# NVlabs/latentfusion

Hardware: AMD Instinct MI355X
Metric: pose-optim iters/sec (reconstruct+render+backward), 16 views, 128^3 voxels (higher is better)
Workload: dtype f32

## Files before the change

### include/lf_hip.h

```cpp
#ifndef LF_HIP_H
#define LF_HIP_H

#include <stddef.h>
#include <stdint.h>

#ifdef __cplusplus
extern "C" {
#endif

#define LF_ABI_VERSION 1

#define LF_EINVAL   (-1)
#define LF_EALIGN   (-2)
#define LF_ENOSPC   (-3)

#define LF_EPI_LRELU     1u
#define LF_EPI_PIXELNORM 2u
#define LF_EPI_ADD       4u
#define LF_EPI_DOT       8u

#define LF_MAP_O2C 0
#define LF_MAP_C2O 1
#define LF_MAP_COEFS 20

int lf_abi_version(void);

int lf_device_name(char* buf, int buflen);

int lf_resample3d_fwd(const float* vol, int vol_n, const float* coef, int kind,
                      float* out, int N, int D, int H, int W, int C, void* stream);

size_t lf_resample3d_bwd_coef_scratch_bytes(int N, int D, int H, int W);
int lf_resample3d_bwd_coef(const float* gout, const float* vol, int vol_n, const float* coef,
                           float* gcoef, void* scratch, size_t scratch_bytes,
                           int N, int D, int H, int W, int C, void* stream);
size_t lf_resample3d_bwd_coef_part_scratch_bytes(int N, int part_n, int D, int H, int W);
int lf_resample3d_bwd_coef_part(const float* gout, const float* vol, int vol_n, const float* coef,
                                float* gcoef, void* scratch, size_t scratch_bytes,
                                int N, int D, int H, int W, int C, int part_n, void* stream);

int lf_resample3d_fwd_indexed(const float* vol, int vol_n, const int32_t* vol_idx, const float* coef, int kind,
                              float* out, int N, int D, int H, int W, int C, void* stream);
size_t lf_resample3d_bwd_coef_indexed_scratch_bytes(int N, int part_n, int D, int H, int W);
int lf_resample3d_bwd_coef_indexed(const float* gout, const float* vol, int vol_n, const int32_t* vol_idx, const float* coef,
                                   float* gcoef, void* scratch, size_t scratch_bytes,
                                   int N, int D, int H, int W, int C, int part_n, void* stream);


size_t lf_resample3d_bwd_vol_det_scratch_bytes(int vol_n, int D, int H, int W, int C);
int lf_resample3d_bwd_vol_det(const float* gout, const float* coef, int kind, float* gvol, int vol_n, void* scratch,
                              size_t scratch_bytes, int N, int D, int H, int W, int C, void* stream);

int lf_conv3x3_cout_padded(int Cout);
int lf_conv1x1_cout_padded(int Cout);

int lf_conv3x3_fwd(const float* x, const float* wpack, const float* bias, float* y, float* norm_out,
                   int dims, int N, int D, int H, int W, int Cin, int Cout,
                   float he, unsigned flags, float slope, float eps, void* stream);

int lf_conv1x1_fwd(const float* x, const float* wpack, const float* bias, float* y, float* norm_out,
                   int N, int P, int Cin, int ksl, long x_batch_stride, long x_slice_stride,
                   int Cout, long y_batch_stride, int y_row_stride, int y_slice_channels,
                   long y_slice_stride,
                   float he, unsigned flags, float slope, float eps, void* stream);
int lf_conv1x1_fwd_scaled(const float* x, const float* xscale, const float* wpack, const float* bias, float* y, float* norm_out,
                          int N, int P, int Cin, int ksl, long x_batch_stride, long x_slice_stride,
                          int Cout, long y_batch_stride, int y_row_stride, int y_slice_channels,
                          long y_slice_stride,
                          float he, unsigned flags, float slope, float eps, void* stream);

int lf_conv3x3_bwd_data(const float* gy, const float* wpack_t, float* gx, int dims, int N, int D, int H, int W,
                        int Cin, int Cout, float he, const float* prev_y, const float* prev_norm,
                        unsigned prev_flags, float slope, void* stream);
int lf_conv1x1_bwd_data(const float* gy, const float* wpack_t, float* gx, int N, int P, int Cin, int Cout,
                        long y_batch_stride, int y_row_stride, int y_slice_channels, long y_slice_stride,
                        float he, const float* prev_y, const float* prev_norm, unsigned prev_flags,
                        float slope, float* amax_out, void* stream);

#define LF_AMAX_FLOATS 2048
size_t lf_conv3d_c16_split_wpack_halfs(void);
void lf_conv3d_c16_split_pairs(int* taps28);
int lf_conv3d_c16_split(const float* x, const void* wsplit, const float* bias, float* y, float* norm_out,
                        int N, int D, int H, int W, float he, unsigned flags, float slope, float eps,
                        const float* prev_y, const float* prev_norm, unsigned prev_flags,
                        const float* amax_in, float* amax_out, void* stream);

size_t lf_conv3d_c16_wino_upack_floats(void);
int lf_conv3d_c16_wino(const float* x, const float* upack, const float* bias, float* y, float* norm_out,
                       int N, int D, int H, int W, float he, unsigned flags, float slope, float eps,
                       const float* prev_y, const float* prev_norm, unsigned prev_flags,
                       float* amax_out, void* stream);

size_t lf_conv3d_c16_wino_proj_pack_floats(int D);
int lf_conv3d_c16_wino_projfwd(const float* x, const float* upack, const float* bias, float* y, float* norm_out,
                               int N, int D, int H, int W, float he, unsigned flags, float slope, float eps,
                               const float* proj_wA, const float* proj_bias, float* zp, float* pnorm,
                               float proj_he, unsigned proj_flags, void* stream);

int lf_round_bf16(const float* x, float* y, long n, void* stream);
size_t lf_conv3d_c16_ring_bf16_wpack_elems(void);
int lf_conv3d_c16_ring_bf16(const float* x, const void* wpack, const float* bias, float* y, float* norm_out,
                            int N, int D, int H, int W, float he, unsigned flags, float slope, float eps,
                            const float* addend, int round_out, void* stream);
#define LF_IO_IN_BF16 1
#define LF_IO_OUT_BF16 2
#define LF_IO_ADDEND_BF16 4
int lf_conv3d_c16_ring_bf16_io(const void* x, const void* wpack, const float* bias, void* y, float* norm_out,
                               int N, int D, int H, int W, float he, unsigned flags, float slope, float eps,
                               const void* addend, int round_out, int io, void* stream);

#define LF_RING_ADD_BF16 1u
#define LF_RING_OUT_BF16 2u
#define LF_RING_ROUND 4u
#define LF_RING_EX_NONE 0
#define LF_RING_EX_RH 1
#define LF_RING_EX_BLEND 2
#define LF_RING_EX_ABWD 3
#define LF_RING_EX_BLOCK 4
#define LF_RING_EX_PREV 5
int lf_conv3d_c16_ring_multi(const void* x, int x_bf16, const void* wpack, int ngroups,
                             void* y0, const void* add0, unsigned flags0, void* y1, const void* add1, unsigned flags1,
                             int extra, const void* e0, const void* e1, void* o2,
                             int N, int D, int H, int W, float he, int addend_per_sample, void* stream);
int lf_conv3d_c16_ring_blend(const void* rh, const void* wpack, void* cand, const void* addend, const float* h, const void* upre,
                             float* h_new, void* h_new_bf16, int N, int D, int H, int W, float he, void* stream);

long lf_wino3d_tiles(int N, int D, int H, int W);
int lf_wino3d_input_transform(const float* x, float* V, int N, int D, int H, int W, int C, void* stream);

#define LF_OUT_DEPTH_INNER 0x100u
int lf_wino_fused_cout_padded(int Cout);
size_t lf_wino_fused_scratch_bytes(int dims, int N, int D, int H, int W, int Cout);
int lf_wino_fused_gemm(const float* V, const float* U2, const float* bias, float* y, void* scratch, size_t scratch_bytes,
                       int dims, int N, int D, int H, int W, int Cin, int Cout, float he, unsigned flags, float slope,
                       void* stream);

size_t lf_wino_fused_scratch_bytes_part(int dims, int N, int D, int H, int W, int Cout, int part_n);
int lf_wino_fused_gemm_part(const float* V, const float* U2, const float* bias, float* y, void* scratch, size_t scratch_bytes,
                            int dims, int N, int D, int H, int W, int Cin, int Cout, float he, unsigned flags, float slope,
                            int part_n, void* stream);

int lf_rows_gemm_cout_padded(int Cout);
int lf_rows_gemm_epi(const float* x, const float* wpack, const float* bias, float* y, float* norm_out,
                     long M, int K, int Cout, float he, unsigned flags, float slope, float eps, void* stream);

int lf_wino_f16x3_cin_padded(int Cin);
int lf_wino3d_input_transform_f16x3(const float* x, const float* amax_in, void* V, int N, int D, int H, int W, int C, void* stream);
size_t lf_wino_fused_f16x3_scratch_bytes(int N, int D, int H, int W, int Cout);
int lf_wino_fused_f16x3_gemm(const void* V, const void* U2, int eU, const float* amax_in, const float* bias, float* y,
                             float* amax_out, void* scratch, size_t scratch_bytes, int N, int D, int H, int W, int Cin, int Cout,
                             float he, unsigned flags, float slope, void* stream);

long lf_wino2d_tiles(int N, int H, int W);
int lf_wino2d_input_transform(const float* x, float* V, int N, int H, int W, int C, void* stream);

int lf_wino2d_input_transform_f16x3(const float* x, void* V, int* eV, int N, int H, int W, int C, void* stream);
size_t lf_wino_fused2d_f16x3_scratch_bytes(int N, int H, int W, int Cout);
int lf_wino_fused2d_f16x3_gemm(const void* V, const int* eV, const void* U2, int eU, const float* bias, float* y, void* scratch,
                               size_t scratch_bytes, int N, int H, int W, int Cin, int Cout, float he, unsigned flags, float slope,
                               void* stream);

int lf_gru_stage_a(const float* upre, const float* rpre, int pre_stride, const float* h, float* u, float* rec,
                   long nvox, int Ch, int rec_stride, int rec_off, void* stream);
int lf_gru_stage_b(const float* h, const float* u, const float* cand, float* h_out, float* rec, long nvox, int Ch,
                   int rec_stride, int rec_off, void* stream);
int lf_gru_stage_b_bwd(const float* g, const float* h, const float* u, const float* cand, float* gh, float* gu, float* gc,
                       long n, void* stream);
int lf_gru_stage_a_bwd(const float* gu, const float* grh, const float* u, const float* rpre, const float* h, float* gupre,
                       float* grpre, float* gh, long n, void* stream);
int lf_gru_train_stage_a(const void* rpre, const float* h, void* rh, long n, int bf16, void* stream);
int lf_gru_train_stage_b(const float* h, const void* upre, const void* cand, float* h_out, long n, int bf16, void* stream);
int lf_gru_train_stage_b_bwd(const float* g, const float* h, const void* upre, const void* cand, float* gh1, void* gupre,
                             void* gc, float* acc_u, float* acc_o, long n, int bf16, void* stream);
int lf_gru_train_stage_a_bwd(const void* grh, const void* rpre, const float* h, const float* gh1, void* grpre, float* gh12,
                             float* acc_r, long n, int bf16, void* stream);
int lf_sum_views_bf16(const void* src, float* dst, long n, int views, int accumulate, void* stream);

int lf_resample3d_fwd_io(const void* vol, int vol_n, const float* coef, int kind, void* out, int N, int D, int H, int W,
                         int io, void* stream);
size_t lf_resample3d_bwd_vol_det_io_scratch_bytes(int vol_n, int N, int D, int H, int W);
int lf_resample3d_bwd_vol_det_io(const void* gout, const float* coef, int kind, void* gvol, int vol_n, void* scratch,
                                 size_t scratch_bytes, int N, int D, int H, int W, int io, void* stream);

int lf_occ_input_fwd(const float* z, const float* w, const float* b, float* ta, float* t16, int N, int D, long P, float slope,
                     void* stream);
int lf_occ_input_bwd(const float* gta, const float* ta, const float* gp16, const float* w, const float* g_zs, const float* wocc,
                     float* gz, long rows, float slope, const float* prev_y, const float* prev_norm, unsigned prev_flags,
                     void* stream);
int lf_occ_input_bwd_proj(const float* gta, const float* gp16, const float* w, const float* gp2d, const float* wpack_t, float he_p,
                          const float* wocc, float* gz, int N, int D, long P, float slope,
                          const float* prev_y, const float* prev_norm, unsigned prev_flags, void* stream);
int lf_occ_weight_grad(const float* z, const float* gp2d, const float* wpack_t, float he_p, float* gw, int N, int D, long P, void* stream);
int lf_occ_weight_grad_softmax_bwd(const float* z, const float* gp2d, const float* wpack_t, float he_p, const float* weights,
                                   float* glogits, int N, int D, long P, void* stream);
int lf_occ_head_bwd(const float* gl, const float* w16, float he, const float* y, const float* norm, unsigned flags, float slope,
                    float* g, long rows, void* stream);
int lf_occ_conv17_fwd(const float* t16, const float* w27, float* pre, int N, int D, int H, int W, void* stream);
int lf_occ_conv17_bwd(const float* g, const float* t16, const float* w27, float* gp16, int N, int D, int H, int W, float slope,
                      void* stream);
int lf_column_reduce_sum_fwd(const float* x, float* y, int N, int D, long P, int C, void* stream);
int lf_column_reduce_sum_bwd(const float* gy, float* gx, int N, int D, long P, int C, void* stream);
int lf_column_softmax_fwd(const float* logits, float* weights, float* zdepth, int N, int D, long P, void* stream);
int lf_column_softmax_head_fwd(const float* y, const float* w16, const float* bias, float he, float* weights, float* zdepth,
                               int N, int D, long P, void* stream);
int lf_column_softmax_bwd(const float* weights, const float* gweights, const float* gzdepth, float* glogits,
                          int N, int D, long P, void* stream);
int lf_column_scale_fwd(const float* z, const float* w, float* out, long rows, int C, void* stream);
int lf_column_scale_bwd(const float* gout, const float* z, const float* w, float* gz, float* gw, long rows, int C,
                        void* stream);

#define LF_FUSE_MEAN   0
#define LF_FUSE_MAX    1
#define LF_FUSE_ABSMAX 2
#define LF_FUSE_MEDIAN 3
int lf_fuse_views_fwd(const float* z, float* out, int* idx, int kind, int V, long n, long view_stride, void* stream);
int lf_fuse_views_bwd(const float* g, const int* idx, float* gz, int kind, int V, long n, long view_stride, void* stream);
int lf_fuse_blend_fwd(const float* z, const float* logits, float* weights, float* out, int V, long rows, int C,
                      long z_view_stride, long logit_view_stride, void* stream);
int lf_fuse_blend_bwd(const float* g, const float* z, const float* weights, float* gz, float* glogits, int V, long rows,
                      int C, long z_view_stride, long logit_view_stride, void* stream);

int lf_lstm_cell_fwd(const float* cc, const float* c_cur, float* h_next, float* c_next, long nvox, int Ch, void* stream);
int lf_lstm_cell_bwd(const float* cc, const float* c_cur, const float* gh, const float* gcn, float* gcc, float* gc,
                     long nvox, int Ch, void* stream);

int lf_grid_sample2d_fwd(const float* img, const float* grid, float* out, int N, int C, int H, int W, int Ho, int Wo,
                         int bilinear, int border, void* stream);
int lf_grid_sample2d_bwd(const float* img, const float* grid, const float* gout, float* gimg, float* ggrid,
                         int N, int C, int H, int W, int Ho, int Wo, int bilinear, int border, void* stream);

#define LF_IBR_PAIR_FLOATS 32
#define LF_IBR_PAIR_SPLIT 16
#define LF_IBR_VIEW_FLOATS 16
#define LF_IBR_VIEW_SPLIT 8
int lf_ibr_reproject_fwd(const float* image_in, const float* depth_in, const float* depth_out, const float* mask_out,
                         const float* pair_rec, const float* in_rec, const float* out_rec, float* image_re, float* depth_re,
                         int B, int Vo, int Vi, int C, int H, int W, long image_row_stride, long depth_row_stride, void* stream);
int lf_ibr_reproject_bwd(const float* image_in, const float* depth_in, const float* depth_out, const float* mask_out,
                         const float* pair_rec, const float* in_rec, const float* out_rec, const float* g_image_re,
                         const float* g_depth_re, float* g_image_in, float* g_depth_in, float* g_depth_out,
                         int B, int Vo, int Vi, int C, int H, int W, void* stream);

size_t lf_conv_bwd_weight_scratch_bytes(int dims, int N, int D, int H, int W, int Cin, int Cout);
int lf_conv_bwd_weight(const float* x, const float* gpre, float* gw, void* scratch, size_t scratch_bytes,
                       int dims, int N, int D, int H, int W, int Cin, int Cout, float scale, void* stream);
size_t lf_conv_bwd_weight_bf16_scratch_bytes(int dims, int N, int D, int H, int W, int Cin, int Cout);
int lf_conv_bwd_weight_bf16(const float* x, const float* gpre, float* gw, void* scratch, size_t scratch_bytes,
                            int dims, int N, int D, int H, int W, int Cin, int Cout, float scale, void* stream);
int lf_conv_bwd_weight_bf16_io(const void* x, const void* gpre, float* gw, void* scratch, size_t scratch_bytes,
                               int dims, int N, int D, int H, int W, int Cin, int Cout, float scale, int io, void* stream);
size_t lf_conv_bwd_weight_wide_scratch_bytes(int dims, int N, int D, int H, int W, int Cin, int Cout);
int lf_conv_bwd_weight_wide(const float* x, const float* gpre, float* gw, void* scratch, size_t scratch_bytes,
                            int dims, int N, int D, int H, int W, int Cin, int Cout, float scale, void* stream);

size_t lf_epilogue_bwd_c16_scratch_bytes(long rows);
int lf_epilogue_bwd_c16(const void* gy, const void* y, const float* norm, void* gp, float* gbias, void* scratch,
                        size_t scratch_bytes, long rows, unsigned flags, float slope, int io, void* stream);

int lf_lift16_fwd(const float* x, const void* wtab, const float* btab, void* vol, float* norm, long R, long P, int S,
                  float he, float slope, float eps, void* stream);
size_t lf_lift16_bwd_scratch_bytes(int S);
int lf_lift16_bwd(const void* gvol, const void* yvol, const float* norm, const float* x, const void* wtab_t, float* gx, float* gw,
                  float* gb, void* scratch, size_t scratch_bytes, long R, long P, int S, float he, float slope, int round_gx,
                  void* stream);

int lf_proj16_fwd(const void* vol, const void* wtab, const float* bias, float* y, float* norm, long R, long P, int S, float he,
                  float slope, float eps, void* stream);
size_t lf_proj16_bwd_scratch_bytes(int S);
int lf_proj16_bwd(const float* gp, const void* vol, const void* wtab_t, void* gxvol, float* gw, void* scratch, size_t scratch_bytes,
                  long R, long P, int S, float he, void* stream);

int lf_pw16_fwd(const void* x, int x_bf16, const void* w_bf16, const float* bias, float he, unsigned flags, float slope, void* y,
                long rows, void* stream);
size_t lf_pw16_bwd_scratch_bytes(long rows);
int lf_pw16_bwd(const void* gy_bf16, const void* wt_bf16, float he, void* gx, int gx_bf16, float* gbias, void* scratch,
                size_t scratch_bytes, long rows, void* stream);

int lf_pixelnorm_fwd(const float* x, float* y, float* norm_out, long rows, int C, float eps, void* stream);

int lf_epilogue_bwd(const float* gy, const float* y, const float* norm, float* gp,
                    long rows, int C, unsigned flags, float slope, void* stream);
int lf_epilogue_bwd_amax(const float* gy, const float* y, const float* norm, float* gp,
                         long rows, int C, unsigned flags, float slope, float* amax_out, void* stream);

size_t lf_latent_cosine_scratch_bytes(int N, long P, int C);
int lf_latent_cosine_fwd(const float* zp, const float* zt, int zt_n, long zt_sn, long zt_sp, long zt_sc, float* sums,
                         float* losses, float w_latent, void* scratch, size_t scratch_bytes, int N, long P, int C,
                         void* stream);
int lf_latent_cosine_bwd_epi(const float* g_in, const float* zp, const float* norm, const float* zt, int zt_n, long zt_sn,
                             long zt_sp, long zt_sc, const float* sums, float gscale, float* gp, int N, long P, int C,
                             unsigned flags, float slope, void* stream);

size_t lf_nn_dist_scratch_bytes(int B, int M, int Q);
int lf_nn_dist(const float* x1, long x1_sb, const float* T1, const float* x2, long x2_sb, const float* T2, float* dist, int* idx,
               float* mean, void* scratch, size_t scratch_bytes, int B, int M, int Q, void* stream);
size_t lf_points_pair_dist_scratch_bytes(int R, int P);
int lf_points_pair_dist(const float* pts, long pts_sr, const float* A, const float* Bm, int rows, float* mean, void* scratch,
                        size_t scratch_bytes, int R, int P, void* stream);

int lf_resize_fwd(const float* x, float* y, int dims, int N, int D, int H, int W, int C, int linear, int up,
                  void* stream);
int lf_resize_bwd(const float* gy, float* gx, int dims, int N, int D, int H, int W, int C, int linear, int up,
                  void* stream);

#define LF_CAM_PARAMS 10
#define LF_CAM_COEFS  24
int lf_camera_coefs(const float* params, const float* intrinsics, float cube_size, float z_span,
                    int crop_h, int crop_w, float* coefs, float* jac, int N, void* stream);
int lf_camera_coefs_bwd(const float* gcoefs, const float* jac, float* gparams, int N, void* stream);

size_t lf_pose_loss_scratch_bytes(int N, int h, int w, int H, int W);
int lf_pose_loss_fwd(const float* logits, const float* coefs, const float* target_depth,
                     const float* target_mask, const float* weights, float* sums, float* losses,
                     float* gsums, void* scratch, size_t scratch_bytes,
                     int N, int h, int w, int H, int W, void* stream);
int lf_pose_loss_bwd(const float* logits, const float* coefs, const float* target_depth,
                     const float* target_mask, const float* gsums, float* glogits, float* gcoefs,
                     void* scratch, size_t scratch_bytes, int N, int h, int w, int H, int W, void* stream);
int lf_pose_loss_fwd_masked(const float* logits, const float* coefs, const float* target_depth,
                            const float* target_mask, const float* weights, float* sums, float* losses,
                            void* scratch, size_t scratch_bytes, int N, int h, int w, int H, int W, void* stream);
int lf_pose_loss_fwd_depth(const float* depth_and_logits, const float* coefs, const float* target_depth,
                           const float* target_mask, const float* weights, float* sums, float* losses,
                           float* gsums, void* scratch, size_t scratch_bytes,
                           int N, int h, int w, int H, int W, void* stream);
int lf_pose_loss_bwd_depth(const float* depth_and_logits, const float* coefs, const float* target_depth,
                           const float* target_mask, const float* gsums, float* gcrop, float* gcoefs,
                           void* scratch, size_t scratch_bytes, int N, int h, int w, int H, int W, void* stream);
int lf_pose_loss_fwd_mt(const float* logits, const float* coefs, const float* target_depth,
                        const float* target_mask, const float* weights, float* sums, float* losses,
                        float* gsums, void* scratch, size_t scratch_bytes,
                        int N, int T, int n, int h, int w, int H, int W, void* stream);
int lf_pose_loss_fwd_masked_mt(const float* logits, const float* coefs, const float* target_depth,
                               const float* target_mask, const float* weights, float* sums, float* losses,
                               void* scratch, size_t scratch_bytes, int N, int T, int n, int h, int w, int H, int W,
                               void* stream);
int lf_pose_loss_bwd_mt(const float* logits, const float* coefs, const float* target_depth,
                        const float* target_mask, const float* gsums, float* glogits, float* gcoefs,
                        void* scratch, size_t scratch_bytes, int N, int T, int n, int h, int w, int H, int W,
                        void* stream);

int lf_adam_step(float* params, const float* grads, float* exp_avg, float* exp_avg_sq,
                 const float* step_size, const float* lr, float bias_correction2_sqrt,
                 float beta1, float beta2, float eps, float weight_decay, int N, int P, void* stream);

int lf_nchw_to_nhwc(const float* src, float* dst, int N, int C, long P, void* stream);
int lf_nhwc_to_nchw(const float* src, float* dst, int N, int C, long P, void* stream);
int lf_lift_unfold(const float* src, const float* norm_or_null, float* dst,
                   int N, long P, int C0, int S, void* stream);
int lf_lift_permute(const float* src, float* dst, int N, long P, int C0, int S, int fold, void* stream);
int lf_lift_norm_unfold(const float* src, void* dst, float* norm_out, int N, long P, int C0, int S, float eps, int out_bf16,
                        void* stream);
int lf_lift_bwd(const void* gvol, const void* yvol, const float* norm, float* gp, int N, long P, int C0, int S, float slope,
                int round_bf16, int io, void* stream);

#ifdef __cplusplus
}
#endif
#endif
```

### latentfusion_amd/_lib.py

```python
import ctypes
import os
from ctypes import c_char_p, c_float, c_int, c_long, c_size_t, c_uint, c_void_p

_HERE = os.path.dirname(os.path.abspath(__file__))
LIB_PATH = os.path.join(_HERE, 'csrc', 'liblf_hip.so')

LF_EPI_LRELU = 1
LF_EPI_PIXELNORM = 2
LF_EPI_ADD = 4
LF_EPI_DOT = 8
LF_RING_ADD_BF16, LF_RING_OUT_BF16, LF_RING_ROUND = 1, 2, 4
LF_RING_EX_NONE, LF_RING_EX_RH, LF_RING_EX_BLEND, LF_RING_EX_ABWD, LF_RING_EX_BLOCK, LF_RING_EX_PREV = 0, 1, 2, 3, 4, 5
LF_OUT_DEPTH_INNER = 0x100
LF_IO_IN_BF16, LF_IO_OUT_BF16, LF_IO_ADDEND_BF16 = 1, 2, 4
LF_MAP_O2C = 0
LF_MAP_C2O = 1
LF_MAP_COEFS = 20
LF_FUSE_MEAN, LF_FUSE_MAX, LF_FUSE_ABSMAX, LF_FUSE_MEDIAN = 0, 1, 2, 3
LF_IBR_PAIR_FLOATS, LF_IBR_PAIR_SPLIT, LF_IBR_VIEW_FLOATS, LF_IBR_VIEW_SPLIT = 32, 16, 16, 8
LF_AMAX_FLOATS = 2048

P = c_void_p
SIGNATURES = {
    'lf_abi_version': (c_int, []),
    'lf_device_name': (c_int, [c_char_p, c_int]),
    'lf_resample3d_fwd': (c_int, [P, c_int, P, c_int, P, c_int, c_int, c_int, c_int, c_int, P]),
    'lf_resample3d_bwd_coef_scratch_bytes': (c_size_t, [c_int, c_int, c_int, c_int]),
    'lf_resample3d_bwd_coef': (c_int, [P, P, c_int, P, P, P, c_size_t, c_int, c_int, c_int, c_int, c_int, P]),
    'lf_resample3d_bwd_coef_part_scratch_bytes': (c_size_t, [c_int, c_int, c_int, c_int, c_int]),
    'lf_resample3d_bwd_coef_part': (c_int, [P, P, c_int, P, P, P, c_size_t, c_int, c_int, c_int, c_int, c_int, c_int, P]),
    'lf_resample3d_fwd_indexed': (c_int, [P, c_int, P, P, c_int, P, c_int, c_int, c_int, c_int, c_int, P]),
    'lf_resample3d_bwd_coef_indexed_scratch_bytes': (c_size_t, [c_int, c_int, c_int, c_int, c_int]),
    'lf_resample3d_bwd_coef_indexed': (c_int, [P, P, c_int, P, P, P, P, c_size_t, c_int, c_int, c_int, c_int, c_int, c_int, P]),
    'lf_resample3d_bwd_vol_det_scratch_bytes': (c_size_t, [c_int, c_int, c_int, c_int, c_int]),
    'lf_resample3d_bwd_vol_det': (c_int, [P, P, c_int, P, c_int, P, c_size_t, c_int, c_int, c_int, c_int, c_int, P]),
    'lf_conv3x3_cout_padded': (c_int, [c_int]),
    'lf_conv1x1_cout_padded': (c_int, [c_int]),
    'lf_conv3x3_fwd': (c_int, [P, P, P, P, P, c_int, c_int, c_int, c_int, c_int, c_int, c_int,
                               c_float, c_uint, c_float, c_float, P]),
    'lf_conv1x1_fwd': (c_int, [P, P, P, P, P, c_int, c_int, c_int, c_int, c_long, c_long, c_int, c_long, c_int,
                               c_int, c_long, c_float, c_uint, c_float, c_float, P]),
    'lf_conv1x1_fwd_scaled': (c_int, [P, P, P, P, P, P, c_int, c_int, c_int, c_int, c_long, c_long, c_int, c_long, c_int,
                                      c_int, c_long, c_float, c_uint, c_float, c_float, P]),
    'lf_conv3x3_bwd_data': (c_int, [P, P, P, c_int, c_int, c_int, c_int, c_int, c_int, c_int, c_float, P, P, c_uint,
                                    c_float, P]),
    'lf_conv1x1_bwd_data': (c_int, [P, P, P, c_int, c_int, c_int, c_int, c_long, c_int, c_int, c_long, c_float, P, P,
                                    c_uint, c_float, P, P]),
    'lf_conv3d_c16_split_wpack_halfs': (c_size_t, []),
    'lf_conv3d_c16_split_pairs': (None, [P]),
    'lf_conv3d_c16_split': (c_int, [P, P, P, P, P, c_int, c_int, c_int, c_int, c_float, c_uint, c_float, c_float, P, P,
                                    c_uint, P, P, P]),
    'lf_conv3d_c16_wino_upack_floats': (c_size_t, []),
    'lf_conv3d_c16_wino': (c_int, [P, P, P, P, P, c_int, c_int, c_int, c_int, c_float, c_uint, c_float, c_float, P, P,
                                   c_uint, P, P]),
    'lf_conv3d_c16_wino_proj_pack_floats': (c_size_t, [c_int]),
    'lf_conv3d_c16_wino_projfwd': (c_int, [P, P, P, P, P, c_int, c_int, c_int, c_int, c_float, c_uint, c_float, c_float,
                                           P, P, P, P, c_float, c_uint, P]),
    'lf_round_bf16': (c_int, [P, P, c_long, P]),
    'lf_conv3d_c16_ring_bf16_wpack_elems': (c_size_t, []),
    'lf_conv3d_c16_ring_bf16': (c_int, [P, P, P, P, P, c_int, c_int, c_int, c_int, c_float, c_uint, c_float, c_float, P, c_int, P]),
    'lf_conv3d_c16_ring_bf16_io': (c_int, [P, P, P, P, P, c_int, c_int, c_int, c_int, c_float, c_uint, c_float, c_float, P, c_int, c_int, P]),
    'lf_conv3d_c16_ring_multi': (c_int, [P, c_int, P, c_int, P, P, c_uint, P, P, c_uint, c_int, P, P, P, c_int, c_int, c_int, c_int, c_float, c_int, P]),
    'lf_conv3d_c16_ring_blend': (c_int, [P, P, P, P, P, P, P, P, c_int, c_int, c_int, c_int, c_float, P]),
    'lf_wino3d_tiles': (c_long, [c_int, c_int, c_int, c_int]),
    'lf_wino3d_input_transform': (c_int, [P, P, c_int, c_int, c_int, c_int, c_int, P]),
    'lf_wino_fused_cout_padded': (c_int, [c_int]),
    'lf_wino_fused_scratch_bytes': (c_size_t, [c_int, c_int, c_int, c_int, c_int, c_int]),
    'lf_wino_fused_gemm': (c_int, [P, P, P, P, P, c_size_t, c_int, c_int, c_int, c_int, c_int, c_int, c_int, c_float, c_uint, c_float, P]),
    'lf_wino_fused_scratch_bytes_part': (c_size_t, [c_int, c_int, c_int, c_int, c_int, c_int, c_int]),
    'lf_wino_fused_gemm_part': (c_int, [P, P, P, P, P, c_size_t, c_int, c_int, c_int, c_int, c_int, c_int, c_int, c_float, c_uint, c_float, c_int, P]),
    'lf_rows_gemm_cout_padded': (c_int, [c_int]),
    'lf_rows_gemm_epi': (c_int, [P, P, P, P, P, c_long, c_int, c_int, c_float, c_uint, c_float, c_float, P]),
    'lf_wino_f16x3_cin_padded': (c_int, [c_int]),
    'lf_wino3d_input_transform_f16x3': (c_int, [P, P, P, c_int, c_int, c_int, c_int, c_int, P]),
    'lf_wino_fused_f16x3_scratch_bytes': (c_size_t, [c_int, c_int, c_int, c_int, c_int]),
    'lf_wino_fused_f16x3_gemm': (c_int, [P, P, c_int, P, P, P, P, P, c_size_t, c_int, c_int, c_int, c_int, c_int, c_int,
                                         c_float, c_uint, c_float, P]),
    'lf_wino2d_tiles': (c_long, [c_int, c_int, c_int]),
    'lf_wino2d_input_transform': (c_int, [P, P, c_int, c_int, c_int, c_int, P]),
    'lf_wino2d_input_transform_f16x3': (c_int, [P, P, P, c_int, c_int, c_int, c_int, P]),
    'lf_wino_fused2d_f16x3_scratch_bytes': (c_size_t, [c_int, c_int, c_int, c_int]),
    'lf_wino_fused2d_f16x3_gemm': (c_int, [P, P, P, c_int, P, P, P, c_size_t, c_int, c_int, c_int, c_int, c_int, c_float, c_uint,
                                           c_float, P]),
    'lf_gru_stage_a': (c_int, [P, P, c_int, P, P, P, c_long, c_int, c_int, c_int, P]),
    'lf_gru_stage_b': (c_int, [P, P, P, P, P, c_long, c_int, c_int, c_int, P]),
    'lf_lstm_cell_fwd': (c_int, [P, P, P, P, c_long, c_int, P]),
    'lf_lstm_cell_bwd': (c_int, [P, P, P, P, P, P, c_long, c_int, P]),
    'lf_gru_stage_b_bwd': (c_int, [P, P, P, P, P, P, P, c_long, P]),
    'lf_gru_stage_a_bwd': (c_int, [P, P, P, P, P, P, P, P, c_long, P]),
    'lf_gru_train_stage_a': (c_int, [P, P, P, c_long, c_int, P]),
    'lf_gru_train_stage_b': (c_int, [P, P, P, P, c_long, c_int, P]),
    'lf_gru_train_stage_b_bwd': (c_int, [P, P, P, P, P, P, P, P, P, c_long, c_int, P]),
    'lf_gru_train_stage_a_bwd': (c_int, [P, P, P, P, P, P, P, c_long, c_int, P]),
    'lf_lift16_fwd': (c_int, [P, P, P, P, P, c_long, c_long, c_int, c_float, c_float, c_float, P]),
    'lf_lift16_bwd_scratch_bytes': (c_size_t, [c_int]),
    'lf_lift16_bwd': (c_int, [P, P, P, P, P, P, P, P, P, c_size_t, c_long, c_long, c_int, c_float, c_float, c_int, P]),
    'lf_proj16_fwd': (c_int, [P, P, P, P, P, c_long, c_long, c_int, c_float, c_float, c_float, P]),
    'lf_proj16_bwd_scratch_bytes': (c_size_t, [c_int]),
    'lf_proj16_bwd': (c_int, [P, P, P, P, P, P, c_size_t, c_long, c_long, c_int, c_float, P]),
    'lf_sum_views_bf16': (c_int, [P, P, c_long, c_int, c_int, P]),
    'lf_occ_input_fwd': (c_int, [P, P, P, P, P, c_int, c_int, c_long, c_float, P]),
    'lf_occ_input_bwd': (c_int, [P, P, P, P, P, P, P, c_long, c_float, P, P, c_uint, P]),
    'lf_occ_conv17_fwd': (c_int, [P, P, P, c_int, c_int, c_int, c_int, P]),
    'lf_occ_conv17_bwd': (c_int, [P, P, P, P, c_int, c_int, c_int, c_int, c_float, P]),
    'lf_column_reduce_sum_fwd': (c_int, [P, P, c_int, c_int, c_long, c_int, P]),
    'lf_column_reduce_sum_bwd': (c_int, [P, P, c_int, c_int, c_long, c_int, P]),
    'lf_column_softmax_fwd': (c_int, [P, P, P, c_int, c_int, c_long, P]),
    'lf_occ_input_bwd_proj': (c_int, [P, P, P, P, P, c_float, P, P, c_int, c_int, c_long, c_float, P, P, c_uint, P]),
    'lf_occ_weight_grad': (c_int, [P, P, P, c_float, P, c_int, c_int, c_long, P]),
    'lf_pw16_fwd': (c_int, [P, c_int, P, P, c_float, c_uint, c_float, P, c_long, P]),
    'lf_pw16_bwd_scratch_bytes': (c_size_t, [c_long]),
    'lf_pw16_bwd': (c_int, [P, P, c_float, P, c_int, P, P, c_size_t, c_long, P]),
    'lf_occ_weight_grad_softmax_bwd': (c_int, [P, P, P, c_float, P, P, c_int, c_int, c_long, P]),
    'lf_occ_head_bwd': (c_int, [P, P, c_float, P, P, c_uint, c_float, P, c_long, P]),
    'lf_column_softmax_head_fwd': (c_int, [P, P, P, c_float, P, P, c_int, c_int, c_long, P]),
    'lf_column_softmax_bwd': (c_int, [P, P, P, P, c_int, c_int, c_long, P]),
    'lf_column_scale_fwd': (c_int, [P, P, P, c_long, c_int, P]),
    'lf_column_scale_bwd': (c_int, [P, P, P, P, P, c_long, c_int, P]),
    'lf_fuse_views_fwd': (c_int, [P, P, P, c_int, c_int, c_long, c_long, P]),
    'lf_fuse_views_bwd': (c_int, [P, P, P, c_int, c_int, c_long, c_long, P]),
    'lf_fuse_blend_fwd': (c_int, [P, P, P, P, c_int, c_long, c_int, c_long, c_long, P]),
    'lf_fuse_blend_bwd': (c_int, [P, P, P, P, P, c_int, c_long, c_int, c_long, c_long, P]),
    'lf_grid_sample2d_fwd': (c_int, [P, P, P, c_int, c_int, c_int, c_int, c_int, c_int, c_int, c_int, P]),
    'lf_grid_sample2d_bwd': (c_int, [P, P, P, P, P, c_int, c_int, c_int, c_int, c_int, c_int, c_int, c_int, P]),
    'lf_ibr_reproject_fwd': (c_int, [P, P, P, P, P, P, P, P, P, c_int, c_int, c_int, c_int, c_int, c_int, c_long, c_long, P]),
    'lf_ibr_reproject_bwd': (c_int, [P, P, P, P, P, P, P, P, P, P, P, P, c_int, c_int, c_int, c_int, c_int, c_int, P]),
    'lf_conv_bwd_weight_scratch_bytes': (c_size_t, [c_int, c_int, c_int, c_int, c_int, c_int, c_int]),
    'lf_conv_bwd_weight': (c_int, [P, P, P, P, c_size_t, c_int, c_int, c_int, c_int, c_int, c_int, c_int, c_float, P]),
    'lf_conv_bwd_weight_bf16_scratch_bytes': (c_size_t, [c_int, c_int, c_int, c_int, c_int, c_int, c_int]),
    'lf_conv_bwd_weight_bf16': (c_int, [P, P, P, P, c_size_t, c_int, c_int, c_int, c_int, c_int, c_int, c_int, c_float, P]),
    'lf_conv_bwd_weight_bf16_io': (c_int, [P, P, P, P, c_size_t, c_int, c_int, c_int, c_int, c_int, c_int, c_int, c_float, c_int, P]),
    'lf_conv_bwd_weight_wide_scratch_bytes': (c_size_t, [c_int, c_int, c_int, c_int, c_int, c_int, c_int]),
    'lf_conv_bwd_weight_wide': (c_int, [P, P, P, P, c_size_t, c_int, c_int, c_int, c_int, c_int, c_int, c_int, c_float, P]),
    'lf_pixelnorm_fwd': (c_int, [P, P, P, c_long, c_int, c_float, P]),
    'lf_epilogue_bwd': (c_int, [P, P, P, P, c_long, c_int, c_uint, c_float, P]),
    'lf_epilogue_bwd_amax': (c_int, [P, P, P, P, c_long, c_int, c_uint, c_float, P, P]),
    'lf_latent_cosine_scratch_bytes': (c_size_t, [c_int, c_long, c_int]),
    'lf_latent_cosine_fwd': (c_int, [P, P, c_int, c_long, c_long, c_long, P, P, c_float, P, c_size_t, c_int, c_long, c_int, P]),
    'lf_latent_cosine_bwd_epi': (c_int, [P, P, P, P, c_int, c_long, c_long, c_long, P, c_float, P, c_int, c_long, c_int, c_uint,
                                         c_float, P]),
    'lf_nn_dist_scratch_bytes': (c_size_t, [c_int, c_int, c_int]),
    'lf_nn_dist': (c_int, [P, c_long, P, P, c_long, P, P, P, P, P, c_size_t, c_int, c_int, c_int, P]),
    'lf_points_pair_dist_scratch_bytes': (c_size_t, [c_int, c_int]),
    'lf_points_pair_dist': (c_int, [P, c_long, P, P, c_int, P, P, c_size_t, c_int, c_int, P]),
    'lf_epilogue_bwd_c16_scratch_bytes': (c_size_t, [c_long]),
    'lf_epilogue_bwd_c16': (c_int, [P, P, P, P, P, P, c_size_t, c_long, c_uint, c_float, c_int, P]),
    'lf_resample3d_fwd_io': (c_int, [P, c_int, P, c_int, P, c_int, c_int, c_int, c_int, c_int, P]),
    'lf_resample3d_bwd_vol_det_io_scratch_bytes': (c_size_t, [c_int, c_int, c_int, c_int, c_int]),
    'lf_resample3d_bwd_vol_det_io': (c_int, [P, P, c_int, P, c_int, P, c_size_t, c_int, c_int, c_int, c_int, c_int, P]),
    'lf_resize_fwd': (c_int, [P, P, c_int, c_int, c_int, c_int, c_int, c_int, c_int, c_int, P]),
    'lf_resize_bwd': (c_int, [P, P, c_int, c_int, c_int, c_int, c_int, c_int, c_int, c_int, P]),
    'lf_camera_coefs': (c_int, [P, P, c_float, c_float, c_int, c_int, P, P, c_int, P]),
    'lf_camera_coefs_bwd': (c_int, [P, P, P, c_int, P]),
    'lf_pose_loss_scratch_bytes': (c_size_t, [c_int, c_int, c_int, c_int, c_int]),
    'lf_pose_loss_fwd': (c_int, [P, P, P, P, P, P, P, P, P, c_size_t, c_int, c_int, c_int, c_int, c_int, P]),
    'lf_pose_loss_bwd': (c_int, [P, P, P, P, P, P, P, P, c_size_t, c_int, c_int, c_int, c_int, c_int, P]),
    'lf_pose_loss_fwd_depth': (c_int, [P, P, P, P, P, P, P, P, P, c_size_t, c_int, c_int, c_int, c_int, c_int, P]),
    'lf_pose_loss_bwd_depth': (c_int, [P, P, P, P, P, P, P, P, c_size_t, c_int, c_int, c_int, c_int, c_int, P]),
    'lf_pose_loss_fwd_masked': (c_int, [P, P, P, P, P, P, P, P, c_size_t, c_int, c_int, c_int, c_int, c_int, P]),
    'lf_pose_loss_fwd_mt': (c_int, [P, P, P, P, P, P, P, P, P, c_size_t, c_int, c_int, c_int, c_int, c_int, c_int, c_int, P]),
    'lf_pose_loss_fwd_masked_mt': (c_int, [P, P, P, P, P, P, P, P, c_size_t, c_int, c_int, c_int, c_int, c_int, c_int, c_int,
                                           P]),
    'lf_pose_loss_bwd_mt': (c_int, [P, P, P, P, P, P, P, P, c_size_t, c_int, c_int, c_int, c_int, c_int, c_int, c_int, P]),
    'lf_adam_step': (c_int, [P, P, P, P, P, P, c_float, c_float, c_float, c_float, c_float, c_int, c_int, P]),
    'lf_nchw_to_nhwc': (c_int, [P, P, c_int, c_int, c_long, P]),
    'lf_nhwc_to_nchw': (c_int, [P, P, c_int, c_int, c_long, P]),
    'lf_lift_unfold': (c_int, [P, P, P, c_int, c_long, c_int, c_int, P]),
    'lf_lift_permute': (c_int, [P, P, c_int, c_long, c_int, c_int, c_int, P]),
    'lf_lift_norm_unfold': (c_int, [P, P, P, c_int, c_long, c_int, c_int, c_float, c_int, P]),
    'lf_lift_bwd': (c_int, [P, P, P, P, c_int, c_long, c_int, c_int, c_float, c_int, c_int, P]),
}

EXPERIMENTAL_SIGNATURES = {
    'lf_set_tuning': (c_int, [c_int, c_int]),
    'lf_resample3d_bwd_vol': (c_int, [P, P, c_int, P, c_int, c_int, c_int, c_int, c_int, c_int, P]),
    'lf_conv3d_c16_wino_projbwd': (c_int, [P, P, c_float, P, P, c_uint, P, P, c_int, c_int, c_int, c_int, c_float, c_float,
                                           P, P, c_uint, P]),
    'lf_conv3d_c16_wino_split_upack_halfs': (c_size_t, []),
    'lf_conv3d_c16_wino_split': (c_int, [P, P, P, P, P, c_int, c_int, c_int, c_int, c_float, c_uint, c_float, c_float, P, P,
                                         c_uint, P, P, P]),
    'lf_conv3d_c16_bf16_wpack_elems': (c_size_t, []),
    'lf_conv3d_c16_bf16': (c_int, [P, P, P, P, P, c_int, c_int, c_int, c_int, c_float, c_uint, c_float, c_float, c_int, P]),
    'lf_wino3d_output_transform': (c_int, [P, P, P, P, c_int, c_int, c_int, c_int, c_int, c_float, c_uint, c_float, c_float, P]),
    'lf_wino2d_output_transform': (c_int, [P, P, P, P, c_int, c_int, c_int, c_int, c_float, c_uint, c_float, c_float, P]),
}

_lib = None


class LFHipError(RuntimeError):
    pass


def lib():
    global _lib
    if _lib is not None:
        return _lib
    if not os.path.exists(LIB_PATH):
        try:
            from .csrc import build as _build
            _build.build(verbose=False)
        except Exception as e:
            raise LFHipError(f'liblf_hip.so is missing at {LIB_PATH} and could not be built: {e}') from e
    import torch
    try:
        handle = ctypes.CDLL(LIB_PATH)
    except OSError as e:
        raise LFHipError(f'cannot load {LIB_PATH}: {e}') from e
    for name, (res, args) in list(SIGNATURES.items()) + list(EXPERIMENTAL_SIGNATURES.items()):
        try:
            fn = getattr(handle, name)
        except AttributeError as e:
            raise LFHipError(f'{LIB_PATH} does not export {name}') from e
        fn.restype = res
        fn.argtypes = args
    if handle.lf_abi_version() != 1:
        raise LFHipError('liblf_hip.so ABI version mismatch')
    _lib = handle
    return _lib


_ERR = {-1: 'LF_EINVAL (bad size/flag combination)', -2: 'LF_EALIGN (alignment / channel count)',
        -3: 'LF_ENOSPC (scratch too small)'}


BYTE_LOG = None
_PENDING = [0]


def note_bytes(t, scratch=False):
    if BYTE_LOG is not None and not scratch:
        n = t.numel() * t.element_size()
        try:
            n = min(n, t.untyped_storage().nbytes() - t.storage_offset() * t.element_size())
        except Exception:
            pass
        _PENDING[0] += n


def check(rc, what):
    if BYTE_LOG is not None:
        e = BYTE_LOG.setdefault(what, [0, 0])
        e[0] += 1
        e[1] += _PENDING[0]
        _PENDING[0] = 0
    if rc != 0:
        raise LFHipError(f'{what} failed: {_ERR.get(rc, "hipError " + str(rc))}')
```

### latentfusion_amd/csrc/image.hip

```cpp
#include "lf_common.h"

namespace {

constexpr int NP = 10;
template <int ND>
struct DualT {
  double v;
  double d[ND];
};
template <int ND> __device__ inline DualT<ND> dconst_(double c) { DualT<ND> r; r.v = c; for (int i = 0; i < ND; ++i) r.d[i] = 0.0; return r; }
template <int ND> __device__ inline DualT<ND> dvar_(double c, int idx, int mine) {
  DualT<ND> r = dconst_<ND>(c);
  if (ND == 1) r.d[0] = (idx == mine) ? 1.0 : 0.0; else r.d[idx % ND] = 1.0;
  return r;
}
template <int ND> __device__ inline DualT<ND> operator+(const DualT<ND>& a, const DualT<ND>& b) { DualT<ND> r; r.v = a.v + b.v; for (int i = 0; i < ND; ++i) r.d[i] = a.d[i] + b.d[i]; return r; }
template <int ND> __device__ inline DualT<ND> operator-(const DualT<ND>& a, const DualT<ND>& b) { DualT<ND> r; r.v = a.v - b.v; for (int i = 0; i < ND; ++i) r.d[i] = a.d[i] - b.d[i]; return r; }
template <int ND> __device__ inline DualT<ND> operator-(const DualT<ND>& a) { DualT<ND> r; r.v = -a.v; for (int i = 0; i < ND; ++i) r.d[i] = -a.d[i]; return r; }
template <int ND> __device__ inline DualT<ND> operator*(const DualT<ND>& a, const DualT<ND>& b) { DualT<ND> r; r.v = a.v * b.v; for (int i = 0; i < ND; ++i) r.d[i] = a.d[i] * b.v + a.v * b.d[i]; return r; }
template <int ND> __device__ inline DualT<ND> operator*(const DualT<ND>& a, double s) { DualT<ND> r; r.v = a.v * s; for (int i = 0; i < ND; ++i) r.d[i] = a.d[i] * s; return r; }
template <int ND> __device__ inline DualT<ND> operator+(const DualT<ND>& a, double s) { DualT<ND> r = a; r.v += s; return r; }
template <int ND> __device__ inline DualT<ND> operator-(const DualT<ND>& a, double s) { DualT<ND> r = a; r.v -= s; return r; }
template <int ND> __device__ inline DualT<ND> operator/(const DualT<ND>& a, const DualT<ND>& b) {
  DualT<ND> r; const double inv = 1.0 / b.v; r.v = a.v * inv;
  for (int i = 0; i < ND; ++i) r.d[i] = (a.d[i] - r.v * b.d[i]) * inv;
  return r;
}
template <int ND> __device__ inline DualT<ND> dsqrt(const DualT<ND>& a) {
  DualT<ND> r; r.v = sqrt(a.v); const double k = r.v > 0.0 ? 0.5 / r.v : 0.0;
  for (int i = 0; i < ND; ++i) r.d[i] = a.d[i] * k;
  return r;
}
template <int ND> __device__ inline DualT<ND> dsin(const DualT<ND>& a) { DualT<ND> r; r.v = sin(a.v); const double c = cos(a.v); for (int i = 0; i < ND; ++i) r.d[i] = a.d[i] * c; return r; }
template <int ND> __device__ inline DualT<ND> dcos(const DualT<ND>& a) { DualT<ND> r; r.v = cos(a.v); const double s = -sin(a.v); for (int i = 0; i < ND; ++i) r.d[i] = a.d[i] * s; return r; }
template <int ND> __device__ inline DualT<ND> dclamp_min(const DualT<ND>& a, double lo) { return a.v >= lo ? a : dconst_<ND>(lo); }

constexpr int NOUT = 24;

template <int ND>
__global__ void camera_coefs_kernel(const float* __restrict__ params, const float* __restrict__ intr,
                                    float cube, float z_span, int crop_h, int crop_w,
                                    float* __restrict__ out, float* __restrict__ jac, int N) {
  typedef DualT<ND> Dual;
  const int tid = blockIdx.x * blockDim.x + threadIdx.x;
  const int n = ND == 1 ? tid / NP : tid, mine = ND == 1 ? tid % NP : 0;
  if (n >= N) return;
  auto dconst = [](double c) { return dconst_<ND>(c); };
  auto dvar = [&](double c, int idx) { return dvar_<ND>(c, idx, mine); };
  const float* p = params + n * NP;
  Dual w[3], t[3], vp[4];
  for (int i = 0; i < 3; ++i) w[i] = dvar((double)p[i], i);
  for (int i = 0; i < 3; ++i) t[i] = dvar((double)p[3 + i], 3 + i);
  for (int i = 0; i < 4; ++i) vp[i] = dvar((double)p[6 + i], 6 + i);
  const double fu = intr[n * 4 + 0], fv = intr[n * 4 + 1], u0 = intr[n * 4 + 2], v0 = intr[n * 4 + 3];

  const Dual theta = dsqrt(w[0] * w[0] + w[1] * w[1] + w[2] * w[2]);
  const Dual sc = dsin(theta) / dclamp_min(theta, 1e-8);
  Dual q[4] = {dcos(theta), sc * w[0], sc * w[1], sc * w[2]};
  for (int rep = 0; rep < 2; ++rep) {
    const Dual nrm = dclamp_min(dsqrt(q[0] * q[0] + q[1] * q[1] + q[2] * q[2] + q[3] * q[3]), 1e-12);
    for (int i = 0; i < 4; ++i) q[i] = q[i] / nrm;
  }
  const Dual qw = q[0], qx = q[1], qy = q[2], qz = q[3];
  const Dual tx = qx * 2.0, ty = qy * 2.0, tz = qz * 2.0;
  Dual R[3][3];
  R[0][0] = dconst(1.0) - (ty * qy + tz * qz); R[0][1] = ty * qx - tz * qw;               R[0][2] = tz * qx + ty * qw;
  R[1][0] = ty * qx + tz * qw;               R[1][1] = dconst(1.0) - (tx * qx + tz * qz); R[1][2] = tz * qy - tx * qw;
  R[2][0] = tz * qx - ty * qw;               R[2][1] = tz * qy + tx * qw;               R[2][2] = dconst(1.0) - (tx * qx + ty * qy);

  const Dual vw = vp[2] - vp[0], vh = vp[3] - vp[1];
  const Dual al0 = (vp[0] - u0) * (1.0 / fu), al1 = vw * (1.0 / fu);
  const Dual be0 = (vp[1] - v0) * (1.0 / fv), be1 = vh * (1.0 / fv);
  const Dual g0 = t[2] - (double)z_span;
  const double g1 = z_span, s = 2.0 / cube;
  Dual c[6][3];
  for (int r = 0; r < 3; ++r) {
    const Dual m0 = R[0][r], m1 = R[1][r], m2 = R[2][r];
    const Dual rt = m0 * t[0] + m1 * t[1] + m2 * t[2];
    c[0][r] = (al0 * g0 * m0 + be0 * g0 * m1 + g0 * m2 - rt) * s;
    c[1][r] = (al1 * g0 * m0) * s;
    c[2][r] = (be1 * g0 * m1) * s;
    c[3][r] = (al0 * m0 + be0 * m1 + m2) * (g1 * s);
    c[4][r] = (al1 * m0) * (g1 * s);
    c[5][r] = (be1 * m1) * (g1 * s);
  }
  Dual o[NOUT];
  for (int j = 0; j < 6; ++j) for (int r = 0; r < 3; ++r) o[j * 3 + r] = c[j][r];
  o[18] = dconst((double)crop_w) / vw;
  o[19] = -(vp[0] * o[18]) - 0.5;
  o[20] = dconst((double)crop_h) / vh;
  o[21] = -(vp[1] * o[20]) - 0.5;
  o[22] = dconst((double)z_span + 0.01);
  o[23] = t[2];
  for (int j = 0; j < NOUT; ++j) {
    if (ND != 1 || mine == 0) out[n * NOUT + j] = (float)o[j].v;
    if (ND == 1) jac[(n * NOUT + j) * NP + mine] = (float)o[j].d[0];
    else for (int i = 0; i < ND; ++i) jac[(n * NOUT + j) * NP + i] = (float)o[j].d[i];
  }
}

__global__ void camera_coefs_bwd_kernel(const float* __restrict__ gout, const float* __restrict__ jac,
                                        float* __restrict__ gparams, int N) {
  const int idx = blockIdx.x * blockDim.x + threadIdx.x;
  if (idx >= N * NP) return;
  const int n = idx / NP, i = idx % NP;
  double s = 0.0;
  for (int j = 0; j < NOUT; ++j) s += (double)gout[n * NOUT + j] * (double)jac[(n * NOUT + j) * NP + i];
  gparams[idx] = (float)s;
}

constexpr int NSUM = 8;
constexpr int LOSS_BLOCK = 256;

struct PixelFwd {
  float sig, dhat, pd, td, mt, valid, l1, logit;
  float wx0, wx1, wy0, wy1, mx, my;
  int x0, x1, y0, y1, xn, yn;
  float dn;
  bool mask_on;
};

__device__ __forceinline__ float sigmoidf_(float v) { return 1.f / (1.f + expf(-v)); }

__device__ __forceinline__ void clip_pos(float p, int size, float& pos, float& mult) {
  const float hi = (float)(size - 1);
  mult = (p > 0.f && p < hi) ? 1.f : 0.f;
  pos = fminf(fmaxf(p, 0.f), hi);
}

template <int MODE = 0>
__device__ __forceinline__ PixelFwd pixel_forward(const float* __restrict__ lg, const float* __restrict__ cf,
                                                  int h, int w, int x, int y, float td_raw, float mt) {
  PixelFwd r;
  float px, py;
  clip_pos(cf[0] * (float)x + cf[1], w, px, r.mx);
  clip_pos(cf[2] * (float)y + cf[3], h, py, r.my);
  const float fx = floorf(px), fy = floorf(py);
  r.wx1 = px - fx; r.wx0 = 1.f - r.wx1; r.wy1 = py - fy; r.wy0 = 1.f - r.wy1;
  r.x0 = (int)fx; r.y0 = (int)fy; r.x1 = min(r.x0 + 1, w - 1); r.y1 = min(r.y0 + 1, h - 1);
  r.xn = (int)nearbyintf(px); r.yn = (int)nearbyintf(py);
  const float m00 = lg[(r.y0 * w + r.x0) * 2 + 1], m01 = lg[(r.y0 * w + r.x1) * 2 + 1];
  const float m10 = lg[(r.y1 * w + r.x0) * 2 + 1], m11 = lg[(r.y1 * w + r.x1) * 2 + 1];
  r.logit = m00 * (r.wx0 * r.wy0) + m01 * (r.wx1 * r.wy0) + m10 * (r.wx0 * r.wy1) + m11 * (r.wx1 * r.wy1);
  r.sig = sigmoidf_(r.logit);
  const float dl = lg[(r.yn * w + r.xn) * 2 + 0], ml = lg[(r.yn * w + r.xn) * 2 + 1];
  if constexpr (MODE == 2) {
    r.mask_on = true;
    r.dn = dl;
    r.dhat = dl;
  } else {
    r.mask_on = sigmoidf_(ml) > 0.5f;
    r.dn = r.mask_on ? tanhf(dl) : (dl != dl ? dl : -1.f);
    r.dhat = r.dn * cf[4] + cf[5];
    if constexpr (MODE == 1) r.dhat *= sigmoidf_(ml);
  }
  r.pd = r.dhat * r.sig;
  r.mt = mt;
  r.valid = (td_raw == 0.f && mt > 0.1f) ? 0.f : 1.f;
  r.td = td_raw * mt;
  r.l1 = fabsf(r.pd - r.td) * r.valid;
  return r;
}

__device__ __forceinline__ void block_reduce_store(float (&acc)[NSUM], float* __restrict__ dst) {
  __shared__ float red[LOSS_BLOCK / 64][NSUM];
  const int lane = threadIdx.x & 63, wave = threadIdx.x >> 6;
#pragma unroll
  for (int i = 0; i < NSUM; ++i) {
    const float s = lf_wave_sum(acc[i]);
    if (lane == 0) red[wave][i] = s;
  }
  __syncthreads();
  if (threadIdx.x < NSUM) {
    float s = 0.f;
    for (int wv = 0; wv < LOSS_BLOCK / 64; ++wv) s += red[wv][threadIdx.x];
    dst[threadIdx.x] = s;
  }
}

template <int MODE>
__global__ void __launch_bounds__(LOSS_BLOCK) pose_loss_fwd_kernel(
    const float* __restrict__ logits, const float* __restrict__ coef, const float* __restrict__ tdepth,
    const float* __restrict__ tmask, float* __restrict__ partial, int nblk, int h, int w, int H, int W) {
  const int n = blockIdx.y;
  const float* lg = logits + (long)n * h * w * 2;
  const float* cf = coef + n * NOUT + 18;
  float acc[NSUM];
#pragma unroll
  for (int i = 0; i < NSUM; ++i) acc[i] = 0.f;
  for (int p = blockIdx.x * LOSS_BLOCK + threadIdx.x; p < H * W; p += nblk * LOSS_BLOCK) {
    const int y = p / W, x = p - y * W;
    const PixelFwd f = pixel_forward<MODE>(lg, cf, h, w, x, y, tdepth[p], tmask[p]);
    acc[0] += f.l1;
    acc[1] += f.l1 * (f.sig * f.mt);
    acc[2] += f.sig * f.mt;
    acc[3] += f.sig;
    acc[4] += f.sig * (f.mt * f.valid);
    acc[5] += f.mt * f.valid;
    acc[6] += (1.f - f.mt) * f.logit + (log1pf(expf(-fabsf(f.logit))) + fmaxf(-f.logit, 0.f));
  }
  block_reduce_store(acc, partial + ((long)n * nblk + blockIdx.x) * NSUM);
}

__global__ void pose_loss_finish_kernel(const float* __restrict__ partial, int nblk, const float* __restrict__ weights,
                                        int N, int HW, float* __restrict__ sums, float* __restrict__ losses,
                                        float* __restrict__ gsums) {
  const int n = blockIdx.x;
  __shared__ double S[NSUM];
#pragma unroll
  for (int c = 0; c < NSUM; ++c) {
    double s = 0.0;
    for (int b = threadIdx.x; b < nblk; b += 64) s += (double)partial[((long)n * nblk + b) * NSUM + c];
#pragma unroll
    for (int o = 32; o > 0; o >>= 1) s += __shfl_xor(s, o, 64);
    if (threadIdx.x == 0) {
      S[c] = s;
      sums[n * NSUM + c] = (float)s;
    }
  }
  __syncthreads();
  if (threadIdx.x == 0) {
    const float S0 = (float)S[0], S1 = (float)S[1], S2 = (float)S[2], S3 = (float)S[3], S4 = (float)S[4],
                S5 = (float)S[5], S6 = (float)S[6];
    const float w_depth = weights[0], w_ov = weights[1], w_iou = weights[2], w_mask = weights[3];
    const float inv_hw = 1.f / (float)HW;
    const float depth = S0 * inv_hw;
    auto clamp_min = [](float v, float lo) { return v < lo ? lo : v; };
    const float num = clamp_min(S1, 1e-5f), den = clamp_min(S2, 1e-4f);
    const float ov = num / den;
    const float uni = S3 + S5 - S4;
    const float iou = logf(clamp_min(uni, 1e-4f)) - logf(clamp_min(S4, 1e-4f));
    const float mask = S6 * inv_hw;
    losses[n * 8 + 0] = depth; losses[n * 8 + 1] = ov; losses[n * 8 + 2] = iou; losses[n * 8 + 3] = mask;
    losses[n * 8 + 4] = w_depth * depth + w_ov * ov + w_iou * iou + w_mask * mask;
    losses[n * 8 + 5] = 0.f; losses[n * 8 + 6] = 0.f; losses[n * 8 + 7] = 0.f;
    const float k = 1.f / (float)N;
    float* g = gsums + n * NSUM;
    const float d_uni = uni > 1e-4f ? 1.f / uni : 0.f;
    g[0] = k * w_depth * inv_hw;
    g[1] = k * w_ov * (S1 > 1e-5f ? 1.f / den : 0.f);
    g[2] = k * w_ov * (S2 > 1e-4f ? -num / (den * den) : 0.f);
    g[3] = k * w_iou * d_uni;
    g[4] = k * w_iou * (-d_uni - (S4 > 1e-4f ? 1.f / S4 : 0.f));
    g[5] = 0.f;
    g[6] = k * w_mask * inv_hw;
    g[7] = 0.f;
  }
}

template <int MODE>
__global__ void __launch_bounds__(LOSS_BLOCK) pose_loss_bwd_pixels_kernel(
    const float* __restrict__ logits, const float* __restrict__ coef, const float* __restrict__ tdepth,
    const float* __restrict__ tmask, const float* __restrict__ gsums, float* __restrict__ gd_frame,
    float* __restrict__ gm_frame, float* __restrict__ partial, int nblk, int h, int w, int H, int W) {
  const int n = blockIdx.y;
  const float* lg = logits + (long)n * h * w * 2;
  const float* cf = coef + n * NOUT + 18;
  const float* g = gsums + n * NSUM;
  const float g0 = g[0], g1 = g[1], g2 = g[2], g3 = g[3], g4 = g[4], g6 = g[6];
  float acc[NSUM];
#pragma unroll
  for (int i = 0; i < NSUM; ++i) acc[i] = 0.f;
  for (int p = blockIdx.x * LOSS_BLOCK + threadIdx.x; p < H * W; p += nblk * LOSS_BLOCK) {
    const int y = p / W, x = p - y * W;
    const PixelFwd f = pixel_forward<MODE>(lg, cf, h, w, x, y, tdepth[p], tmask[p]);
    const float dl1 = g0 + g1 * (f.sig * f.mt);
    const float diff = f.pd - f.td;
    const float dpd = dl1 * f.valid * (diff > 0.f ? 1.f : (diff < 0.f ? -1.f : 0.f));
    const float ddhat = dpd * f.sig;
    const float dsig = dpd * f.dhat + g1 * f.l1 * f.mt + g2 * f.mt + g3 + g4 * (f.mt * f.valid);
    const float dlogit = dsig * f.sig * (1.f - f.sig) + g6 * (f.sig - f.mt);
    gd_frame[(long)n * H * W + p] = ddhat;
    gm_frame[(long)n * H * W + p] = dlogit;
    const float m00 = lg[(f.y0 * w + f.x0) * 2 + 1], m01 = lg[(f.y0 * w + f.x1) * 2 + 1];
    const float m10 = lg[(f.y1 * w + f.x0) * 2 + 1], m11 = lg[(f.y1 * w + f.x1) * 2 + 1];
    const float dix = ((m01 - m00) * f.wy0 + (m11 - m10) * f.wy1) * f.mx * dlogit;
    const float diy = ((m10 - m00) * f.wx0 + (m11 - m01) * f.wx1) * f.my * dlogit;
    acc[0] += dix * (float)x; acc[1] += dix;
    acc[2] += diy * (float)y; acc[3] += diy;
    if constexpr (MODE != 2) { acc[4] += ddhat * f.dn;   acc[5] += ddhat; }
  }
  block_reduce_store(acc, partial + ((long)n * nblk + blockIdx.x) * NSUM);
}

__global__ void __launch_bounds__(256) pose_loss_bwd_rows_kernel(
    const float* __restrict__ coef, const float* __restrict__ gd_frame, const float* __restrict__ gm_frame,
    float* __restrict__ Td, float* __restrict__ Tm, int w, int H, int W) {
  const int n = blockIdx.z;
  const int y = blockIdx.y;
  const int cx = blockIdx.x * blockDim.x + threadIdx.x;
  if (cx >= w) return;
  const float ax = coef[n * NOUT + 18], bx = coef[n * NOUT + 19];
  int xlo = (int)floorf(((float)cx - 1.f - bx) / ax) - 1, xhi = (int)ceilf(((float)cx + 1.f - bx) / ax) + 1;
  if (cx == 0) xlo = 0;
  if (cx == w - 1) xhi = W - 1;
  xlo = max(xlo, 0); xhi = min(xhi, W - 1);
  const float* gd = gd_frame + ((long)n * H + y) * W;
  const float* gm = gm_frame + ((long)n * H + y) * W;
  float sd = 0.f, sm = 0.f;
  for (int x = xlo; x <= xhi; ++x) {
    float px, mult;
    clip_pos(ax * (float)x + bx, w, px, mult);
    const float fx = floorf(px);
    const int x0 = (int)fx, x1 = min(x0 + 1, w - 1);
    const float wx1 = px - fx, wx0 = 1.f - wx1;
    float wgt = 0.f;
    if (x0 == cx) wgt += wx0;
    if (x1 == cx) wgt += wx1;
    sm += wgt * gm[x];
    if ((int)nearbyintf(px) == cx) sd += gd[x];
  }
  Td[((long)n * H + y) * w + cx] = sd;
  Tm[((long)n * H + y) * w + cx] = sm;
}

template <int MODE>
__global__ void __launch_bounds__(256) pose_loss_bwd_cols_kernel(
    const float* __restrict__ logits, const float* __restrict__ coef, const float* __restrict__ Td,
    const float* __restrict__ Tm, float* __restrict__ glogits, int h, int w, int H) {
  const int n = blockIdx.z;
  const int cy = blockIdx.y;
  const int cx = blockIdx.x * blockDim.x + threadIdx.x;
  if (cx >= w) return;
  const float ay = coef[n * NOUT + 20], by = coef[n * NOUT + 21], a_depth = coef[n * NOUT + 22];
  int ylo = (int)floorf(((float)cy - 1.f - by) / ay) - 1, yhi = (int)ceilf(((float)cy + 1.f - by) / ay) + 1;
  if (cy == 0) ylo = 0;
  if (cy == h - 1) yhi = H - 1;
  ylo = max(ylo, 0); yhi = min(yhi, H - 1);
  float sd = 0.f, sm = 0.f;
  for (int y = ylo; y <= yhi; ++y) {
    float py, mult;
    clip_pos(ay * (float)y + by, h, py, mult);
    const float fy = floorf(py);
    const int y0 = (int)fy, y1 = min(y0 + 1, h - 1);
    const float wy1 = py - fy, wy0 = 1.f - wy1;
    float wgt = 0.f;
    if (y0 == cy) wgt += wy0;
    if (y1 == cy) wgt += wy1;
    sm += wgt * Tm[((long)n * H + y) * w + cx];
    if ((int)nearbyintf(py) == cy) sd += Td[((long)n * H + y) * w + cx];
  }
  const long o = ((long)n * h * w + (long)cy * w + cx) * 2;
  if constexpr (MODE == 2) {
    glogits[o] = sd;
  } else {
    const float dl = logits[o], ml = logits[o + 1];
    const float th = tanhf(dl);
    const bool on = sigmoidf_(ml) > 0.5f;
    const float g = on ? sd * a_depth * (1.f - th * th) : 0.f;
    glogits[o] = (!on && dl != dl) ? dl : g;
  }
  glogits[o + 1] = sm;
}

__global__ void reduce_partials_kernel(const float* __restrict__ partial, int nblk, float* __restrict__ out, int ncomp,
                                       int out_stride, int out_offset) {
  const int n = blockIdx.x;
  for (int c = 0; c < ncomp; ++c) {
    double s = 0.0;
    for (int b = threadIdx.x; b < nblk; b += 64) s += (double)partial[((long)n * nblk + b) * NSUM + c];
#pragma unroll
    for (int o = 32; o > 0; o >>= 1) s += __shfl_xor(s, o, 64);
    if (threadIdx.x == 0) out[n * out_stride + out_offset + c] = (float)s;
  }
}

constexpr int LOSS_NBLK = 240;

}

extern "C" int lf_camera_coefs(const float* params, const float* intrinsics, float cube_size, float z_span,
                               int crop_h, int crop_w, float* coefs, float* jac, int N, void* stream) {
  lf_clear_error();
  if (N <= 0 || crop_h <= 0 || crop_w <= 0 || cube_size <= 0.f) return LF_EINVAL;
  hipLaunchKernelGGL((camera_coefs_kernel<1>), dim3((N * NP + 63) / 64), dim3(64), 0, (hipStream_t)stream, params, intrinsics,
                     cube_size, z_span, crop_h, crop_w, coefs, jac, N);
  return lf_launch_status();
}

extern "C" int lf_camera_coefs_bwd(const float* gcoefs, const float* jac, float* gparams, int N, void* stream) {
  lf_clear_error();
  if (N <= 0) return LF_EINVAL;
  hipLaunchKernelGGL(camera_coefs_bwd_kernel, dim3((N * NP + 63) / 64), dim3(64), 0, (hipStream_t)stream, gcoefs, jac,
                     gparams, N);
  return lf_launch_status();
}

extern "C" size_t lf_pose_loss_scratch_bytes(int N, int h, int w, int H, int W) {
  return ((size_t)N * LOSS_NBLK * NSUM + 2 * (size_t)N * H * W + 2 * (size_t)N * H * w) * sizeof(float);
}

static int pose_loss_fwd_launch(int mode, const float* logits, const float* coefs, const float* target_depth,
                                const float* target_mask, const float* weights, float* sums, float* losses,
                                float* gsums, void* scratch, size_t scratch_bytes,
                                int N, int h, int w, int H, int W, void* stream) {
  lf_clear_error();
  if (N <= 0 || h <= 1 || w <= 1 || H <= 0 || W <= 0) return LF_EINVAL;
  if (scratch_bytes < lf_pose_loss_scratch_bytes(N, h, w, H, W)) return LF_ENOSPC;
  hipStream_t s = (hipStream_t)stream;
  float* partial = (float*)scratch;
  if (mode == 1)
    hipLaunchKernelGGL(pose_loss_fwd_kernel<1>, dim3(LOSS_NBLK, N), dim3(LOSS_BLOCK), 0, s, logits, coefs, target_depth,
                       target_mask, partial, LOSS_NBLK, h, w, H, W);
  else if (mode == 2)
    hipLaunchKernelGGL(pose_loss_fwd_kernel<2>, dim3(LOSS_NBLK, N), dim3(LOSS_BLOCK), 0, s, logits, coefs, target_depth,
                       target_mask, partial, LOSS_NBLK, h, w, H, W);
  else
    hipLaunchKernelGGL(pose_loss_fwd_kernel<0>, dim3(LOSS_NBLK, N), dim3(LOSS_BLOCK), 0, s, logits, coefs, target_depth,
                       target_mask, partial, LOSS_NBLK, h, w, H, W);
  int st = lf_launch_status();
  if (st) return st;
  hipLaunchKernelGGL(pose_loss_finish_kernel, dim3(N), dim3(64), 0, s, partial, LOSS_NBLK, weights, N, H * W, sums, losses,
                     gsums);
  return lf_launch_status();
}

extern "C" int lf_pose_loss_fwd(const float* logits, const float* coefs, const float* target_depth,
                                const float* target_mask, const float* weights, float* sums, float* losses,
                                float* gsums, void* scratch, size_t scratch_bytes,
                                int N, int h, int w, int H, int W, void* stream) {
  return pose_loss_fwd_launch(0, logits, coefs, target_depth, target_mask, weights, sums, losses, gsums, scratch,
                              scratch_bytes, N, h, w, H, W, stream);
}

extern "C" int lf_pose_loss_fwd_depth(const float* depth_and_logits, const float* coefs, const float* target_depth,
                                      const float* target_mask, const float* weights, float* sums, float* losses,
                                      float* gsums, void* scratch, size_t scratch_bytes,
                                      int N, int h, int w, int H, int W, void* stream) {
  return pose_loss_fwd_launch(2, depth_and_logits, coefs, target_depth, target_mask, weights, sums, losses, gsums, scratch,
                              scratch_bytes, N, h, w, H, W, stream);
}

extern "C" int lf_pose_loss_fwd_masked(const float* logits, const float* coefs, const float* target_depth,
                                       const float* target_mask, const float* weights, float* sums, float* losses,
                                       void* scratch, size_t scratch_bytes,
                                       int N, int h, int w, int H, int W, void* stream) {
  float* gs = (float*)scratch + (size_t)N * LOSS_NBLK * NSUM;
  return pose_loss_fwd_launch(1, logits, coefs, target_depth, target_mask, weights, sums, losses, gs, scratch,
                              scratch_bytes, N, h, w, H, W, stream);
}

static int pose_loss_bwd_launch(int mode, const float* logits, const float* coefs, const float* target_depth,
                                const float* target_mask, const float* gsums, float* glogits, float* gcoefs,
                                void* scratch, size_t scratch_bytes, int N, int h, int w, int H, int W, void* stream);

extern "C" int lf_pose_loss_bwd(const float* logits, const float* coefs, const float* target_depth,
                                const float* target_mask, const float* gsums, float* glogits, float* gcoefs,
                                void* scratch, size_t scratch_bytes, int N, int h, int w, int H, int W, void* stream) {
  return pose_loss_bwd_launch(0, logits, coefs, target_depth, target_mask, gsums, glogits, gcoefs, scratch, scratch_bytes, N, h, w, H, W,
                              stream);
}

extern "C" int lf_pose_loss_bwd_depth(const float* depth_and_logits, const float* coefs, const float* target_depth,
                                      const float* target_mask, const float* gsums, float* gcrop, float* gcoefs,
                                      void* scratch, size_t scratch_bytes, int N, int h, int w, int H, int W, void* stream) {
  return pose_loss_bwd_launch(2, depth_and_logits, coefs, target_depth, target_mask, gsums, gcrop, gcoefs, scratch, scratch_bytes, N, h, w,
                              H, W, stream);
}

static int pose_loss_bwd_launch(int mode, const float* logits, const float* coefs, const float* target_depth,
                                const float* target_mask, const float* gsums, float* glogits, float* gcoefs,
                                void* scratch, size_t scratch_bytes, int N, int h, int w, int H, int W, void* stream) {
  lf_clear_error();
  if (N <= 0 || h <= 1 || w <= 1 || H <= 0 || W <= 0) return LF_EINVAL;
  if (scratch_bytes < lf_pose_loss_scratch_bytes(N, h, w, H, W)) return LF_ENOSPC;
  hipStream_t s = (hipStream_t)stream;
  float* partial = (float*)scratch;
  float* gd = partial + (size_t)N * LOSS_NBLK * NSUM;
  float* gm = gd + (size_t)N * H * W;
  float* Td = gm + (size_t)N * H * W;
  float* Tm = Td + (size_t)N * H * w;
  if (mode == 2)
    hipLaunchKernelGGL(pose_loss_bwd_pixels_kernel<2>, dim3(LOSS_NBLK, N), dim3(LOSS_BLOCK), 0, s, logits, coefs, target_depth,
                       target_mask, gsums, gd, gm, partial, LOSS_NBLK, h, w, H, W);
  else
    hipLaunchKernelGGL(pose_loss_bwd_pixels_kernel<0>, dim3(LOSS_NBLK, N), dim3(LOSS_BLOCK), 0, s, logits, coefs, target_depth,
                       target_mask, gsums, gd, gm, partial, LOSS_NBLK, h, w, H, W);
  int st = lf_launch_status();
  if (st) return st;
  hipLaunchKernelGGL(reduce_partials_kernel, dim3(N), dim3(64), 0, s, partial, LOSS_NBLK, gcoefs, 6, NOUT, 18);
  hipLaunchKernelGGL(pose_loss_bwd_rows_kernel, dim3((w + 255) / 256, H, N), dim3(256), 0, s, coefs, gd, gm, Td, Tm, w, H, W);
  if (mode == 2)
    hipLaunchKernelGGL(pose_loss_bwd_cols_kernel<2>, dim3((w + 255) / 256, h, N), dim3(256), 0, s, logits, coefs, Td, Tm, glogits,
                       h, w, H);
  else
    hipLaunchKernelGGL(pose_loss_bwd_cols_kernel<0>, dim3((w + 255) / 256, h, N), dim3(256), 0, s, logits, coefs, Td, Tm, glogits,
                       h, w, H);
  return lf_launch_status();
}

static bool pose_loss_mt_args_ok(int N, int T, int n) {
  return T >= 1 && n >= 1 && (long)T * n == (long)N;
}

static int pose_loss_fwd_mt_launch(int mode, const float* logits, const float* coefs, const float* target_depth,
                                   const float* target_mask, const float* weights, float* sums, float* losses,
                                   float* gsums, void* scratch, size_t scratch_bytes,
                                   int N, int T, int n, int h, int w, int H, int W, void* stream) {
  if (N <= 0 || h <= 1 || w <= 1 || H <= 0 || W <= 0) return LF_EINVAL;
  if (scratch_bytes < lf_pose_loss_scratch_bytes(N, h, w, H, W)) return LF_ENOSPC;
  hipStream_t s = (hipStream_t)stream;
  float* partial = (float*)scratch;
  for (int t = 0; t < T; ++t) {
    const long r0 = (long)t * n;
    const float* lg = logits + r0 * h * w * 2;
    const float* cf = coefs + r0 * NOUT;
    const float* td = target_depth + (long)t * H * W;
    const float* tm = target_mask + (long)t * H * W;
    float* pt = partial + r0 * LOSS_NBLK * NSUM;
    if (mode == 1)
      hipLaunchKernelGGL(pose_loss_fwd_kernel<1>, dim3(LOSS_NBLK, n), dim3(LOSS_BLOCK), 0, s, lg, cf, td, tm, pt, LOSS_NBLK, h, w, H, W);
    else
      hipLaunchKernelGGL(pose_loss_fwd_kernel<0>, dim3(LOSS_NBLK, n), dim3(LOSS_BLOCK), 0, s, lg, cf, td, tm, pt, LOSS_NBLK, h, w, H, W);
    int st = lf_launch_status();
    if (st) return st;
  }
  hipLaunchKernelGGL(pose_loss_finish_kernel, dim3(N), dim3(64), 0, s, partial, LOSS_NBLK, weights, n, H * W, sums, losses, gsums);
  return lf_launch_status();
}

extern "C" int lf_pose_loss_fwd_mt(const float* logits, const float* coefs, const float* target_depth,
                                   const float* target_mask, const float* weights, float* sums, float* losses,
                                   float* gsums, void* scratch, size_t scratch_bytes,
                                   int N, int T, int n, int h, int w, int H, int W, void* stream) {
  lf_clear_error();
  if (!logits || !coefs || !target_depth || !target_mask || !weights || !sums || !losses || !gsums || !scratch)
    return LF_EINVAL;
  if (!pose_loss_mt_args_ok(N, T, n)) return LF_EINVAL;
  return pose_loss_fwd_mt_launch(0, logits, coefs, target_depth, target_mask, weights, sums, losses, gsums, scratch,
                                 scratch_bytes, N, T, n, h, w, H, W, stream);
// ... 44 lines not shown
```

### latentfusion_amd/csrc/lf_common.h

```cpp
#pragma once
#include <hip/hip_runtime.h>
#include <stdint.h>
#include "../../include/lf_hip.h"
#include "../../include/lf_hip_experimental.h"

#define LF_WAVE 64

typedef float f32x4 __attribute__((ext_vector_type(4)));

static inline void lf_clear_error() { (void)hipGetLastError(); }

static inline int lf_launch_status() {
  hipError_t e = hipGetLastError();
  return (int)e;
}

static inline bool lf_aligned16(const void* p) { return (((uintptr_t)p) & 15u) == 0; }

#include <atomic>
typedef std::atomic<unsigned long long> lf_devmask_t;
static inline hipError_t lf_ensure_dyn_lds(lf_devmask_t& done, const void* fn, int bytes) {
  int dev = 0;
  if (hipGetDevice(&dev) != hipSuccess) dev = 0;
  const unsigned long long bit = 1ull << (dev & 63);
  if (done.load(std::memory_order_acquire) & bit) return hipSuccess;
  const hipError_t e = hipFuncSetAttribute(fn, hipFuncAttributeMaxDynamicSharedMemorySize, bytes);
  if (e == hipSuccess) done.fetch_or(bit, std::memory_order_release);
  return e;
}

static inline int lf_cu_count() {
  static std::atomic<int> cus[64];
  int dev = 0, v = 0;
  const bool known = hipGetDevice(&dev) == hipSuccess;
  std::atomic<int>& slot = cus[dev & 63];
  const int c = slot.load(std::memory_order_relaxed);
  if (c != 0) return c;
  const int n = (known && hipDeviceGetAttribute(&v, hipDeviceAttributeMultiprocessorCount, dev) == hipSuccess && v > 0) ? v : 256;
  slot.store(n, std::memory_order_relaxed);
  return n;
}

__device__ __forceinline__ float lf_wave_sum(float v) {
#pragma unroll
  for (int o = 32; o > 0; o >>= 1) v += __shfl_xor(v, o, 64);
  return v;
}

#define LF_AMAX_SLOTS 64
#define LF_AMAX_STRIDE 32
static_assert(LF_AMAX_FLOATS == LF_AMAX_SLOTS * LF_AMAX_STRIDE, "lf_hip.h: LF_AMAX_FLOATS");

__device__ __forceinline__ void lf_amax_publish(float* base, float wave_max, int lane) {
  if (lane == 0 && wave_max > 0.f)
    atomicMax((unsigned int*)(base + (blockIdx.x % LF_AMAX_SLOTS) * LF_AMAX_STRIDE), __float_as_uint(wave_max));
}

__device__ __forceinline__ float lf_amax_read(const float* base, int lane) {
  float m = base[(lane % LF_AMAX_SLOTS) * LF_AMAX_STRIDE];
#pragma unroll
  for (int o = 32; o > 0; o >>= 1) m = fmaxf(m, __shfl_xor(m, o, 64));
  return m;
}

__device__ __forceinline__ float lf_lrelu(float v, float slope) { return v > 0.f ? v : v * slope; }

int lf_internal_ring_bf16_set_wgs(int v);
int lf_internal_wino_set_pack(int v);
int lf_internal_wino_set_forms(int v);
int lf_internal_fused_set_cfg(int v);
int lf_internal_splat_set_variant(int v);
int lf_internal_splat_set_chunk_cap(int v);
```

### latentfusion_amd/csrc/resample.hip

```cpp
#include "resample_map.h"

namespace {

typedef unsigned u32x4_t __attribute__((ext_vector_type(4)));

struct Tap {
  int x0, y0, z0, x1, y1, z1;
  float tx, ty, tz;
  float mx, my, mz;
};

__device__ __forceinline__ float lattice01(int i, int size, float step) {
  return (i < size / 2) ? step * (float)i : 1.f - step * (float)(size - 1 - i);
}


template <int KIND>
__device__ __forceinline__ void eval_grid(const float* __restrict__ cf, int x, int y, int z,
                                          int W, int H, int D, Steps st, float& gx, float& gy, float& gz,
                                          float& a, float& b, float& k) {
  a = lattice01(x, W, st.w);
  b = lattice01(y, H, st.h);
  k = lattice01(z, D, st.d);
  if (KIND == LF_MAP_O2C) {
    const float ak = a * k, bk = b * k;
    gx = cf[0] + cf[3] * a + cf[6] * b + cf[9] * k + cf[12] * ak + cf[15] * bk;
    gy = cf[1] + cf[4] * a + cf[7] * b + cf[10] * k + cf[13] * ak + cf[16] * bk;
    gz = cf[2] + cf[5] * a + cf[8] * b + cf[11] * k + cf[14] * ak + cf[17] * bk;
  } else {
    const float lx = 2.f * a - 1.f, ly = 2.f * b - 1.f, lz = 2.f * k - 1.f;
    const float n0 = cf[0] * lx + cf[1] * ly + cf[2] * lz + cf[3];
    const float n1 = cf[4] * lx + cf[5] * ly + cf[6] * lz + cf[7];
    const float n2 = cf[8] * lx + cf[9] * ly + cf[10] * lz + cf[11];
    const float dn = cf[12] * lx + cf[13] * ly + cf[14] * lz + cf[15];
    gx = n0 / dn;
    gy = n1 / dn;
    gz = n2;
  }
}

__device__ __forceinline__ void unnormalize_clip(float g, int size, float& pos, float& mult) {
  float p = ((g + 1.f) * (float)size - 1.f) * 0.5f;
  const float hi = (float)(size - 1);
  mult = (p > 0.f && p < hi) ? 0.5f * (float)size : 0.f;
  p = fminf(fmaxf(p, 0.f), hi);
  pos = p;
}

__device__ __forceinline__ Tap make_tap(float gx, float gy, float gz, int W, int H, int D) {
  Tap t;
  float px, py, pz;
  unnormalize_clip(gx, W, px, t.mx);
  unnormalize_clip(gy, H, py, t.my);
  unnormalize_clip(gz, D, pz, t.mz);
  if (!(px == px)) px = 0.f;
  if (!(py == py)) py = 0.f;
  if (!(pz == pz)) pz = 0.f;
  const float fx = floorf(px), fy = floorf(py), fz = floorf(pz);
  t.tx = px - fx; t.ty = py - fy; t.tz = pz - fz;
  t.x0 = (int)fx; t.y0 = (int)fy; t.z0 = (int)fz;
  t.x1 = min(t.x0 + 1, W - 1); t.y1 = min(t.y0 + 1, H - 1); t.z1 = min(t.z0 + 1, D - 1);
  return t;
}

__device__ __forceinline__ unsigned xcd_contiguous(unsigned b, unsigned nb) {
  return (nb % 8 == 0) ? (b % 8) * (nb / 8) + b / 8 : b;
}

static int bwd_vox_per_block(long nvox, int N) {
  long v = nvox * N / 2048;
  int p = 64;
  while (p < 4096 && p * 2 <= v) p <<= 1;
  return p;
}
struct BwdTile { int lx, ly, lz, ntx, nty, ntz; };
static BwdTile bwd_tile(int vpb, int D, int H, int W) {
  int lg = 0;
  while ((1 << lg) < vpb) ++lg;
  BwdTile t;
  t.lx = (lg + 2) / 3; t.ly = (lg + 1) / 3; t.lz = lg / 3;
  t.ntx = (W + (1 << t.lx) - 1) >> t.lx; t.nty = (H + (1 << t.ly) - 1) >> t.ly; t.ntz = (D + (1 << t.lz) - 1) >> t.lz;
  return t;
}

__global__ void __launch_bounds__(256) resample_bwd_coef_reduce(const float* __restrict__ partial,
                                                                int nblk, float* __restrict__ gcoef) {
  const int n = blockIdx.x;
  __shared__ double red[256];
  const int comp = threadIdx.x % 18;
  const int grp = threadIdx.x / 18;
  double s = 0.0;
  if (grp < 14)
    for (int b = grp; b < nblk; b += 14) s += (double)partial[((long)n * nblk + b) * 18 + comp];
  red[threadIdx.x] = (grp < 14) ? s : 0.0;
  __syncthreads();
  if (threadIdx.x < 18) {
    double tot = 0.0;
    for (int g = 0; g < 14; ++g) tot += red[g * 18 + threadIdx.x];
    gcoef[(long)n * 18 + threadIdx.x] = (float)tot;
  }
}

template <int KIND>
__global__ void __launch_bounds__(256) resample_bwd_vol_kernel(
    const float* __restrict__ gout, const float* __restrict__ coef, float* __restrict__ gvol,
    long gvol_bstride, int N, int D, int H, int W, int C, Steps st) {
  const long per_sample = (long)D * H * W * C;
  const int n = blockIdx.y;
  const float* cf = coef + (long)n * LF_MAP_COEFS;
  for (long idx = (long)blockIdx.x * blockDim.x + threadIdx.x; idx < per_sample;
       idx += (long)gridDim.x * blockDim.x) {
    const int c = (int)(idx % C);
    long v = idx / C;
    const int x = (int)(v % W); v /= W;
    const int y = (int)(v % H);
    const int z = (int)(v / H);
    float gx, gy, gz, a, b, k;
    eval_grid<KIND>(cf, x, y, z, W, H, D, st, gx, gy, gz, a, b, k);
    const Tap t = make_tap(gx, gy, gz, W, H, D);
    const float go = gout[(long)n * per_sample + idx];
    float* base = gvol + (long)n * gvol_bstride + c;
    const long sW = C, sH = (long)W * C, sD = (long)H * W * C;
    const float wx1 = t.tx, wx0 = 1.f - t.tx, wy1 = t.ty, wy0 = 1.f - t.ty, wz1 = t.tz, wz0 = 1.f - t.tz;
    atomicAdd(base + t.z0 * sD + t.y0 * sH + t.x0 * sW, go * (wx0 * wy0 * wz0));
    atomicAdd(base + t.z0 * sD + t.y0 * sH + t.x1 * sW, go * (wx1 * wy0 * wz0));
    atomicAdd(base + t.z0 * sD + t.y1 * sH + t.x0 * sW, go * (wx0 * wy1 * wz0));
    atomicAdd(base + t.z0 * sD + t.y1 * sH + t.x1 * sW, go * (wx1 * wy1 * wz0));
    atomicAdd(base + t.z1 * sD + t.y0 * sH + t.x0 * sW, go * (wx0 * wy0 * wz1));
    atomicAdd(base + t.z1 * sD + t.y0 * sH + t.x1 * sW, go * (wx1 * wy0 * wz1));
    atomicAdd(base + t.z1 * sD + t.y1 * sH + t.x0 * sW, go * (wx0 * wy1 * wz1));
    atomicAdd(base + t.z1 * sD + t.y1 * sH + t.x1 * sW, go * (wx1 * wy1 * wz1));
  }
}

typedef unsigned u32;

struct Tap32 {
  u32 o000, o001, o010, o011, o100, o101, o110, o111;
  float tx, ty, tz, mx, my, mz;
};

__device__ __forceinline__ void axis_tap(float g, int size, u32 stride, u32& o0, u32& d1, float& t, float& m) {
  float p;
  unnormalize_clip(g, size, p, m);
  if (!(p == p)) p = 0.f;
  const float f = floorf(p);
  t = p - f;
  const int i0 = (int)f;
  o0 = (u32)i0 * stride;
  d1 = (i0 + 1 <= size - 1) ? stride : 0u;
}

__device__ __forceinline__ Tap32 make_tap32(float gx, float gy, float gz, int W, int H, int D, u32 rec_bytes) {
  Tap32 t;
  u32 x0, dx, y0, dy, z0, dz;
  axis_tap(gx, W, rec_bytes, x0, dx, t.tx, t.mx);
  axis_tap(gy, H, rec_bytes * (u32)W, y0, dy, t.ty, t.my);
  axis_tap(gz, D, rec_bytes * (u32)W * (u32)H, z0, dz, t.tz, t.mz);
  const u32 b00 = z0 + y0, b01 = b00 + dy, b10 = b00 + dz, b11 = b01 + dz;
  t.o000 = b00 + x0; t.o001 = t.o000 + dx;
  t.o010 = b01 + x0; t.o011 = t.o010 + dx;
  t.o100 = b10 + x0; t.o101 = t.o100 + dx;
  t.o110 = b11 + x0; t.o111 = t.o110 + dx;
  return t;
}

__device__ __forceinline__ f32x4 ldrec(__amdgpu_buffer_rsrc_t rs, u32 off) {
  return __builtin_bit_cast(f32x4, __builtin_amdgcn_raw_buffer_load_b128(rs, (int)off, 0, 0));
}

typedef unsigned u32x2_t __attribute__((ext_vector_type(2)));
template <bool B16>
__device__ __forceinline__ f32x4 ldrec_t(__amdgpu_buffer_rsrc_t rs, u32 off) {
  if constexpr (B16)
    return __builtin_convertvector(__builtin_bit_cast(bf16x4r, __builtin_amdgcn_raw_buffer_load_b64(rs, (int)off, 0, 0)), f32x4);
  else
    return __builtin_bit_cast(f32x4, __builtin_amdgcn_raw_buffer_load_b128(rs, (int)off, 0, 0));
}

__device__ __forceinline__ float quad_sum4(float v) {
  const float a = v + __int_as_float(__builtin_amdgcn_update_dpp(0, __float_as_int(v), 0xB1, 0xF, 0xF, true));
  return a + __int_as_float(__builtin_amdgcn_update_dpp(0, __float_as_int(a), 0x4E, 0xF, 0xF, true));
}

__device__ __forceinline__ long vol_offset(int n, long vol_bstride, const int* __restrict__ vol_idx, int vol_n) {
  const int v = vol_idx[n];
  return (long)(v < 0 ? 0 : (v >= vol_n ? vol_n - 1 : v)) * vol_bstride;
}

#define GATHER_KERNEL(stem) stem##_kernel
#define GATHER_TABLE_PARAMS
#define GATHER_VOL_OFFSET ((long)n * vol_bstride)
#include "resample_gather.inc"
#undef GATHER_KERNEL
#undef GATHER_TABLE_PARAMS
#undef GATHER_VOL_OFFSET
#define GATHER_KERNEL(stem) stem##_indexed_kernel
#define GATHER_TABLE_PARAMS const int* __restrict__ vol_idx, int vol_n,
#define GATHER_VOL_OFFSET vol_offset(n, vol_bstride, vol_idx, vol_n)
#include "resample_gather.inc"
#undef GATHER_KERNEL
#undef GATHER_TABLE_PARAMS
#undef GATHER_VOL_OFFSET

template <int KIND>
__global__ void __launch_bounds__(256) resample_fwd_c16_dedup_kernel(
    const float* __restrict__ vol, long vol_bstride, const float* __restrict__ coef,
    float* __restrict__ out, int D, int H, int W, int nbx, int nby, int nbz, Steps st) {
  __shared__ u32x4_t tapo[4][64];
  __shared__ f32x4 tapf[4][64];
  const int lane = threadIdx.x & 63, wave = threadIdx.x >> 6;
  const int n = blockIdx.z / nbz, bz = blockIdx.z - n * nbz;
  const int x0 = ((blockIdx.x << 2) + wave) << 2, y0 = blockIdx.y << 2, z0 = bz << 2;
  const u32 sample_bytes = (u32)D * (u32)H * (u32)W * 64u;
  const __amdgpu_buffer_rsrc_t rs = __builtin_amdgcn_make_buffer_rsrc((void*)(vol + (long)n * vol_bstride), 0, sample_bytes, 0x00020000);
  const __amdgpu_buffer_rsrc_t ro = __builtin_amdgcn_make_buffer_rsrc((void*)(out + (long)n * D * H * W * 16), 0, sample_bytes, 0x00020000);
  const float* cf = coef + n * LF_MAP_COEFS;
  {
    const int x = x0 + (lane & 3), y = y0 + ((lane >> 2) & 3), z = z0 + (lane >> 4);
    const bool live = x < W && y < H && z < D;
    float gx, gy, gz, a, b, k;
    eval_grid<KIND>(cf, live ? x : 0, live ? y : 0, live ? z : 0, W, H, D, st, gx, gy, gz, a, b, k);
    const Tap32 t = make_tap32(gx, gy, gz, W, H, D, 64u);
    u32x4_t o;
    o[0] = live ? t.o000 : 0xffffffffu;
    o[1] = t.o001 - t.o000; o[2] = t.o010 - t.o000; o[3] = t.o100 - t.o000;
    tapo[wave][lane] = o;
    tapf[wave][lane] = (f32x4){t.tx, t.ty, t.tz, 0.f};
  }
  asm volatile("s_waitcnt lgkmcnt(0)" ::: "memory");
  const int q = lane & 3, vq = lane >> 2;
  const u32 co = (u32)q * 16u;
#pragma unroll
  for (int i = 0; i < 4; ++i) {
    const int vi = 16 * i + vq;
    const u32x4_t o = tapo[wave][vi];
    const f32x4 f = tapf[wave][vi];
    if (o[0] == 0xffffffffu) continue;
    const u32 b00 = o[0] + co, b01 = b00 + o[2], b10 = b00 + o[3], b11 = b01 + o[3];
    const f32x4 v000 = ldrec(rs, b00), v001 = ldrec(rs, b00 + o[1]), v010 = ldrec(rs, b01), v011 = ldrec(rs, b01 + o[1]);
    const f32x4 v100 = ldrec(rs, b10), v101 = ldrec(rs, b10 + o[1]), v110 = ldrec(rs, b11), v111 = ldrec(rs, b11 + o[1]);
    const float wx1 = f[0], wx0 = 1.f - f[0], wy1 = f[1], wy0 = 1.f - f[1], wz1 = f[2], wz0 = 1.f - f[2];
    const float w000 = wx0 * wy0 * wz0, w001 = wx1 * wy0 * wz0, w010 = wx0 * wy1 * wz0, w011 = wx1 * wy1 * wz0;
    const float w100 = wx0 * wy0 * wz1, w101 = wx1 * wy0 * wz1, w110 = wx0 * wy1 * wz1, w111 = wx1 * wy1 * wz1;
    f32x4 r;
#pragma unroll
    for (int e = 0; e < 4; ++e) {
      float acc = v000[e] * w000;
      asm("v_fmac_f32 %0, %1, %2" : "+v"(acc) : "v"(v001[e]), "v"(w001));
      asm("v_fmac_f32 %0, %1, %2" : "+v"(acc) : "v"(v010[e]), "v"(w010));
      asm("v_fmac_f32 %0, %1, %2" : "+v"(acc) : "v"(v011[e]), "v"(w011));
      asm("v_fmac_f32 %0, %1, %2" : "+v"(acc) : "v"(v100[e]), "v"(w100));
      asm("v_fmac_f32 %0, %1, %2" : "+v"(acc) : "v"(v101[e]), "v"(w101));
      asm("v_fmac_f32 %0, %1, %2" : "+v"(acc) : "v"(v110[e]), "v"(w110));
      asm("v_fmac_f32 %0, %1, %2" : "+v"(acc) : "v"(v111[e]), "v"(w111));
      r[e] = acc;
    }
    const int x = x0 + (vi & 3), y = y0 + ((vi >> 2) & 3), z = z0 + (vi >> 4);
    __builtin_amdgcn_raw_buffer_store_b128(__builtin_bit_cast(u32x4_t, r), ro, (int)((u32)((z * H + y) * W + x) * 64u + co), 0, 2);
  }
}

#include "resample_staged.inc"

#ifdef STAGED_TPW_OVERRIDE
constexpr int STAGED_TPW = STAGED_TPW_OVERRIDE;
#else
constexpr int STAGED_TPW = 16;
#endif

int g_bwd_coef_variant = 10;
int g_resample_variant = 3;

}

struct FwdPlan {
  bool vec;
  int lpt, tlx, tly, tlz, nbz;
  dim3 grid;
  Steps st;
};
static int fwd_plan(const float* vol, const float* out, int N, int D, int H, int W, int C, FwdPlan& p) {
  if ((long)D * H * W >= 0x7fffffffL) return LF_EINVAL;
  p.vec = (C % 4 == 0) && lf_aligned16(vol) && lf_aligned16(out);
  const int lpv = p.vec ? C / 4 : C;
  p.lpt = lpv < 256 ? lpv : 256;
  int lg = 0;
  while ((2 << lg) * p.lpt <= 256) ++lg;
  if (lg >= 6) { p.tlx = (lg + 2) / 3; p.tly = (lg + 1) / 3; p.tlz = lg / 3; }
  else         { p.tlx = lg < 2 ? lg : 2; p.tly = lg - p.tlx < 2 ? lg - p.tlx : 2; p.tlz = lg - p.tlx - p.tly; }
  p.nbz = (D + (1 << p.tlz) - 1) >> p.tlz;
  const int nby = (H + (1 << p.tly) - 1) >> p.tly;
  if ((long)p.nbz * N > 65535 || nby > 65535) return LF_EINVAL;
  p.grid = dim3((unsigned)((W + (1 << p.tlx) - 1) >> p.tlx), (unsigned)nby, (unsigned)(p.nbz * N));
  p.st = make_steps(D, H, W);
  return 0;
}

extern "C" int lf_resample3d_fwd(const float* vol, int vol_n, const float* coef, int kind, float* out,
                                 int N, int D, int H, int W, int C, void* stream) {
  lf_clear_error();
  if (N <= 0 || D <= 0 || H <= 0 || W <= 0 || C <= 0) return LF_EINVAL;
  if (vol_n != 1 && vol_n != N) return LF_EINVAL;
  if (kind != LF_MAP_O2C && kind != LF_MAP_C2O) return LF_EINVAL;
  const long bstride = vol_n == 1 ? 0 : (long)D * H * W * C;
  FwdPlan p;
  if (int e = fwd_plan(vol, out, N, D, H, W, C, p)) return e;
  hipStream_t s = (hipStream_t)stream;
  if (g_resample_variant == 4 && p.vec && C == 16 && (long)D * H * W * 64 < 0xffffffffL && W <= 65535) {
    const int ntx = (W + LT_X - 1) / LT_X, nty = (H + LT_Y - 1) / LT_Y, ntz = (D + LT_Z - 1) / LT_Z;
    const long nwg = (long)ntx * nty * ntz * N;
    if (nwg > 0x7fffffffL) return LF_EINVAL;
    LAUNCH_BY_KIND(resample_fwd_staged_kernel, dim3((unsigned)nwg), vol, bstride, coef, out, D, H, W, ntx, nty, ntz, p.st);
    return lf_launch_status();
  }
  if (g_resample_variant == 5 && p.vec && C == 16 && (long)D * H * W * 64 < 0xffffffffL) {
    const int nbz4 = (D + 3) >> 2, nbx16 = (W + 15) >> 4, nby4 = (H + 3) >> 2;
    if ((long)nbz4 * N > 65535 || nby4 > 65535) return LF_EINVAL;
    dim3 g5((unsigned)nbx16, (unsigned)nby4, (unsigned)(nbz4 * N));
    LAUNCH_BY_KIND(resample_fwd_c16_dedup_kernel, g5, vol, bstride, coef, out, D, H, W, nbx16, nby4, nbz4, p.st);
    return lf_launch_status();
  }
  if (g_resample_variant >= 3 && p.vec && C == 16 && (long)D * H * W * 64 < 0xffffffffL) {
    LAUNCH_BY_KIND(resample_fwd_c16_kernel, p.grid, vol, bstride, coef, out, D, H, W, p.nbz, p.st);
  } else if (g_resample_variant >= 2 && p.vec && (long)D * H * W * C * 4 < 0xffffffffL) {
    LAUNCH_BY_KIND(resample_fwd_lean_kernel, p.grid, vol, bstride, coef, out, D, H, W, C, p.lpt, p.tlx, p.tly, p.tlz, p.nbz, p.st);
  } else {
#define LAUNCH(K, V) hipLaunchKernelGGL((resample_fwd_kernel<K, V>), p.grid, dim3(256), 0, s, vol, bstride, coef, out, N, D, H, W, C, p.lpt, p.tlx, p.tly, p.tlz, p.nbz, p.st)
    if (kind == LF_MAP_O2C) { if (p.vec) LAUNCH(LF_MAP_O2C, 4); else LAUNCH(LF_MAP_O2C, 1); }
    else                    { if (p.vec) LAUNCH(LF_MAP_C2O, 4); else LAUNCH(LF_MAP_C2O, 1); }
#undef LAUNCH
  }
  return lf_launch_status();
}

static long staged_bwd_blocks(int D, int H, int W) {
  const long nt = (long)((W + LT_X - 1) / LT_X) * ((H + LT_Y - 1) / LT_Y) * ((D + LT_Z - 1) / LT_Z);
  return (nt + STAGED_TPW - 1) / STAGED_TPW;
}

static size_t bwd_coef_scratch_bytes(int N, int part_n, int D, int H, int W) {
  const long nvox = (long)D * H * W;
  const int vpb = bwd_vox_per_block(nvox, part_n);
  const BwdTile bt = bwd_tile(vpb, D, H, W);
  const long nblk = (long)bt.ntx * bt.nty * bt.ntz;
  const long nblk_staged = staged_bwd_blocks(D, H, W);
  return (size_t)N * (nblk > nblk_staged ? nblk : nblk_staged) * 18 * sizeof(float);
}

extern "C" size_t lf_resample3d_bwd_coef_scratch_bytes(int N, int D, int H, int W) {
  return bwd_coef_scratch_bytes(N, N, D, H, W);
}

extern "C" size_t lf_resample3d_bwd_coef_part_scratch_bytes(int N, int part_n, int D, int H, int W) {
  if (N <= 0 || part_n <= 0) return 0;
  return bwd_coef_scratch_bytes(N, part_n, D, H, W);
}

struct BwdCoefPlan {
  long nvox;
  int vpb, nblk, lpv;
  BwdTile bt;
  bool vec;
  dim3 grid;
  Steps st;
};
static int bwd_coef_plan(const float* gout, const float* vol, size_t scratch_bytes, int N, int part_n, int D, int H, int W, int C,
                         BwdCoefPlan& p) {
  if (scratch_bytes < bwd_coef_scratch_bytes(N, part_n, D, H, W)) return LF_ENOSPC;
  if ((long)D * H * W >= 0x7fffffffL) return LF_EINVAL;
  p.nvox = (long)D * H * W;
  p.vpb = bwd_vox_per_block(p.nvox, part_n);
  p.bt = bwd_tile(p.vpb, D, H, W);
  const long nblk_l = (long)p.bt.ntx * p.bt.nty * p.bt.ntz;
  if (nblk_l * N > 0x7fffffffL) return LF_EINVAL;
  p.nblk = (int)nblk_l;
  p.grid = dim3((unsigned)(nblk_l * N));
  p.vec = (C % 4 == 0) && lf_aligned16(gout) && lf_aligned16(vol);
  const int groups = p.vec ? C / 4 : C;
  p.lpv = 1;
  while (p.lpv < groups) p.lpv <<= 1;
  if (p.lpv > 64) return LF_EINVAL;
  p.st = make_steps(D, H, W);
  return 0;
}

static int bwd_coef_finish(const float* partial, int nblk, float* gcoef, int N, hipStream_t s) {
  if (int e = lf_launch_status()) return e;
  hipLaunchKernelGGL(resample_bwd_coef_reduce, dim3(N), dim3(256), 0, s, partial, nblk, gcoef);
  return lf_launch_status();
}

static int bwd_coef_launch(const float* gout, const float* vol, int vol_n, const float* coef,
                           float* gcoef, void* scratch, size_t scratch_bytes,
                           int N, int part_n, int D, int H, int W, int C, void* stream) {
  if (N <= 0 || D <= 0 || H <= 0 || W <= 0 || C <= 0) return LF_EINVAL;
  if (vol_n != 1 && vol_n != N) return LF_EINVAL;
  BwdCoefPlan p;
  if (int e = bwd_coef_plan(gout, vol, scratch_bytes, N, part_n, D, H, W, C, p)) return e;
  const long bstride = vol_n == 1 ? 0 : p.nvox * C;
  hipStream_t s = (hipStream_t)stream;
  float* partial = (float*)scratch;
  if (g_resample_variant == 4 && p.vec && C == 16 && p.nvox * 64 < 0xffffffffL && W <= 65535) {
    const int ntx = (W + LT_X - 1) / LT_X, nty = (H + LT_Y - 1) / LT_Y, ntz = (D + LT_Z - 1) / LT_Z;
    const long nb = staged_bwd_blocks(D, H, W);
    if (nb * N > 0x7fffffffL) return LF_EINVAL;
    hipLaunchKernelGGL((resample_bwd_coef_staged_kernel<STAGED_TPW>), dim3((unsigned)(nb * N)), dim3(256), 0, s, gout, vol, bstride, coef,
                       partial, (int)nb, D, H, W, ntx, nty, ntz, p.st);
    return bwd_coef_finish(partial, (int)nb, gcoef, N, s);
  }
  if (g_resample_variant >= 2 && p.vec && C == 16 && p.vpb >= 64 && p.nvox * 64 < 0xffffffffL) {
    const int v = g_bwd_coef_variant;
    const bool big = p.vpb >= 256;
#define LAUNCH(...) hipLaunchKernelGGL((__VA_ARGS__), p.grid, dim3(256), 0, s, gout, vol, bstride, coef, partial, p.nblk, p.vpb, p.bt, D, H, W, p.st)
    if (v == 1)              LAUNCH(resample_bwd_coef_c16_kernel<1, 1>);
    else if (v == 2)         LAUNCH(resample_bwd_coef_c16_kernel<1, 2>);
    else if (v == 3)         LAUNCH(resample_bwd_coef_c16_kernel<4, 2>);
    else if (v == 6 && big)  LAUNCH(resample_bwd_coef_c16_dedup_kernel<2, 1>);
    else if (v == 7 && big)  LAUNCH(resample_bwd_coef_c16_dedup_kernel<1, 1>);
    else if (v == 8 && big)  LAUNCH(resample_bwd_coef_c16_dedup_kernel<2, 4>);
    else if (v == 9 && big)  LAUNCH(resample_bwd_coef_c16_dedup_kernel<1, 5>);
    else if (v == 10 && big) LAUNCH(resample_bwd_coef_c16_dedup_kernel<2, 1, true>);
    else if (v == 11 && big) LAUNCH(resample_bwd_coef_c16_dedup_kernel<1, 1, true>);
    else if (v == 4)         LAUNCH(resample_bwd_coef_c16_kernel<6, 1>);
    else                     LAUNCH(resample_bwd_coef_c16_kernel<8, 1>);
#undef LAUNCH
  } else if (p.vec) {
    hipLaunchKernelGGL((resample_bwd_coef_kernel<4>), p.grid, dim3(256), 0, s, gout, vol, bstride, coef, partial, p.nblk, p.vpb, p.bt, N, D, H, W, C, p.lpv, p.st);
  } else {
    hipLaunchKernelGGL((resample_bwd_coef_kernel<1>), p.grid, dim3(256), 0, s, gout, vol, bstride, coef, partial, p.nblk, p.vpb, p.bt, N, D, H, W, C, p.lpv, p.st);
  }
  return bwd_coef_finish(partial, p.nblk, gcoef, N, s);
}

extern "C" int lf_resample3d_bwd_coef(const float* gout, const float* vol, int vol_n, const float* coef,
                                      float* gcoef, void* scratch, size_t scratch_bytes,
                                      int N, int D, int H, int W, int C, void* stream) {
  lf_clear_error();
  return bwd_coef_launch(gout, vol, vol_n, coef, gcoef, scratch, scratch_bytes, N, N, D, H, W, C, stream);
}

extern "C" int lf_resample3d_bwd_coef_part(const float* gout, const float* vol, int vol_n, const float* coef,
                                           float* gcoef, void* scratch, size_t scratch_bytes,
                                           int N, int D, int H, int W, int C, int part_n, void* stream) {
  lf_clear_error();
  if (!gout || !vol || !coef || !gcoef || !scratch) return LF_EINVAL;
  if (part_n <= 0 || N <= 0) return LF_EINVAL;
  return bwd_coef_launch(gout, vol, vol_n, coef, gcoef, scratch, scratch_bytes, N, part_n, D, H, W, C, stream);
}

extern "C" int lf_resample3d_fwd_indexed(const float* vol, int vol_n, const int* vol_idx, const float* coef, int kind, float* out,
                                         int N, int D, int H, int W, int C, void* stream) {
  lf_clear_error();
  if (!vol || !vol_idx || !coef || !out) return LF_EINVAL;
  if (N <= 0 || D <= 0 || H <= 0 || W <= 0 || C <= 0 || vol_n < 1) return LF_EINVAL;
  if (kind != LF_MAP_O2C && kind != LF_MAP_C2O) return LF_EINVAL;
  if (((uintptr_t)vol_idx & 3) != 0) return LF_EALIGN;
  const long bstride = (long)D * H * W * C;
  FwdPlan p;
  if (int e = fwd_plan(vol, out, N, D, H, W, C, p)) return e;
  hipStream_t s = (hipStream_t)stream;
  if (g_resample_variant >= 3 && p.vec && C == 16 && (long)D * H * W * 64 < 0xffffffffL) {
    LAUNCH_BY_KIND(resample_fwd_c16_indexed_kernel, p.grid, vol, bstride, vol_idx, vol_n, coef, out, D, H, W, p.nbz, p.st);
  } else if (g_resample_variant >= 2 && p.vec && (long)D * H * W * C * 4 < 0xffffffffL) {
    LAUNCH_BY_KIND(resample_fwd_lean_indexed_kernel, p.grid, vol, bstride, vol_idx, vol_n, coef, out, D, H, W, C, p.lpt, p.tlx, p.tly, p.tlz, p.nbz, p.st);
  } else {
#define LAUNCH(K, V) hipLaunchKernelGGL((resample_fwd_indexed_kernel<K, V>), p.grid, dim3(256), 0, s, vol, bstride, vol_idx, vol_n, coef, out, N, D, H, W, C, p.lpt, p.tlx, p.tly, p.tlz, p.nbz, p.st)
    if (kind == LF_MAP_O2C) { if (p.vec) LAUNCH(LF_MAP_O2C, 4); else LAUNCH(LF_MAP_O2C, 1); }
    else                    { if (p.vec) LAUNCH(LF_MAP_C2O, 4); else LAUNCH(LF_MAP_C2O, 1); }
#undef LAUNCH
  }
  return lf_launch_status();
}

extern "C" size_t lf_resample3d_bwd_coef_indexed_scratch_bytes(int N, int part_n, int D, int H, int W) {
  if (N <= 0 || part_n <= 0) return 0;
  return bwd_coef_scratch_bytes(N, part_n, D, H, W);
}

extern "C" int lf_resample3d_bwd_coef_indexed(const float* gout, const float* vol, int vol_n, const int* vol_idx, const float* coef,
                                              float* gcoef, void* scratch, size_t scratch_bytes,
                                              int N, int D, int H, int W, int C, int part_n, void* stream) {
  lf_clear_error();
  if (!gout || !vol || !vol_idx || !coef || !gcoef || !scratch) return LF_EINVAL;
  if (part_n <= 0 || N <= 0 || vol_n < 1) return LF_EINVAL;
  if (D <= 0 || H <= 0 || W <= 0 || C <= 0) return LF_EINVAL;
  if (((uintptr_t)vol_idx & 3) != 0) return LF_EALIGN;
  BwdCoefPlan p;
  if (int e = bwd_coef_plan(gout, vol, scratch_bytes, N, part_n, D, H, W, C, p)) return e;
  const long bstride = p.nvox * C;
  hipStream_t s = (hipStream_t)stream;
  float* partial = (float*)scratch;
  if (g_resample_variant >= 2 && p.vec && C == 16 && p.vpb >= 64 && p.nvox * 64 < 0xffffffffL) {
    if (p.vpb >= 256)
      hipLaunchKernelGGL((resample_bwd_coef_c16_dedup_indexed_kernel<2, 1, true>), p.grid, dim3(256), 0, s, gout, vol, bstride, vol_idx, vol_n, coef, partial, p.nblk, p.vpb, p.bt, D, H, W, p.st);
    else
      hipLaunchKernelGGL((resample_bwd_coef_c16_indexed_kernel<8, 1>), p.grid, dim3(256), 0, s, gout, vol, bstride, vol_idx, vol_n, coef, partial, p.nblk, p.vpb, p.bt, D, H, W, p.st);
  } else if (p.vec) {
    hipLaunchKernelGGL((resample_bwd_coef_indexed_kernel<4>), p.grid, dim3(256), 0, s, gout, vol, bstride, vol_idx, vol_n, coef, partial, p.nblk, p.vpb, p.bt, N, D, H, W, C, p.lpv, p.st);
  } else {
    hipLaunchKernelGGL((resample_bwd_coef_indexed_kernel<1>), p.grid, dim3(256), 0, s, gout, vol, bstride, vol_idx, vol_n, coef, partial, p.nblk, p.vpb, p.bt, N, D, H, W, C, p.lpv, p.st);
  }
  return bwd_coef_finish(partial, p.nblk, gcoef, N, s);
}

extern "C" int lf_resample3d_bwd_vol(const float* gout, const float* coef, int kind, float* gvol, int vol_n,
                                     int N, int D, int H, int W, int C, void* stream) {
  lf_clear_error();
  if (N <= 0 || D <= 0 || H <= 0 || W <= 0 || C <= 0) return LF_EINVAL;
  if (vol_n != 1 && vol_n != N) return LF_EINVAL;
  const long bstride = vol_n == 1 ? 0 : (long)D * H * W * C;
  const long items = (long)D * H * W * C;
  dim3 grid((unsigned)min((items + 255) / 256, (long)65535 * 16), N), block(256);
  hipStream_t s = (hipStream_t)stream;
  if (kind == LF_MAP_O2C)
    hipLaunchKernelGGL((resample_bwd_vol_kernel<LF_MAP_O2C>), grid, block, 0, s, gout, coef, gvol, bstride, N, D, H, W, C, make_steps(D, H, W));
  else if (kind == LF_MAP_C2O)
    hipLaunchKernelGGL((resample_bwd_vol_kernel<LF_MAP_C2O>), grid, block, 0, s, gout, coef, gvol, bstride, N, D, H, W, C, make_steps(D, H, W));
  else
    return LF_EINVAL;
  return lf_launch_status();
}

#ifdef STAGE_TS
extern "C" int lf_debug_stage_ts(void* dst) {
  return (int)hipMemcpyFromSymbol(dst, HIP_SYMBOL(g_stage_ts), sizeof(unsigned long long) * 256 * 16, 0, hipMemcpyDeviceToHost);
}
#endif

extern "C" int lf_set_tuning(int key, int value) {
  if (key == 1) {
    const int prev = g_resample_variant;
    if (value >= 1 && value <= 5) g_resample_variant = value;
    return prev;
  }
  if (key == 4) return lf_internal_splat_set_variant(value);
  if (key == 6) return lf_internal_splat_set_chunk_cap(value);
  if (key == 3) return lf_internal_fused_set_cfg(value);
  if (key == 7) return lf_internal_wino_set_pack(value);
  if (key == 8) return lf_internal_wino_set_forms(value);
  if (key == 5) return lf_internal_ring_bf16_set_wgs(value);
  if (key == 2) {
    const int prev = g_bwd_coef_variant;
    if (value >= 1 && value <= 11) g_bwd_coef_variant = value;
    return prev;
  }
  return LF_EINVAL;
}

extern "C" int lf_resample3d_fwd_io(const void* vol, int vol_n, const float* coef, int kind, void* out,
                                    int N, int D, int H, int W, int io, void* stream) {
  lf_clear_error();
  if (N <= 0 || D <= 0 || H <= 0 || W <= 0 || io < 0 || io > 3) return LF_EINVAL;
  if ((vol_n != 1 && vol_n != N) || (kind != LF_MAP_O2C && kind != LF_MAP_C2O)) return LF_EINVAL;
  if (!lf_aligned16(vol) || !lf_aligned16(out)) return LF_EALIGN;
  if ((long)D * H * W * 64 >= 0xffffffffL) return LF_EINVAL;
  const long bstride = vol_n == 1 ? 0 : (long)D * H * W * 16;
  const int nbz4 = (D + 3) >> 2;
  if ((long)nbz4 * N > 65535 || ((H + 3) >> 2) > 65535) return LF_EINVAL;
  dim3 g4((unsigned)((W + 3) >> 2), (unsigned)((H + 3) >> 2), (unsigned)(nbz4 * N)), block(256);
  const Steps st = make_steps(D, H, W);
  typedef void (*kern_t)(const float*, long, const float*, float*, int, int, int, int, Steps);
  static const kern_t kerns[2][4] = {
      {resample_fwd_c16_kernel<LF_MAP_O2C, 0>, resample_fwd_c16_kernel<LF_MAP_O2C, 1>, resample_fwd_c16_kernel<LF_MAP_O2C, 2>, resample_fwd_c16_kernel<LF_MAP_O2C, 3>},
      {resample_fwd_c16_kernel<LF_MAP_C2O, 0>, resample_fwd_c16_kernel<LF_MAP_C2O, 1>, resample_fwd_c16_kernel<LF_MAP_C2O, 2>, resample_fwd_c16_kernel<LF_MAP_C2O, 3>}};
  hipLaunchKernelGGL(kerns[kind == LF_MAP_O2C ? 0 : 1][io], g4, block, 0, (hipStream_t)stream, (const float*)vol, bstride, coef, (float*)out, D, H, W, nbz4, st);
  return lf_launch_status();
}
```

### latentfusion_amd/csrc/resample_gather.inc

```

template <int KIND, int VEC>
__global__ void __launch_bounds__(256) GATHER_KERNEL(resample_fwd)(
    const float* __restrict__ vol, long vol_bstride, GATHER_TABLE_PARAMS const float* __restrict__ coef,
    float* __restrict__ out, int N, int D, int H, int W, int C, int lpt, int lx, int ly, int lz, int nbz, Steps st) {
  const int lpv = C / VEC;
  const int n = blockIdx.z / nbz, bz = blockIdx.z - n * nbz;
  const int slot = threadIdx.x / lpt, q0 = threadIdx.x - slot * lpt;
  if (slot >= (1 << (lx + ly + lz))) return;
  const int x = (blockIdx.x << lx) + (slot & ((1 << lx) - 1));
  const int y = (blockIdx.y << ly) + ((slot >> lx) & ((1 << ly) - 1));
  const int z = (bz << lz) + (slot >> (lx + ly));
  if (x >= W || y >= H || z >= D) return;
  const float* cf = coef + (long)n * LF_MAP_COEFS;
  float gx, gy, gz, a, b, k;
  eval_grid<KIND>(cf, x, y, z, W, H, D, st, gx, gy, gz, a, b, k);
  const Tap t = make_tap(gx, gy, gz, W, H, D);
  const float wx1 = t.tx, wx0 = 1.f - t.tx, wy1 = t.ty, wy0 = 1.f - t.ty, wz1 = t.tz, wz0 = 1.f - t.tz;
  const float w000 = wx0 * wy0 * wz0, w001 = wx1 * wy0 * wz0, w010 = wx0 * wy1 * wz0, w011 = wx1 * wy1 * wz0;
  const float w100 = wx0 * wy0 * wz1, w101 = wx1 * wy0 * wz1, w110 = wx0 * wy1 * wz1, w111 = wx1 * wy1 * wz1;
  const int r00 = (t.z0 * H + t.y0) * W, r01 = (t.z0 * H + t.y1) * W;
  const int r10 = (t.z1 * H + t.y0) * W, r11 = (t.z1 * H + t.y1) * W;
  const float* base = vol + GATHER_VOL_OFFSET;
  float* orow = out + ((long)n * D * H * W + ((long)z * H + y) * W + x) * C;
  for (int q = q0; q < lpv; q += lpt) {
    const int co = q * VEC;
    if (VEC == 4) {
      const f32x4 v000 = *(const f32x4*)(base + (long)(r00 + t.x0) * C + co), v001 = *(const f32x4*)(base + (long)(r00 + t.x1) * C + co);
      const f32x4 v010 = *(const f32x4*)(base + (long)(r01 + t.x0) * C + co), v011 = *(const f32x4*)(base + (long)(r01 + t.x1) * C + co);
      const f32x4 v100 = *(const f32x4*)(base + (long)(r10 + t.x0) * C + co), v101 = *(const f32x4*)(base + (long)(r10 + t.x1) * C + co);
      const f32x4 v110 = *(const f32x4*)(base + (long)(r11 + t.x0) * C + co), v111 = *(const f32x4*)(base + (long)(r11 + t.x1) * C + co);
      const f32x4 r = v000 * w000 + v001 * w001 + v010 * w010 + v011 * w011 + v100 * w100 + v101 * w101 + v110 * w110 +
                      v111 * w111;
      __builtin_nontemporal_store(r, (f32x4*)(orow + co));
    } else {
      const float r = base[(long)(r00 + t.x0) * C + co] * w000 + base[(long)(r00 + t.x1) * C + co] * w001 +
                      base[(long)(r01 + t.x0) * C + co] * w010 + base[(long)(r01 + t.x1) * C + co] * w011 +
                      base[(long)(r10 + t.x0) * C + co] * w100 + base[(long)(r10 + t.x1) * C + co] * w101 +
                      base[(long)(r11 + t.x0) * C + co] * w110 + base[(long)(r11 + t.x1) * C + co] * w111;
      orow[co] = r;
    }
  }
}

template <int VEC>
__global__ void __launch_bounds__(256) GATHER_KERNEL(resample_bwd_coef)(
    const float* __restrict__ gout, const float* __restrict__ vol, long vol_bstride, GATHER_TABLE_PARAMS
    const float* __restrict__ coef, float* __restrict__ partial, int nblk, int vpb, BwdTile bt,
    int N, int D, int H, int W, int C, int lpv, Steps st) {
  const unsigned fb = xcd_contiguous(blockIdx.x, gridDim.x);
  const int n = fb / nblk, blk = fb - n * nblk;
  const float* cf = coef + (long)n * LF_MAP_COEFS;
  const int nvox = D * H * W;
  const int tx = blk % bt.ntx, ty = (blk / bt.ntx) % bt.nty, tz = blk / (bt.ntx * bt.nty);
  const int q = threadIdx.x % lpv;
  const int vslot = threadIdx.x / lpv;
  const int vstep = blockDim.x / lpv;
  float acc[18];
#pragma unroll
  for (int i = 0; i < 18; ++i) acc[i] = 0.f;
  const int iters = (vpb + vstep - 1) / vstep;
  for (int it = 0; it < iters; ++it) {
    const int i = it * vstep + vslot;
    const int sub = i >> 6;
    const int sbx = bt.lx - 2, sby = bt.ly - 2;
    const int x = (tx << bt.lx) + ((sub & ((1 << sbx) - 1)) << 2) + (i & 3);
    const int y = (ty << bt.ly) + (((sub >> sbx) & ((1 << sby) - 1)) << 2) + ((i >> 2) & 3);
    const int z = (tz << bt.lz) + ((sub >> (sbx + sby)) << 2) + ((i >> 4) & 3);
    const bool live = i < vpb && x < W && y < H && z < D;
    const int v = (z * H + y) * W + x;
    float hx = 0.f, hy = 0.f, hz = 0.f, a = 0.f, b = 0.f, k = 0.f;
    if (live && q * VEC < C) {
      float gx, gy, gz;
      eval_grid<LF_MAP_O2C>(cf, x, y, z, W, H, D, st, gx, gy, gz, a, b, k);
      const Tap t = make_tap(gx, gy, gz, W, H, D);
      const float* base = vol + GATHER_VOL_OFFSET + (long)q * VEC;
      const float* g = gout + (((long)n * nvox + v) * C) + (long)q * VEC;
      const long o00 = (long)((t.z0 * H + t.y0) * W) * C, o01 = (long)((t.z0 * H + t.y1) * W) * C;
      const long o10 = (long)((t.z1 * H + t.y0) * W) * C, o11 = (long)((t.z1 * H + t.y1) * W) * C;
      const long x0 = (long)t.x0 * C, x1 = (long)t.x1 * C;
      const float wx1 = t.tx, wx0 = 1.f - t.tx, wy1 = t.ty, wy0 = 1.f - t.ty, wz1 = t.tz, wz0 = 1.f - t.tz;
      float dx = 0.f, dy = 0.f, dz = 0.f;
#pragma unroll
      for (int e = 0; e < VEC; ++e) {
        const float go = __builtin_nontemporal_load(g + e);
        const float v000 = base[o00 + x0 + e], v001 = base[o00 + x1 + e];
        const float v010 = base[o01 + x0 + e], v011 = base[o01 + x1 + e];
        const float v100 = base[o10 + x0 + e], v101 = base[o10 + x1 + e];
        const float v110 = base[o11 + x0 + e], v111 = base[o11 + x1 + e];
        dx += go * ((v001 - v000) * (wy0 * wz0) + (v011 - v010) * (wy1 * wz0) +
                    (v101 - v100) * (wy0 * wz1) + (v111 - v110) * (wy1 * wz1));
        dy += go * ((v010 - v000) * (wx0 * wz0) + (v011 - v001) * (wx1 * wz0) +
                    (v110 - v100) * (wx0 * wz1) + (v111 - v101) * (wx1 * wz1));
        dz += go * ((v100 - v000) * (wx0 * wy0) + (v101 - v001) * (wx1 * wy0) +
                    (v110 - v010) * (wx0 * wy1) + (v111 - v011) * (wx1 * wy1));
      }
      hx = dx * t.mx; hy = dy * t.my; hz = dz * t.mz;
    }
    for (int o = lpv >> 1; o > 0; o >>= 1) {
      hx += __shfl_xor(hx, o, 64);
      hy += __shfl_xor(hy, o, 64);
      hz += __shfl_xor(hz, o, 64);
    }
    if (q == 0 && live) {
      const float ak = a * k, bk = b * k;
      acc[0] += hx;       acc[1] += hy;       acc[2] += hz;
      acc[3] += hx * a;   acc[4] += hy * a;   acc[5] += hz * a;
      acc[6] += hx * b;   acc[7] += hy * b;   acc[8] += hz * b;
      acc[9] += hx * k;   acc[10] += hy * k;  acc[11] += hz * k;
      acc[12] += hx * ak; acc[13] += hy * ak; acc[14] += hz * ak;
      acc[15] += hx * bk; acc[16] += hy * bk; acc[17] += hz * bk;
    }
  }
  __shared__ float red[4][18];
  const int wave = threadIdx.x >> 6, lane = threadIdx.x & 63;
#pragma unroll
  for (int i = 0; i < 18; ++i) {
    const float s = lf_wave_sum(acc[i]);
    if (lane == 0) red[wave][i] = s;
  }
  __syncthreads();
  if (threadIdx.x < 18) {
    const float s = (red[0][threadIdx.x] + red[1][threadIdx.x]) + (red[2][threadIdx.x] + red[3][threadIdx.x]);
    partial[((long)n * nblk + blk) * 18 + threadIdx.x] = s;
  }
}

template <int KIND>
__global__ void __launch_bounds__(256) GATHER_KERNEL(resample_fwd_lean)(
    const float* __restrict__ vol, long vol_bstride, GATHER_TABLE_PARAMS const float* __restrict__ coef,
    float* __restrict__ out, int D, int H, int W, int C, int lpt, int lx, int ly, int lz, int nbz, Steps st) {
  const int lpv = C >> 2;
  const int n = blockIdx.z / nbz, bz = blockIdx.z - n * nbz;
  const int slot = threadIdx.x / lpt, q0 = threadIdx.x - slot * lpt;
  if (slot >= (1 << (lx + ly + lz))) return;
  const int x = (blockIdx.x << lx) + (slot & ((1 << lx) - 1));
  const int y = (blockIdx.y << ly) + ((slot >> lx) & ((1 << ly) - 1));
  const int z = (bz << lz) + (slot >> (lx + ly));
  if (x >= W || y >= H || z >= D) return;
  const u32 rec = (u32)C * 4u;
  const u32 sample_bytes = (u32)D * (u32)H * (u32)W * rec;
  const __amdgpu_buffer_rsrc_t rs = __builtin_amdgcn_make_buffer_rsrc((void*)(vol + GATHER_VOL_OFFSET), 0, sample_bytes, 0x00020000);
  const __amdgpu_buffer_rsrc_t ro = __builtin_amdgcn_make_buffer_rsrc((void*)(out + (long)n * D * H * W * C), 0, sample_bytes, 0x00020000);
  const float* cf = coef + n * LF_MAP_COEFS;
  float gx, gy, gz, a, b, k;
  eval_grid<KIND>(cf, x, y, z, W, H, D, st, gx, gy, gz, a, b, k);
  const Tap32 t = make_tap32(gx, gy, gz, W, H, D, rec);
  const float wx1 = t.tx, wx0 = 1.f - t.tx, wy1 = t.ty, wy0 = 1.f - t.ty, wz1 = t.tz, wz0 = 1.f - t.tz;
  const float w000 = wx0 * wy0 * wz0, w001 = wx1 * wy0 * wz0, w010 = wx0 * wy1 * wz0, w011 = wx1 * wy1 * wz0;
  const float w100 = wx0 * wy0 * wz1, w101 = wx1 * wy0 * wz1, w110 = wx0 * wy1 * wz1, w111 = wx1 * wy1 * wz1;
  const u32 orow = (u32)((z * H + y) * W + x) * rec;
  for (int q = q0; q < lpv; q += lpt) {
    const u32 co = (u32)q * 16u;
    const f32x4 v000 = ldrec(rs, t.o000 + co), v001 = ldrec(rs, t.o001 + co), v010 = ldrec(rs, t.o010 + co), v011 = ldrec(rs, t.o011 + co);
    const f32x4 v100 = ldrec(rs, t.o100 + co), v101 = ldrec(rs, t.o101 + co), v110 = ldrec(rs, t.o110 + co), v111 = ldrec(rs, t.o111 + co);
    const f32x4 r = v000 * w000 + v001 * w001 + v010 * w010 + v011 * w011 + v100 * w100 + v101 * w101 + v110 * w110 + v111 * w111;
    __builtin_amdgcn_raw_buffer_store_b128(__builtin_bit_cast(u32x4_t, r), ro, (int)(orow + co), 0, 2);
  }
}

template <int KIND, int IO = 0>
__global__ void __launch_bounds__(256) GATHER_KERNEL(resample_fwd_c16)(
    const float* __restrict__ vol, long vol_bstride, GATHER_TABLE_PARAMS const float* __restrict__ coef,
    float* __restrict__ out, int D, int H, int W, int nbz, Steps st) {
  constexpr bool IN16 = (IO & 1) != 0, OUT16 = (IO & 2) != 0;
  constexpr u32 IREC = IN16 ? 32u : 64u, OREC = OUT16 ? 32u : 64u;
  const int n = blockIdx.z / nbz, bz = blockIdx.z - n * nbz;
  const int q = threadIdx.x & 3, vs = threadIdx.x >> 2;
  const int x = (blockIdx.x << 2) + (vs & 3), y = (blockIdx.y << 2) + ((vs >> 2) & 3), z = (bz << 2) + (vs >> 4);
  if (x >= W || y >= H || z >= D) return;
  const u32 nvox = (u32)D * (u32)H * (u32)W;
  const __amdgpu_buffer_rsrc_t rs = __builtin_amdgcn_make_buffer_rsrc((void*)((const char*)vol + GATHER_VOL_OFFSET * (IN16 ? 2 : 4)), 0, nvox * IREC, 0x00020000);
  const __amdgpu_buffer_rsrc_t ro = __builtin_amdgcn_make_buffer_rsrc((void*)((char*)out + (long)n * nvox * OREC), 0, nvox * OREC, 0x00020000);
  const float* cf = coef + n * LF_MAP_COEFS;
  float gx, gy, gz, a, b, k;
  eval_grid<KIND>(cf, x, y, z, W, H, D, st, gx, gy, gz, a, b, k);
  const Tap32 t = make_tap32(gx, gy, gz, W, H, D, IREC);
  const u32 co = (u32)q * (IREC / 4u);
  const f32x4 v000 = ldrec_t<IN16>(rs, t.o000 + co), v001 = ldrec_t<IN16>(rs, t.o001 + co), v010 = ldrec_t<IN16>(rs, t.o010 + co), v011 = ldrec_t<IN16>(rs, t.o011 + co);
  const f32x4 v100 = ldrec_t<IN16>(rs, t.o100 + co), v101 = ldrec_t<IN16>(rs, t.o101 + co), v110 = ldrec_t<IN16>(rs, t.o110 + co), v111 = ldrec_t<IN16>(rs, t.o111 + co);
  const float wx1 = t.tx, wx0 = 1.f - t.tx, wy1 = t.ty, wy0 = 1.f - t.ty, wz1 = t.tz, wz0 = 1.f - t.tz;
  const float w000 = wx0 * wy0 * wz0, w001 = wx1 * wy0 * wz0, w010 = wx0 * wy1 * wz0, w011 = wx1 * wy1 * wz0;
  const float w100 = wx0 * wy0 * wz1, w101 = wx1 * wy0 * wz1, w110 = wx0 * wy1 * wz1, w111 = wx1 * wy1 * wz1;
  f32x4 r;
#pragma unroll
  for (int e = 0; e < 4; ++e) {
    float acc = v000[e] * w000;
    asm("v_fmac_f32 %0, %1, %2" : "+v"(acc) : "v"(v001[e]), "v"(w001));
    asm("v_fmac_f32 %0, %1, %2" : "+v"(acc) : "v"(v010[e]), "v"(w010));
    asm("v_fmac_f32 %0, %1, %2" : "+v"(acc) : "v"(v011[e]), "v"(w011));
    asm("v_fmac_f32 %0, %1, %2" : "+v"(acc) : "v"(v100[e]), "v"(w100));
    asm("v_fmac_f32 %0, %1, %2" : "+v"(acc) : "v"(v101[e]), "v"(w101));
    asm("v_fmac_f32 %0, %1, %2" : "+v"(acc) : "v"(v110[e]), "v"(w110));
    asm("v_fmac_f32 %0, %1, %2" : "+v"(acc) : "v"(v111[e]), "v"(w111));
    r[e] = acc;
  }
  if constexpr (OUT16)
    __builtin_amdgcn_raw_buffer_store_b64(__builtin_bit_cast(u32x2_t, __builtin_convertvector(r, bf16x4r)), ro,
                                          (int)((u32)((z * H + y) * W + x) * 32u + (u32)q * 8u), 0, 2);
  else
    __builtin_amdgcn_raw_buffer_store_b128(__builtin_bit_cast(u32x4_t, r), ro, (int)((u32)((z * H + y) * W + x) * 64u + (u32)q * 16u), 0, 2);
}

template <int MINW, int UNR>
__global__ void __launch_bounds__(256, MINW) GATHER_KERNEL(resample_bwd_coef_c16)(
    const float* __restrict__ gout, const float* __restrict__ vol, long vol_bstride, GATHER_TABLE_PARAMS
    const float* __restrict__ coef, float* __restrict__ partial, int nblk, int vpb, BwdTile bt,
    int D, int H, int W, Steps st) {
  const unsigned fb = xcd_contiguous(blockIdx.x, gridDim.x);
  const int n = fb / nblk, blk = fb - n * nblk;
  const float* cf = coef + n * LF_MAP_COEFS;
  const u32 rec = 64u;
  const u32 sample_bytes = (u32)D * (u32)H * (u32)W * rec;
  const __amdgpu_buffer_rsrc_t rs = __builtin_amdgcn_make_buffer_rsrc((void*)(vol + GATHER_VOL_OFFSET), 0, sample_bytes, 0x00020000);
  const __amdgpu_buffer_rsrc_t rg = __builtin_amdgcn_make_buffer_rsrc((void*)(gout + (long)n * D * H * W * 16), 0, sample_bytes, 0x00020000);
  const int tx = blk % bt.ntx, ty = (blk / bt.ntx) % bt.nty, tz = blk / (bt.ntx * bt.nty);
  const int q = threadIdx.x & 3, vs = threadIdx.x >> 2;
  const int px = vs & 3, py = (vs >> 2) & 3, pz = vs >> 4;
  const int sbx = bt.lx - 2, sby = bt.ly - 2;
  float acc[6];
#pragma unroll
  for (int i = 0; i < 6; ++i) acc[i] = 0.f;
  const int nsub = vpb >> 6;
  const u32 co = (u32)q * 16u;
  for (int sub0 = 0; sub0 < nsub; sub0 += UNR) {
    Tap32 t[UNR];
    float a[UNR], b[UNR], k[UNR];
    f32x4 go[UNR], v[UNR][8];
#pragma unroll
    for (int u = 0; u < UNR; ++u) {
      const int sub = sub0 + u;
      const int x = (tx << bt.lx) + ((sub & ((1 << sbx) - 1)) << 2) + px;
      const int y = (ty << bt.ly) + (((sub >> sbx) & ((1 << sby) - 1)) << 2) + py;
      const int z = (tz << bt.lz) + ((sub >> (sbx + sby)) << 2) + pz;
      const bool live = sub < nsub && x < W && y < H && z < D;
      float gx, gy, gz;
      eval_grid<LF_MAP_O2C>(cf, live ? x : 0, live ? y : 0, live ? z : 0, W, H, D, st, gx, gy, gz, a[u], b[u], k[u]);
      t[u] = make_tap32(gx, gy, gz, W, H, D, rec);
      const u32 dead = live ? 0u : 0xffffffffu;
      go[u] = __builtin_bit_cast(f32x4, __builtin_amdgcn_raw_buffer_load_b128(
          rg, (int)(((u32)((z * H + y) * W + x) * rec + co) | dead), 0, 2));
      v[u][0] = ldrec(rs, (t[u].o000 + co) | dead); v[u][1] = ldrec(rs, (t[u].o001 + co) | dead);
      v[u][2] = ldrec(rs, (t[u].o010 + co) | dead); v[u][3] = ldrec(rs, (t[u].o011 + co) | dead);
      v[u][4] = ldrec(rs, (t[u].o100 + co) | dead); v[u][5] = ldrec(rs, (t[u].o101 + co) | dead);
      v[u][6] = ldrec(rs, (t[u].o110 + co) | dead); v[u][7] = ldrec(rs, (t[u].o111 + co) | dead);
    }
#pragma unroll
    for (int u = 0; u < UNR; ++u) {
      float p[8];
#pragma unroll
      for (int c8 = 0; c8 < 8; ++c8)
        p[c8] = quad_sum4((go[u][0] * v[u][c8][0] + go[u][1] * v[u][c8][1]) + (go[u][2] * v[u][c8][2] + go[u][3] * v[u][c8][3]));
      const float wx1 = t[u].tx, wx0 = 1.f - wx1, wy1 = t[u].ty, wy0 = 1.f - wy1, wz1 = t[u].tz, wz0 = 1.f - wz1;
      const float dxv = (p[1] - p[0]) * (wy0 * wz0) + (p[3] - p[2]) * (wy1 * wz0) + (p[5] - p[4]) * (wy0 * wz1) + (p[7] - p[6]) * (wy1 * wz1);
      const float dyv = (p[2] - p[0]) * (wx0 * wz0) + (p[3] - p[1]) * (wx1 * wz0) + (p[6] - p[4]) * (wx0 * wz1) + (p[7] - p[5]) * (wx1 * wz1);
      const float dzv = (p[4] - p[0]) * (wx0 * wy0) + (p[5] - p[1]) * (wx1 * wy0) + (p[6] - p[2]) * (wx0 * wy1) + (p[7] - p[3]) * (wx1 * wy1);
      const float hx = dxv * t[u].mx, hy = dyv * t[u].my, hz = dzv * t[u].mz;
      const float B0 = q == 0 ? 1.f : (q == 1 ? b[u] : (q == 2 ? a[u] * k[u] : 0.f));
      const float B1 = q == 0 ? a[u] : (q == 1 ? k[u] : (q == 2 ? b[u] * k[u] : 0.f));
      acc[0] += hx * B0; acc[1] += hy * B0; acc[2] += hz * B0;
      acc[3] += hx * B1; acc[4] += hy * B1; acc[5] += hz * B1;
    }
  }
  __shared__ double red[4][18];
  const int wave = threadIdx.x >> 6, lane = threadIdx.x & 63;
#pragma unroll
  for (int i = 0; i < 6; ++i) {
    double s = (double)acc[i];
#pragma unroll
    for (int o = 32; o >= 4; o >>= 1) s += __shfl_xor(s, o, 64);
    if (lane < 3) red[wave][(2 * lane + i / 3) * 3 + (i % 3)] = s;
  }
  __syncthreads();
  if (threadIdx.x < 18) {
    const double s = (red[0][threadIdx.x] + red[1][threadIdx.x]) + (red[2][threadIdx.x] + red[3][threadIdx.x]);
    partial[((long)n * nblk + blk) * 18 + threadIdx.x] = (float)s;
  }
}

template <int PIF, int MINW, bool GOPF = false>
__global__ void __launch_bounds__(256, MINW) GATHER_KERNEL(resample_bwd_coef_c16_dedup)(
    const float* __restrict__ gout, const float* __restrict__ vol, long vol_bstride, GATHER_TABLE_PARAMS
    const float* __restrict__ coef, float* __restrict__ partial, int nblk, int vpb, BwdTile bt,
    int D, int H, int W, Steps st) {
  __shared__ u32x4_t tapbuf[4][64];
  __shared__ float pbuf[4][64 * 8];
  __shared__ double red[4][18];
  const unsigned fb = xcd_contiguous(blockIdx.x, gridDim.x);
  const int n = fb / nblk, blk = fb - n * nblk;
  const float* cf = coef + n * LF_MAP_COEFS;
  const u32 rec = 64u;
  const u32 sample_bytes = (u32)D * (u32)H * (u32)W * rec;
  const __amdgpu_buffer_rsrc_t rs = __builtin_amdgcn_make_buffer_rsrc((void*)(vol + GATHER_VOL_OFFSET), 0, sample_bytes, 0x00020000);
  const __amdgpu_buffer_rsrc_t rg = __builtin_amdgcn_make_buffer_rsrc((void*)(gout + (long)n * D * H * W * 16), 0, sample_bytes, 0x00020000);
  const int tx = blk % bt.ntx, ty = (blk / bt.ntx) % bt.nty, tz = blk / (bt.ntx * bt.nty);
  const int lane = threadIdx.x & 63, wave = threadIdx.x >> 6;
  const int px = lane & 3, py = (lane >> 2) & 3, pz = lane >> 4;
  const int q = lane & 3, vq = lane >> 2;
  const int sbx = bt.lx - 2, sby = bt.ly - 2;
  const int nsub = vpb >> 6;
  const u32 co = (u32)q * 16u;
  float acc[18];
#pragma unroll
  for (int i = 0; i < 18; ++i) acc[i] = 0.f;
  u32x4_t* tb = tapbuf[wave];
  float* pb = pbuf[wave];
  f32x4 gnext[4];
  auto load_go = [&](int sub_, f32x4 (&dst)[4]) {
    const int bx0 = (tx << bt.lx) + ((sub_ & ((1 << sbx) - 1)) << 2);
    const int by0 = (ty << bt.ly) + (((sub_ >> sbx) & ((1 << sby) - 1)) << 2);
    const int bz0 = (tz << bt.lz) + ((sub_ >> (sbx + sby)) << 2);
#pragma unroll
    for (int i = 0; i < 4; ++i) {
      const int vi = 16 * i + vq;
      const int vx = bx0 + (vi & 3), vy = by0 + ((vi >> 2) & 3), vz = bz0 + (vi >> 4);
      const u32 dead = (sub_ < nsub && vx < W && vy < H && vz < D) ? 0u : 0xffffffffu;
      dst[i] = __builtin_bit_cast(f32x4, __builtin_amdgcn_raw_buffer_load_b128(
          rg, (int)(((u32)((vz * H + vy) * W + vx) * rec + co) | dead), 0, 2));
    }
  };
  if (GOPF) load_go(wave, gnext);
  for (int sub = wave; sub < nsub; sub += 4) {
    const int x0 = (tx << bt.lx) + ((sub & ((1 << sbx) - 1)) << 2);
    const int y0 = (ty << bt.ly) + (((sub >> sbx) & ((1 << sby) - 1)) << 2);
    const int z0 = (tz << bt.lz) + ((sub >> (sbx + sby)) << 2);
    f32x4 gcur[4];
    if (GOPF) {
#pragma unroll
      for (int i = 0; i < 4; ++i) gcur[i] = gnext[i];
      load_go(sub + 4, gnext);
    }
    const int x = x0 + px, y = y0 + py, z = z0 + pz;
    const bool live = x < W && y < H && z < D;
    float gx, gy, gz, a, b, k;
    eval_grid<LF_MAP_O2C>(cf, live ? x : 0, live ? y : 0, live ? z : 0, W, H, D, st, gx, gy, gz, a, b, k);
    u32 ox, dx, oy, dy, oz, dz;
    float tx_, ty_, tz_, mx, my, mz;
    axis_tap(gx, W, rec, ox, dx, tx_, mx);
    axis_tap(gy, H, rec * (u32)W, oy, dy, ty_, my);
    axis_tap(gz, D, rec * (u32)W * (u32)H, oz, dz, tz_, mz);
    u32x4_t tr;
    tr[0] = live ? (oz + oy + ox) : 0xffffffffu;
    tr[1] = live ? dx : 0u; tr[2] = live ? dy : 0u; tr[3] = live ? dz : 0u;
    tb[lane] = tr;
    asm volatile("s_waitcnt lgkmcnt(0)" ::: "memory");
#pragma unroll 1
    for (int i0 = 0; i0 < 4; i0 += (GOPF ? 4 : PIF)) {
      if (GOPF) {
#pragma unroll
        for (int j0 = 0; j0 < 4; j0 += PIF) {
          f32x4 v[PIF][8];
#pragma unroll
          for (int u = 0; u < PIF; ++u) {
            const u32x4_t t = tb[16 * (j0 + u) + vq];
            const u32 dead = t[0] == 0xffffffffu ? 0xffffffffu : 0u;
            const u32 b00 = (t[0] + co) | dead, b01 = b00 + t[2], b10 = b00 + t[3], b11 = b01 + t[3];
            v[u][0] = ldrec(rs, b00); v[u][1] = ldrec(rs, b00 + t[1]);
            v[u][2] = ldrec(rs, b01); v[u][3] = ldrec(rs, b01 + t[1]);
            v[u][4] = ldrec(rs, b10); v[u][5] = ldrec(rs, b10 + t[1]);
            v[u][6] = ldrec(rs, b11); v[u][7] = ldrec(rs, b11 + t[1]);
          }
#pragma unroll
          for (int u = 0; u < PIF; ++u) {
            const f32x4 go = gcur[j0 + u];
            float p[8];
#pragma unroll
            for (int c8 = 0; c8 < 8; ++c8)
              p[c8] = quad_sum4((go[0] * v[u][c8][0] + go[1] * v[u][c8][1]) + (go[2] * v[u][c8][2] + go[3] * v[u][c8][3]));
            const float e0 = q == 0 ? p[0] : (q == 1 ? p[2] : (q == 2 ? p[4] : p[6]));
            const float e1 = q == 0 ? p[1] : (q == 1 ? p[3] : (q == 2 ? p[5] : p[7]));
            *(float2*)(pb + (16 * (j0 + u) + vq) * 8 + 2 * q) = make_float2(e0, e1);
          }
          __builtin_amdgcn_sched_barrier(0);
        }
        continue;
      }
      f32x4 go[PIF], v[PIF][8];
#pragma unroll
      for (int u = 0; u < PIF; ++u) {
        const int vi = 16 * (i0 + u) + vq;
        const u32x4_t t = tb[vi];
        const int vx = x0 + (vi & 3), vy = y0 + ((vi >> 2) & 3), vz = z0 + (vi >> 4);
        const u32 dead = t[0] == 0xffffffffu ? 0xffffffffu : 0u;
        go[u] = __builtin_bit_cast(f32x4, __builtin_amdgcn_raw_buffer_load_b128(
            rg, (int)(((u32)((vz * H + vy) * W + vx) * rec + co) | dead), 0, 2));
        const u32 b00 = (t[0] + co) | dead, b01 = b00 + t[2], b10 = b00 + t[3], b11 = b01 + t[3];
        v[u][0] = ldrec(rs, b00); v[u][1] = ldrec(rs, b00 + t[1]);
        v[u][2] = ldrec(rs, b01); v[u][3] = ldrec(rs, b01 + t[1]);
        v[u][4] = ldrec(rs, b10); v[u][5] = ldrec(rs, b10 + t[1]);
        v[u][6] = ldrec(rs, b11); v[u][7] = ldrec(rs, b11 + t[1]);
      }
#pragma unroll
      for (int u = 0; u < PIF; ++u) {
        float p[8];
#pragma unroll
        for (int c8 = 0; c8 < 8; ++c8)
          p[c8] = quad_sum4((go[u][0] * v[u][c8][0] + go[u][1] * v[u][c8][1]) + (go[u][2] * v[u][c8][2] + go[u][3] * v[u][c8][3]));
        const float e0 = q == 0 ? p[0] : (q == 1 ? p[2] : (q == 2 ? p[4] : p[6]));
        const float e1 = q == 0 ? p[1] : (q == 1 ? p[3] : (q == 2 ? p[5] : p[7]));
        *(float2*)(pb + (16 * (i0 + u) + vq) * 8 + 2 * q) = make_float2(e0, e1);
      }
    }
    asm volatile("s_waitcnt lgkmcnt(0)" ::: "memory");
    {
      const f32x4 pa = *(const f32x4*)(pb + lane * 8), pc = *(const f32x4*)(pb + lane * 8 + 4);
      const float wx1 = tx_, wx0 = 1.f - wx1, wy1 = ty_, wy0 = 1.f - wy1, wz1 = tz_, wz0 = 1.f - wz1;
      const float dxv = (pa[1] - pa[0]) * (wy0 * wz0) + (pa[3] - pa[2]) * (wy1 * wz0) + (pc[1] - pc[0]) * (wy0 * wz1) + (pc[3] - pc[2]) * (wy1 * wz1);
      const float dyv = (pa[2] - pa[0]) * (wx0 * wz0) + (pa[3] - pa[1]) * (wx1 * wz0) + (pc[2] - pc[0]) * (wx0 * wz1) + (pc[3] - pc[1]) * (wx1 * wz1);
      const float dzv = (pc[0] - pa[0]) * (wx0 * wy0) + (pc[1] - pa[1]) * (wx1 * wy0) + (pc[2] - pa[2]) * (wx0 * wy1) + (pc[3] - pa[3]) * (wx1 * wy1);
      const float hx = live ? dxv * mx : 0.f, hy = live ? dyv * my : 0.f, hz = live ? dzv * mz : 0.f;
      const float ak = a * k, bk = b * k;
      acc[0] += hx;       acc[1] += hy;       acc[2] += hz;
      acc[3] += hx * a;   acc[4] += hy * a;   acc[5] += hz * a;
      acc[6] += hx * b;   acc[7] += hy * b;   acc[8] += hz * b;
      acc[9] += hx * k;   acc[10] += hy * k;  acc[11] += hz * k;
      acc[12] += hx * ak; acc[13] += hy * ak; acc[14] += hz * ak;
      acc[15] += hx * bk; acc[16] += hy * bk; acc[17] += hz * bk;
    }
    asm volatile("" ::: "memory");
  }
#pragma unroll
  for (int i = 0; i < 18; ++i) {
    double s = (double)acc[i];
#pragma unroll
    for (int o = 32; o > 0; o >>= 1) s += __shfl_xor(s, o, 64);
    if (lane == 0) red[wave][i] = s;
  }
  __syncthreads();
  if (threadIdx.x < 18) {
    const double s = (red[0][threadIdx.x] + red[1][threadIdx.x]) + (red[2][threadIdx.x] + red[3][threadIdx.x]);
    partial[((long)n * nblk + blk) * 18 + threadIdx.x] = (float)s;
  }
}
```

### latentfusion_amd/engine.py

```python
import collections
import contextlib
import math

import torch

from . import _lib, ops
from ._lib import LF_EPI_LRELU, LF_EPI_PIXELNORM, LF_MAP_O2C, check

NCOEF = 24
NPAR = 10


def _s():
    return torch.cuda.current_stream().cuda_stream


class _CameraCoefs(torch.autograd.Function):

    @staticmethod
    def forward(ctx, params, intr, cube, z_span, h, w):
        L = _lib.lib()
        n = params.shape[0]
        coefs = torch.empty(n, NCOEF, device=params.device, dtype=torch.float32)
        jac = torch.empty(n, NCOEF, NPAR, device=params.device, dtype=torch.float32)
# ... 119 lines not shown
    def __init__(self, convs, z):
        super().__init__(convs, z)
        self.packs = [(ops.pack_conv3x3(w), ops.pack_conv3x3(w, transpose=True)) for w in self.w]
        self.folds_prev = _block_kinds([tuple(w.shape[:2]) for w in self.w], z.shape[1])[0]

    def forward(self, li, x, flags, depth_inner=False):
        return ops._conv3x3_raw(x, self.packs[li][0], self.bias[li], self.w[li].shape[0], self.he[li], flags, True)

    def data_grad(self, i, g, acts, norms, flags, bounds):
        if self.folds_prev:
            return ops.conv3x3_bwd_data(g, self.packs[i][1], self.w[i].shape[1], self.he[i], _prev(i, acts, norms, flags))
        gpre = ops._epilogue_bwd(g, acts[i + 1], norms[i], flags)
        return ops._conv3x3_raw(gpre, self.packs[i][1], None, self.w[i].shape[1], self.he[i], 0, False)[0]


class _Winograd16(_CameraBlocks):
    folds_prev = wino16 = True

    def __init__(self, convs, z):
        super().__init__(convs, z)
        self.packs = [(ops.pack_conv3d_c16_wino(w), ops.pack_conv3d_c16_wino(w, transpose=True)) for w in self.w]
        self.rider = None

    def ride_projection(self, proj_pack, proj_bias, proj_he):
        self.rider = (proj_pack, proj_bias, proj_he)

    def forward(self, li, x, flags, depth_inner=False):
        if self.rider is not None and li == len(self.w) - 1:
            return ops.conv3d_c16_wino_projfwd(x, self.packs[li][0], self.bias[li], self.he[li], flags, *self.rider, flags)
        return ops.conv3d_c16_wino(x, self.packs[li][0], self.bias[li], self.he[li], flags)

    def data_grad(self, i, g, acts, norms, flags, bounds):
        return ops.conv3d_c16_wino(g, self.packs[i][1], None, self.he[i], 0, prev=_prev(i, acts, norms, flags))[0]


class _Direct16F16x3(_CameraBlocks):
    folds_prev = plain_factor_only = True
    _pack, _conv = staticmethod(ops.pack_conv3d_c16_split), staticmethod(ops.conv3d_c16_split)

    def __init__(self, convs, z):
        super().__init__(convs, z)
        self.packs = [(self._pack(w), self._pack(w, transpose=True)) for w in self.w]
        self.x0_bound = None

    def grad_bounds(self):
        return ops.amax_buffer(None, self.dev, rows=len(self.w) + 1)

    def forward(self, li, x, flags, depth_inner=False):
        return self._conv(x, self.packs[li][0], self.bias[li], self.he[li], flags, amax_in=self.x0_bound if li == 0 else None)

    def data_grad(self, i, g, acts, norms, flags, bounds):
        return self._conv(g, self.packs[i][1], None, self.he[i], 0, prev=_prev(i, acts, norms, flags), amax_in=bounds[i + 1],
                          amax_out=bounds[i])[0]


class _WideWinograd(_CameraBlocks):
    wide = True
    part_n = None

    def forward(self, li, x, flags, depth_inner=False):
        return ops.wide_conv(x, self.w[li], self.bias[li], self.he[li], flags, depth_inner=depth_inner, part_n=self.part_n)

    def data_grad(self, i, g, acts, norms, flags, bounds):
        gpre = ops._epilogue_bwd(g, acts[i + 1], norms[i], flags)
        return ops.wide_conv(gpre, self.w[i], None, self.he[i], 0, transpose=True, part_n=self.part_n)[0]


class _WideWinogradF16x3(_CameraBlocks):
    wide = plain_factor_only = True

    def __init__(self, convs, z):
        super().__init__(convs, z)
        self.x_bound = [ops.amax_buffer(z.abs().amax(), self.dev)] + [
            ops.amax_buffer(torch.tensor(math.sqrt(w.shape[1])), self.dev) for w in self.w[1:]]
        for w in self.w:
            ops._pk(w, 'wxf', lambda w_: ops.pack_conv_wino_fused_f16x3(w_))
            ops._pk(w, 'wxb', lambda w_: ops.pack_conv_wino_fused_f16x3(w_, transpose=True))

    def forward(self, li, x, flags, depth_inner=False):
        return ops.wide_conv_f16x3(x, self.w[li], self.bias[li], self.he[li], flags, depth_inner=depth_inner, amax_in=self.x_bound[li])

    def data_grad(self, i, g, acts, norms, flags, bounds):
        amax = ops.amax_buffer(None, self.dev)
        gpre = ops.epilogue_bwd_amax(g, acts[i + 1], norms[i], flags, amax)
        return ops.wide_conv_f16x3(gpre, self.w[i], None, self.he[i], 0, transpose=True, amax_in=amax)[0]


CONV_MODES = ('auto', 'fp32', 'winograd', 'f16x3')


def _block_kinds(shapes, C):
    c16 = C == 16 and len(shapes) > 0 and all(tuple(sh) == (16, 16) for sh in shapes)
    wide = len(shapes) > 0 and all(co >= 64 and ci >= 64 and co % 4 == 0 and ci % 4 == 0 for co, ci in shapes)
    return c16, wide


def select_camera_blocks(conv_mode, shapes, C):
    if conv_mode not in CONV_MODES:
        raise ValueError(conv_mode)
    c16, wide = _block_kinds(shapes, C)
    if conv_mode == 'auto':
        conv_mode = 'winograd' if (c16 or wide) else 'fp32'
    if conv_mode == 'f16x3' and not (c16 or wide):
        raise NotImplementedError('f16x3 mode is implemented for 16->16 and wide (>= 64 channel) camera blocks')
    if conv_mode == 'winograd' and not (c16 or wide):
        raise NotImplementedError('winograd mode needs 16->16 or wide (>= 64 channel) camera blocks')
    if conv_mode == 'fp32':
        return conv_mode, _Fp32Direct
    if conv_mode == 'winograd':
        return conv_mode, _Winograd16 if c16 else _WideWinograd
    return conv_mode, _Direct16F16x3 if c16 else _WideWinogradF16x3


PROJ_KERNELS = ('library', 'mfma')


def select_proj_kernel(proj_kernel, default, K, cout):
    if proj_kernel is None:
        proj_kernel = default
    if proj_kernel not in PROJ_KERNELS:
        raise ValueError(f'proj_kernel {proj_kernel!r}: one of {PROJ_KERNELS}')
    if proj_kernel == 'mfma':
        if K is None or cout is None:
            raise NotImplementedError("proj_kernel 'mfma' needs the 'factor' projection")
        if not (K >= 4 and K % 4 == 0 and 16 <= cout <= 256 and cout % 4 == 0):
            raise NotImplementedError(f"proj_kernel 'mfma': lf_rows_gemm_epi takes K % 4 == 0 and 16 <= Cout <= 256, Cout % 4 == 0; "
                                      f'this projection is K = {K}, Cout = {cout}')
    return proj_kernel


LATENT_KERNELS = ('autograd', 'fused')


def select_latent_kernel(latent_kernel, default):
    if latent_kernel is None:
        latent_kernel = default
    if latent_kernel not in LATENT_KERNELS:
        raise ValueError(f'latent_kernel {latent_kernel!r}: one of {LATENT_KERNELS}')
    return latent_kernel


_Tail = collections.namedtuple('_Tail', 'zp pnorm feat leaf occ_saved lat', defaults=(None,))


class RenderLoopEngine:

    LOSS_KEYS = ('depth', 'ov_depth', 'iou', 'mask')
    EXPLICIT_DECODER = True
    EXPLICIT_OCCLUSION = True
    PROJ_GEMM = True
    PROJ_KERNEL = 'library'
    LATENT_KERNEL = 'autograd'

    @staticmethod
    def supports(photographer, loss_weights):
        return (photographer.projection_type in ('factor', 'sum')
                and not photographer.skip_connections
                and all(b.interpolate is None for b in photographer.camera_blocks)
                and photographer.predict_depth and photographer.predict_mask and not photographer.predict_color
                and photographer.camera_config[-1] % 4 == 0)

    CONV_MODES = CONV_MODES
    FUSE_FORMS = ('fwd',)
    _select_blocks = staticmethod(select_camera_blocks)

    def __init__(self, photographer, z_obj, target_obs, loss_weights, conv_mode='auto', fuse_projection=None, proj_kernel=None,
                 latent_kernel=None):
        self.ph = photographer
        self.cube = photographer.cube_size
        dev = z_obj.device
        self.z = self._resident_volume(photographer, z_obj)
        self.S = self.z.shape[-1]
        self.C = self.z.shape[1]
        self.crop = photographer.out_size
        self.tdepth = target_obs.depth.reshape(-1).float().to(dev).contiguous()
        self.tmask = target_obs.mask.reshape(-1).float().to(dev).contiguous()
        self.H, self.W = target_obs.depth.shape[-2:]
        self.set_weights(loss_weights)
        convs = [conv for blk in photographer.camera_blocks for conv in (blk.conv1, blk.conv2)]
        self.nconv = len(convs)
        self.conv_mode, family = self._select_blocks(conv_mode, [tuple(c.module.weight.shape[:2]) for c in convs], self.C)
        self.generic_tail = photographer.projection_type != 'factor' or photographer.occlusion_module is not None
        if self.generic_tail and family.plain_factor_only:
            raise NotImplementedError("the split-precision conv modes drive the plain 'factor' renderer only")
        self.plan = family(convs, self.z)
        C, D = (convs[-1].module.weight.shape[0] if convs else self.C), self.S
        self.Cl = C
        self.occ = None
        if photographer.occlusion_module is not None and self.plan.wino16 and C == 16 and RenderLoopEngine.EXPLICIT_OCCLUSION:
            self.occ = self._plan_occlusion(photographer.occlusion_module)
        cout, pw = C, None
        self.proj = None
        factor = photographer.projection_type == 'factor'
        self.proj_kernel = select_proj_kernel(proj_kernel, self.PROJ_KERNEL, D * C if factor else None,
                                              photographer.projection_block.conv.module.weight.shape[0] if factor else None)
        self.latent_kernel = select_latent_kernel(latent_kernel, self.LATENT_KERNEL)
        self.proj_rows_pack = None
        if factor:
            pw = photographer.projection_block.conv.module.weight
            cout = pw.shape[0]
            self.proj_rows_t = pw.detach().reshape(cout, C, D).permute(2, 1, 0).reshape(D * C, cout).contiguous()
            self.proj = (pw, photographer.projection_block.conv.bias, ops.he_constant(pw),
                         ops.pack_conv1x1(pw.reshape(cout, C, D).permute(0, 2, 1).reshape(cout, D * C)),
                         ops.pack_conv1x1(pw.reshape(cout, C, D).permute(2, 1, 0).reshape(D * C, cout)))
        can_fuse = self.plan.wino16 and cout == 16 and C == 16 and not self.generic_tail
        if fuse_projection is None:
            fuse_projection = ('fwd',) if can_fuse else ()
        elif fuse_projection is False:
            fuse_projection = ()
        elif fuse_projection is True:
            fuse_projection = self.FUSE_FORMS
        if any(f not in self.FUSE_FORMS for f in fuse_projection):
            raise ValueError(f'fuse_projection {fuse_projection!r}: this engine fuses {self.FUSE_FORMS}')
        if fuse_projection and not can_fuse:
            raise NotImplementedError("fuse_projection needs conv_mode 'winograd' on 16-channel blocks and a 16-channel projection")
        self.fuse_projection = tuple(fuse_projection)
        self.proj_fused = None
        if self.fuse_projection:
            wdm = pw.reshape(cout, C, D).permute(0, 2, 1).reshape(cout, D * C)
            self.proj_fused = (ops.pack_wino_proj(wdm), ops.pack_wino_proj(wdm, transpose=True))
        if 'fwd' in self.fuse_projection:
            self.plan.ride_projection(self.proj_fused[0], self.proj[1], self.proj[2])
        self._wide_factor = self.plan.wide and not self.generic_tail
        if self.proj_kernel == 'mfma' and self._wide_factor:
            self.proj_rows_pack = ops.pack_rows_gemm(pw.detach().reshape(cout, C, D).permute(0, 2, 1).reshape(cout, D * C))
        self.dev = dev
        self._params = list(photographer.parameters())
        self._intr = None
        self.heads = None
        obs = list(photographer.output_blocks)
        if len(obs) > 1 and all(getattr(ob, 'activation', None) is None and getattr(ob.conv, 'kernel_size', 0) == 1
                                and ob.conv.bias is not None for ob in obs):
            self.heads = (torch.cat([ob.conv.module.weight.detach() for ob in obs], dim=0).contiguous(),
                          torch.cat([ob.conv.bias.detach() for ob in obs], dim=0).contiguous())
        self.dec = None
        dec = photographer.image_decoder
        blocks2d = list(dec.down_blocks) + list(dec.up_blocks)
        plain = (dec.input_block is None and dec.output_block is None and self.heads is not None
                 and (not self.generic_tail or (self.occ is not None and photographer.projection_type == 'factor'))
                 and (len(dec.up_blocks) < 2 or len(dec.down_blocks) < 2)
                 and all(getattr(b, 'interpolate', True) is None for b in blocks2d) and len(blocks2d) > 0
                 and all(c.module.weight.dim() == 4 and tuple(c.module.weight.shape[2:]) == (3, 3) and c.module.weight.shape[0] <= 64
                         for b in blocks2d for c in (b.conv1, b.conv2)))
        if plain and RenderLoopEngine.EXPLICIT_DECODER:
            self.dec = []
            for blk in blocks2d:
                for conv in (blk.conv1, blk.conv2):
                    w = conv.module.weight
                    self.dec.append((w, conv.bias, ops.he_constant(w), ops.pack_conv3x3(w), ops.pack_conv3x3(w, transpose=True)))
            hw = self.heads[0]
            self.heads_pack = (ops.he_constant(hw), ops.pack_conv1x1(hw.reshape(hw.shape[0], hw.shape[1])),
                               ops.pack_conv1x1(hw.reshape(hw.shape[0], hw.shape[1]).t()))

    @staticmethod
    def _resident_volume(photographer, z_obj):
        z = ops.cl(z_obj.reshape(1, *z_obj.shape[-4:]))
        if len(photographer.object_blocks):
            with torch.no_grad():
                zo = z
                for blk in photographer.object_blocks:
                    zo = blk(zo)
            z = ops.cl(zo.detach())
        return z

    def set_weights(self, loss_weights):
        self.weights = torch.tensor([loss_weights.get(k, 0.0) for k in self.LOSS_KEYS], dtype=torch.float32,
                                    device=self.z.device)
        self.w_latent = float(loss_weights.get('latent', 0.0))

    def forward_backward(self, camera, need_grad=True, z_target_latent=None, params=None, masked_depth=False):
        if masked_depth and need_grad:
            raise ValueError('masked_depth is the forward-only loss form of the ranking estimators (no gradient is defined here)')
        if self.w_latent != 0.0 and z_target_latent is None:
            raise ValueError("the loss weights carry a 'latent' term: pass z_target_latent (LatentFusionModel.compute_latent_code)")
        params = (camera_params(camera) if params is None else params).detach().contiguous()
        K = camera.intrinsic
        if self._intr is None or self._intr[0] is not K or self._intr[1] != K._version:
            self._intr = (K, K._version, camera_intrinsics(camera))
        intr = self._intr[2]
        n = params.shape[0]
        zt = z_target_latent if (z_target_latent is not None and self.w_latent != 0.0) else None
        if zt is not None and zt.shape[0] == 1 and n > 1:
            zt = zt.expand(n, *zt.shape[1:])
        with _frozen(self._params):
            return self._run(params, intr, float(camera.z_span), need_grad, zt, masked_depth)

    def _run(self, params, intr, z_span, need_grad, zt, masked_depth):
        return self._forward_backward_group(params, intr, z_span, need_grad, 1.0, zt, masked_depth)

    @staticmethod
    def _plan_occlusion(om):
        from .modules.blocks import OutputBlock
        blocks = list(om.down_blocks) + list(om.up_blocks)
        ib, ob = om.input_block, om.output_block
        if (ib is None or not isinstance(ob, OutputBlock) or ob.activation is not None or len(om.down_blocks) != 1
                or len(om.up_blocks) != 1 or any(b.interpolate is not None for b in blocks)):
            return None
        w1, wo = ib.conv.module.weight, ob.conv.module.weight
        convs = [c for b in blocks for c in (b.conv1, b.conv2)]
        shapes = [tuple(c.module.weight.shape) for c in convs]
        if (tuple(w1.shape) != (17, 17, 1, 1, 1) or tuple(wo.shape) != (1, 16, 1, 1, 1) or shapes[0] != (16, 17, 3, 3, 3)
                or any(sh != (16, 16, 3, 3, 3) for sh in shapes[1:]) or ib.conv.bias is None or ob.conv.bias is None):
            return None
        dev = w1.device
        wi = torch.zeros(17, 20, device=dev, dtype=torch.float32)
        wi[:, :17] = w1.detach().reshape(17, 17) * ops.he_constant(w1)
        bi = torch.zeros(20, device=dev, dtype=torch.float32)
        bi[:17] = ib.conv.bias.detach()
        w2 = convs[0].module.weight.detach()
        w2a = w2[:, :16].contiguous()
        he2 = ops.he_constant(w2)
        w27 = (w2[:, 16].reshape(16, 27).t() * he2).float().contiguous()
        pk = ops.pack_conv3d_c16_wino
        first = (convs[0].bias, he2, pk(w2a), pk(w2a, transpose=True), w27)
        rest = [(c.bias, ops.he_constant(c.module.weight), pk(c.module.weight), pk(c.module.weight, transpose=True)) for c in convs[1:]]
        wo2 = wo.detach().reshape(1, 16)
        head = (ob.conv.bias, ops.he_constant(wo), ops.pack_conv1x1(wo2))
        return dict(wi=wi.contiguous(), bi=bi, first=first, rest=rest, head=head, head_w16=wo2.reshape(16).float().contiguous())

    def _occlusion_fwd(self, zc, flags):
        L = _lib.lib()
        o, s, dev = self.occ, _s(), self.dev
        n, _, D, H, W = zc.shape
        P = H * W
        ta, t16 = ops.empty_cl(zc.shape, dev), torch.empty(n, 1, D, H, W, device=dev, dtype=torch.float32)
        with ops._timed('occ_input_fwd'):
            check(L.lf_occ_input_fwd(zc.data_ptr(), o['wi'].data_ptr(), o['bi'].data_ptr(), ta.data_ptr(), t16.data_ptr(), n, D, P,
                                     ops.SLOPE, s), 'lf_occ_input_fwd')
        b2, he2, pa, _pat, w27 = o['first']
        pre = ops.empty_cl(zc.shape, dev)
        with ops._timed('occ_conv17_fwd'):
            check(L.lf_occ_conv17_fwd(t16.data_ptr(), w27.data_ptr(), pre.data_ptr(), n, D, H, W, s), 'lf_occ_conv17_fwd')
        y, nrm = ops.conv3d_c16_wino(ta, pa, b2, he2, flags, prev=(pre, None, _lib.LF_EPI_ADD), out=pre)
        ys, ns = [y], [nrm]
        for (b, he, pk, _pkt) in o['rest']:
            y, nrm = ops.conv3d_c16_wino(ys[-1], pk, b, he, flags)
            ys.append(y)
            ns.append(nrm)
        hb, hhe, hpk = o['head']
        wocc = torch.empty(n, 1, D, H, W, device=dev, dtype=torch.float32)
        if D <= 256:
            with ops._timed('column_softmax_head'):
                check(L.lf_column_softmax_head_fwd(ys[-1].data_ptr(), o['head_w16'].data_ptr(), hb.data_ptr() if hb is not None else None,
                                                   hhe, wocc.data_ptr(), None, n, D, P, s), 'lf_column_softmax_head_fwd')
        else:
            logits = torch.empty(n, 1, D, H, W, device=dev, dtype=torch.float32)
            ops._conv1x1_raw(ys[-1], hpk, hb, n, D * P, 16, 1, D * P * 16, 0, 1, logits, hhe, 0)
            with ops._timed('column_softmax'):
                check(L.lf_column_softmax_fwd(logits.data_ptr(), wocc.data_ptr(), None, n, D, P, s), 'lf_column_softmax_fwd')
        if self.proj is not None:
            return None, (ta, t16, ys, ns, wocc)
        zs = ops.empty_cl(zc.shape, dev)
        check(L.lf_column_scale_fwd(zc.data_ptr(), wocc.data_ptr(), zs.data_ptr(), n * D * P, 16, s), 'lf_column_scale_fwd')
        return zs, (ta, t16, ys, ns, wocc)

    def _occlusion_bwd(self, g_zs, zc, saved, flags, prev, proj_bwd=None):
        L = _lib.lib()
        o, s, dev = self.occ, _s(), self.dev
        ta, t16, ys, ns, wocc = saved
        n, _, D, H, W = zc.shape
        P = H * W
        gl = torch.empty_like(wocc)
        if proj_bwd is not None and D <= 256:
            with ops._timed('occ_weight_grad_softmax_bwd'):
                check(L.lf_occ_weight_grad_softmax_bwd(zc.data_ptr(), proj_bwd[0].data_ptr(), proj_bwd[1].data_ptr(), proj_bwd[2], wocc.data_ptr(),
                                                       gl.data_ptr(), n, D, P, s), 'lf_occ_weight_grad_softmax_bwd')
        else:
            gw = torch.empty_like(wocc)
            if proj_bwd is not None:
                check(L.lf_occ_weight_grad(zc.data_ptr(), proj_bwd[0].data_ptr(), proj_bwd[1].data_ptr(), proj_bwd[2], gw.data_ptr(), n, D, P, s),
                      'lf_occ_weight_grad')
            else:
                check(L.lf_column_scale_bwd(g_zs.data_ptr(), zc.data_ptr(), wocc.data_ptr(), None, gw.data_ptr(), n * D * P, 16, s),
                      'lf_column_scale_bwd')
            check(L.lf_column_softmax_bwd(wocc.data_ptr(), gw.data_ptr(), None, gl.data_ptr(), n, D, P, s), 'lf_column_softmax_bwd')
        hhe = o['head'][1]
        g = ops.empty_cl(zc.shape, dev)
        with ops._timed('occ_head_bwd'):
            check(L.lf_occ_head_bwd(gl.data_ptr(), o['head_w16'].data_ptr(), hhe, ys[-1].data_ptr(), ns[-1].data_ptr(), flags, ops.SLOPE,
                                    g.data_ptr(), n * D * P, s), 'lf_occ_head_bwd')
        for i in range(len(o['rest']) - 1, -1, -1):
            _b, he, _pk, pkt = o['rest'][i]
            g = ops.conv3d_c16_wino(g, pkt, None, he, 0, prev=(ys[i], ns[i], flags))[0]
        _b2, he2, _pa, pat, w27 = o['first']
        gp16 = torch.empty_like(t16)
        gta = ops.conv3d_c16_wino(g, pat, None, he2, 0, prev=(ta, None, LF_EPI_LRELU))[0]
        with ops._timed('occ_conv17_bwd'):
            check(L.lf_occ_conv17_bwd(g.data_ptr(), t16.data_ptr(), w27.data_ptr(), gp16.data_ptr(), n, D, H, W, ops.SLOPE, s),
                  'lf_occ_conv17_bwd')
        gz = ops.empty_cl(zc.shape, dev)
        if proj_bwd is not None:
            gp2d, ppack_t, phe = proj_bwd
            with ops._timed('occ_input_bwd'):
                check(L.lf_occ_input_bwd_proj(gta.data_ptr(), gp16.data_ptr(), o['wi'].data_ptr(), gp2d.data_ptr(), ppack_t.data_ptr(), phe,
                                              wocc.data_ptr(), gz.data_ptr(), n, D, P, ops.SLOPE, zc.data_ptr(), prev[1].data_ptr(), prev[2], s),
                      'lf_occ_input_bwd_proj')
            return gz
        with ops._timed('occ_input_bwd'):
            check(L.lf_occ_input_bwd(gta.data_ptr(), None, gp16.data_ptr(), o['wi'].data_ptr(), g_zs.data_ptr(),
                                     wocc.data_ptr(), gz.data_ptr(), n * D * P, ops.SLOPE, zc.data_ptr(), prev[1].data_ptr(), prev[2], s),
                  'lf_occ_input_bwd')
        return gz

    def _forward_backward_group(self, params, intr, z_span, need_grad, grad_scale, zt=None, masked_depth=False):
        n = params.shape[0]
        flags = LF_EPI_LRELU | LF_EPI_PIXELNORM
        coefs, jac, cf20 = self._coefficients(params, intr, z_span, n)
        proj_gemm = self.PROJ_GEMM and self._wide_factor and not need_grad
        acts, norms, rode = self._blocks_fwd(self._resample(cf20, n), flags, proj_gemm)
        tail = self._tail_fwd(acts[-1], rode, flags, need_grad, proj_gemm, n)
        fused_lat = zt is not None and self.latent_kernel == 'fused' and tail.pnorm is not None
        latent_grad = zt is not None and need_grad and not fused_lat
        explicit = self.dec is not None and not latent_grad
        if explicit:
            dacts, dnorms, logits = self._decoder_fwd(tail.zp, tail.pnorm, flags, n)
        else:
            logits = self._decoder_autograd(tail.feat, need_grad)
        if latent_grad:
            cf_leaf = coefs.detach().requires_grad_(True)
            with torch.enable_grad():
                total, losses = self._loss_autograd(logits, cf_leaf)
                lat = self._latent_distance(tail.feat, zt, n)
                total = total + self.w_latent * lat
                losses = losses.clone()
                losses[:, 5] = lat.detach()
                losses[:, 4] += self.w_latent * lat.detach()
                objective = self._objective(total)
            g_leaf, g_cf = torch.autograd.grad(objective, [tail.leaf, cf_leaf])
            gp = None
        else:
            lg = ops.cl(logits.detach())
            losses, gsums, scratch = self._loss_fwd(lg, coefs, masked_depth)
            if fused_lat:
                zt = zt.to(device=self.dev, dtype=torch.float32)
                lat_sums = ops.latent_cosine_fwd(tail.zp, zt, losses, self.w_latent)
                if need_grad:
                    tail = tail._replace(lat=(zt, lat_sums, self.w_latent / self._mean_rows(n)))
            if not need_grad:
                if zt is not None and not fused_lat:
                    lat = self._latent_distance(tail.zp, zt, n)
                    losses[:, 5] = lat
                    losses[:, 4] += self.w_latent * lat
                return losses, None
            glogits = torch.empty_like(lg)
            g_cf = torch.empty(n, NCOEF, device=self.dev, dtype=torch.float32)
            self._loss_bwd(lg, coefs, gsums, glogits, g_cf, scratch)
            if explicit and fused_lat:
                gp, g_leaf = None, self._decoder_bwd(glogits, dacts, dnorms, flags, n, fold_first=False)
            elif explicit:
                gp, g_leaf = self._decoder_bwd(glogits, dacts, dnorms, flags, n), None
            else:
                gp, (g_leaf,) = None, torch.autograd.grad(logits, [tail.leaf], grad_outputs=[glogits])
        g, first, bounds = self._tail_bwd(tail, gp, g_leaf, acts, norms, flags, n)
        for i in range(first, -1, -1):
            g = self.plan.data_grad(i, g, acts, norms, flags, bounds)
        return self._finish_backward(g, g_cf, cf20, jac, n, grad_scale, losses)

    def _coefficients(self, params, intr, z_span, n):
        L = _lib.lib()
        params = params.contiguous()
        intr = intr.contiguous()
        coefs = torch.empty(n, NCOEF, device=self.dev, dtype=torch.float32)
        jac = torch.empty(n, NCOEF, NPAR, device=self.dev, dtype=torch.float32)
        check(L.lf_camera_coefs(params.data_ptr(), intr.data_ptr(), float(self.cube), z_span, self.crop,
                                self.crop, coefs.data_ptr(), jac.data_ptr(), n, _s()), 'lf_camera_coefs')
        cf20 = torch.empty(n, 20, device=self.dev, dtype=torch.float32)
        cf20[:, :18] = coefs[:, :18]
        return coefs, jac, cf20

    def _resample(self, cf20, n):
        L = _lib.lib()
        S = self.S
        x0 = ops.empty_cl((n, self.C, S, S, S), self.dev)
        with ops._timed('resample_fwd'):
            check(L.lf_resample3d_fwd(self.z.data_ptr(), 1, cf20.data_ptr(), LF_MAP_O2C, x0.data_ptr(), n, S, S, S, self.C, _s()),
                  'lf_resample3d_fwd')
        return x0

    def _blocks_fwd(self, x0, flags, proj_gemm):
        acts, norms, rode = [x0], [], []
        last = self.nconv - 1
        for li in range(self.nconv):
            y, nrm, *rode = self.plan.forward(li, acts[-1], flags, depth_inner=proj_gemm and li == last)
            acts.append(y)
            norms.append(nrm)
        return acts, norms, rode

    def _tail_fwd(self, act, rode, flags, need_grad, proj_gemm, n):
        if self.occ is not None:
            return self._occlusion_tail_fwd(act, flags, need_grad, n)
        if self.generic_tail:
            return self._module_tail_fwd(act, need_grad)
        return self._factor_fwd(act, rode, flags, need_grad, proj_gemm, n)

    def _tail_bwd(self, tail, gp, g_leaf, acts, norms, flags, n):
        if self.occ is not None:
            return self._occlusion_tail_bwd(tail, gp, g_leaf, acts, norms, flags, n)
        if self.generic_tail:
            return self._module_tail_bwd(tail, g_leaf, acts, norms, flags)
        return self._factor_bwd(tail, gp, g_leaf, acts, norms, flags, n)

    def _proj_pre_grad(self, tail, gp, g_leaf, flags):
        if tail.lat is not None:
            zt, lat_sums, gscale = tail.lat
            return ops.latent_cosine_bwd_epi(ops.cl(g_leaf), tail.zp, tail.pnorm, zt, lat_sums, gscale, flags)
        return gp if gp is not None else ops._epilogue_bwd(ops.cl(g_leaf), tail.zp, tail.pnorm, flags)

    def _factor_fwd(self, act, rode, flags, need_grad, proj_gemm, n):
        L = _lib.lib()
        pw, pb, phe, ppack, _ppack_t = self.proj
        cout, S, Cl = pw.shape[0], self.S, self.Cl
        if rode:
            zp, pnorm = rode
        elif proj_gemm and self.proj_kernel == 'mfma':
            rows, pnorm = ops.rows_gemm_epilogue(act.view(n * S * S, S * Cl), self.proj_rows_pack, pb, phe, cout, flags,
                                                 tag='factor_project_fwd')
            zp = rows.view(n, S, S, cout).permute(0, 3, 1, 2)
        elif proj_gemm:
            with ops._timed('factor_project_fwd'):
                x2 = act.view(n * S * S, S * Cl)
                if pb is not None:
                    rows = torch.addmm(pb.detach(), x2, self.proj_rows_t, alpha=phe)
                else:
                    rows = torch.mm(x2, self.proj_rows_t).mul_(phe)
                torch.nn.functional.leaky_relu_(rows, ops.SLOPE)
                pnorm = torch.empty(n * S * S, device=self.dev, dtype=torch.float32)
                check(L.lf_pixelnorm_fwd(rows.data_ptr(), rows.data_ptr(), pnorm.data_ptr(), n * S * S, cout, ops.PN_EPS, _s()), 'lf_pixelnorm_fwd')
            zp = rows.view(n, S, S, cout).permute(0, 3, 1, 2)
        else:
            zp = ops.empty_cl((n, cout, S, S), self.dev)
            with ops._timed('factor_project_fwd'):
                pnorm = ops._conv1x1_raw(act, ppack, pb, n, S * S, Cl, S, S * S * S * Cl, S * S * Cl, cout, zp, phe, flags)
        leaf = zp.detach().requires_grad_(need_grad)
        return _Tail(zp, pnorm, leaf, leaf, None)

    def _factor_bwd(self, tail, gp, g_leaf, acts, norms, flags, n):
        L = _lib.lib()
        pw, _pb, phe, _ppack, ppack_t = self.proj
        cout, S, Cl, nconv = pw.shape[0], self.S, self.Cl, self.nconv
        gp = self._proj_pre_grad(tail, gp, g_leaf, flags)
        fused = self._proj_bwd_fused(gp, acts, norms, flags) if self.plan.folds_prev else None
        if fused is not None:
            return fused + (None,)
        g = ops.empty_cl((n, Cl, S, S, S), self.dev)
        bounds = self.plan.grad_bounds()
        if self.plan.folds_prev:
            with ops._timed('factor_project_bwd'):
                check(L.lf_conv1x1_bwd_data(gp.data_ptr(), ppack_t.data_ptr(), g.data_ptr(), n, S * S, cout, S * Cl,
                                            S * S * S * Cl, Cl, Cl, S * S * Cl, phe, acts[nconv].data_ptr(),
                                            norms[nconv - 1].data_ptr(), flags, ops.SLOPE,
                                            bounds[nconv].data_ptr() if bounds is not None else None, _s()), 'lf_conv1x1_bwd_data')
        else:
            ops._conv1x1_raw(gp, ppack_t, None, n, S * S, cout, 1, S * S * cout, 0, S * Cl, g, phe, 0,
                             yaddr=(S * S * S * Cl, Cl, Cl, S * S * Cl))
        return g, nconv - 1, bounds

    def _proj_bwd_fused(self, gp, acts, norms, flags):
        return None

    def _occlusion_tail_fwd(self, act, flags, need_grad, n):
        zs, occ_saved = self._occlusion_fwd(act, flags)
        if self.proj is None:
            leaf = zs.detach().requires_grad_(need_grad)
            with torch.set_grad_enabled(need_grad):
                zp = ops.column_sum(leaf)
            return _Tail(zp, None, zp, leaf, occ_saved)
        pw, pb, phe, ppack, _ppack_t = self.proj
        cout, S, Cl = pw.shape[0], self.S, self.Cl
        zp = ops.empty_cl((n, cout, S, S), self.dev)
        with ops._timed('factor_project_fwd'):
            pnorm = ops._conv1x1_raw(act, ppack, pb, n, S * S, Cl, S, S * S * S * Cl, S * S * Cl, cout, zp, phe, flags,
                                     xscale=occ_saved[4])
        leaf = zp.detach().requires_grad_(need_grad)
        return _Tail(zp, pnorm, leaf, leaf, occ_saved)

    def _occlusion_tail_bwd(self, tail, gp, g_leaf, acts, norms, flags, n):
        S, Cl, nconv = self.S, self.Cl, self.nconv
        proj_bwd = None
        if self.proj is None:
            g_zs = ops.cl(g_leaf)
        else:
            pw, _pb, phe, _ppack, ppack_t = self.proj
            cout = pw.shape[0]
            gp = self._proj_pre_grad(tail, gp, g_leaf, flags)
            with ops._timed('factor_project_bwd'):
                if Cl == 16 and cout == 16 and (S * S) % 16 == 0:
                    g_zs, proj_bwd = None, (gp, ppack_t, phe)
                else:
                    g_zs = ops.empty_cl((n, Cl, S, S, S), self.dev)
                    ops._conv1x1_raw(gp, ppack_t, None, n, S * S, cout, 1, S * S * cout, 0, S * Cl, g_zs, phe, 0,
                                     yaddr=(S * S * S * Cl, Cl, Cl, S * S * Cl))
        g = self._occlusion_bwd(g_zs, acts[-1], tail.occ_saved, flags, (acts[nconv], norms[nconv - 1], flags), proj_bwd)
        return g, nconv - 1, None

    def _module_tail_fwd(self, act, need_grad):
        from .recon.utils import get_normalized_voxel_depth
        leaf = act.detach().requires_grad_(need_grad)
        with torch.set_grad_enabled(need_grad):
            zt_ = leaf
            if self.ph.occlusion_module is not None:
                occ = self.ph.occlusion_module(torch.cat((zt_, get_normalized_voxel_depth(zt_)), dim=1))
                wocc = ops.column_softmax(occ)[0]
                if tuple(occ.shape[-3:]) != tuple(zt_.shape[-3:]):
                    wocc = ops.column_softmax(ops.resize_nearest_to(occ, zt_.size(-1)))[0]
                zt_ = ops.column_scale(zt_, wocc)
            zp = ops.column_sum(zt_) if self.ph.projection_type == 'sum' else self.ph.projection_block(zt_)
        return _Tail(zp, None, zp, leaf, None)

    def _module_tail_bwd(self, tail, g_leaf, acts, norms, flags):
        g = ops.cl(g_leaf)
        if self.plan.folds_prev:
            g = ops._epilogue_bwd(g, acts[self.nconv], norms[self.nconv - 1], flags)
        return g, self.nconv - 1, None

    def _decoder_fwd(self, zp, pnorm, flags, n):
        dacts, dnorms = [zp], [pnorm]
        for (w2, b2, he2, pk2, _pkt2) in self.dec:
            y2, n2 = ops._conv3x3_raw(dacts[-1], pk2, b2, w2.shape[0], he2, flags, True)
            dacts.append(y2)
            dnorms.append(n2)
        hw, hb = self.heads
        hhe, hpk, _hpkt = self.heads_pack
        hh, ww = dacts[-1].shape[-2:]
        logits = ops.empty_cl((n, hw.shape[0], hh, ww), self.dev)
        ops._conv1x1_raw(dacts[-1], hpk, hb, n, hh * ww, hw.shape[1], 1, hh * ww * hw.shape[1], 0, hw.shape[0], logits, hhe, 0)
        return dacts, dnorms, logits

    def _decoder_bwd(self, glogits, dacts, dnorms, flags, n, fold_first=True):
        L = _lib.lib()
        hw = self.heads[0]
        cin_h = hw.shape[1]
        hh, ww = dacts[-1].shape[-2:]
        g2 = ops.empty_cl((n, cin_h, hh, ww), self.dev)
        fuse_h = cin_h == 16
        check(L.lf_conv1x1_bwd_data(glogits.data_ptr(), self.heads_pack[2].data_ptr(), g2.data_ptr(), n, hh * ww, hw.shape[0],
                                    cin_h, hh * ww * cin_h, cin_h, cin_h if fuse_h else (1 << 30), 0, self.heads_pack[0],
                                    dacts[-1].data_ptr() if fuse_h else None, dnorms[-1].data_ptr() if fuse_h else None,
                                    flags if fuse_h else 0, ops.SLOPE, None, _s()), 'lf_conv1x1_bwd_data')
        if not fuse_h:
            g2 = ops._epilogue_bwd(g2, dacts[-1], dnorms[-1], flags)
        for i in range(len(self.dec) - 1, -1, -1):
            w2, _b2, he2, _pk2, pkt2 = self.dec[i]
            cin2 = w2.shape[1]
            if i == 0 and not fold_first:
                g2 = ops.conv3x3_bwd_data(g2, pkt2, cin2, he2, None)
            elif cin2 in (16, 32, 64):
                g2 = ops.conv3x3_bwd_data(g2, pkt2, cin2, he2, (dacts[i], dnorms[i], flags))
            else:
                g2 = ops._epilogue_bwd(ops.conv3x3_bwd_data(g2, pkt2, cin2, he2, None), dacts[i], dnorms[i], flags)
        return g2

    def _decoder_autograd(self, feat, need_grad):
        with torch.set_grad_enabled(need_grad), ops.wide2d_f16x3(self.conv_mode == 'f16x3'):
            yimg, rescale = self.ph.decode_features(feat)
            if self.heads is not None:
                logits = ops.conv1x1(yimg, self.heads[0], self.heads[1])
            else:
                logits = torch.cat([ob(yimg) for ob in self.ph.output_blocks], dim=1)
            return rescale(logits) if rescale is not None else logits

    def _loss_fwd(self, lg, coefs, masked_depth):
        return _pose_loss_fwd(lg, coefs, self.tdepth, self.tmask, self.weights, self.H, self.W, masked_depth)

    def _loss_bwd(self, lg, coefs, gsums, glogits, g_cf, scratch):
        _pose_loss_bwd(lg, coefs, self.tdepth, self.tmask, gsums, glogits, g_cf, scratch, self.H, self.W)

    def _loss_autograd(self, logits, coefs):
        return pose_loss(logits, coefs, self.tdepth, self.tmask, self.weights, self.H, self.W)

    def _objective(self, total):
        return total.mean()

    def _mean_rows(self, n):
        return n

    def _latent_distance(self, zp, zt, n):
        return 1.0 - torch.cosine_similarity(zp.reshape(n, -1), zt.reshape(n, -1).to(zp.dtype), 1, 1e-8)

    def _bwd_coef(self, g, cf20, gcoef18, n):
        L = _lib.lib()
        S = self.S
        nbytes = L.lf_resample3d_bwd_coef_scratch_bytes(n, S, S, S)
        scratch = torch.empty(nbytes // 4 + 1, device=self.dev, dtype=torch.float32)
        with ops._timed('resample_bwd_coef'):
            check(L.lf_resample3d_bwd_coef(g.data_ptr(), self.z.data_ptr(), 1, cf20.data_ptr(), gcoef18.data_ptr(),
                                           scratch.data_ptr(), scratch.numel() * 4, n, S, S, S, self.C, _s()), 'lf_resample3d_bwd_coef')

    def _finish_backward(self, g, g_cf, cf20, jac, n, grad_scale, losses):
        L = _lib.lib()
        dev, s = self.dev, _s()
        gcoef18 = torch.empty(n, 18, device=dev, dtype=torch.float32)
        self._bwd_coef(g, cf20, gcoef18, n)
        gcoefs = g_cf.contiguous()
        gcoefs[:, :18] = gcoef18
        gparams = torch.empty(n, NPAR, device=dev, dtype=torch.float32)
        check(L.lf_camera_coefs_bwd(gcoefs.data_ptr(), jac.data_ptr(), gparams.data_ptr(), n, s), 'lf_camera_coefs_bwd')
        if grad_scale != 1.0:
            gparams *= grad_scale
        return losses, gparams
```

Measured before the change: 197.6.

## Fuse coefficient-gradient reduction and camera chain rule into gather kernel tail

The coefficient-gradient gather kernels get a last-block-ticket tail. The final block of each sample reduces the per-block partials, writes the 24 coefficient gradients, and applies the camera Jacobian to produce the parameter gradients. This removes the separate reduce launch, the slice copy and the camera_coefs_bwd launch. The camera coefficient kernel also writes the padded 20-wide O2C block directly, which drops a torch slice copy. In exchange, partial stores become agent-scope atomic stores, there is a per-sample atomic counter in persistent zeroed scratch, and the final reduction runs serially inside one block.

```diff
diff --git a/include/lf_hip.h b/include/lf_hip.h
--- a/include/lf_hip.h
+++ b/include/lf_hip.h
@@ -38,6 +38,11 @@
 int lf_resample3d_bwd_coef_part(const float* gout, const float* vol, int vol_n, const float* coef,
                                 float* gcoef, void* scratch, size_t scratch_bytes,
                                 int N, int D, int H, int W, int C, int part_n, void* stream);
+#define LF_SCRATCH_TICKET_BYTES 4096
+size_t lf_resample3d_bwd_coef_params_scratch_bytes(int N, int D, int H, int W);
+int lf_resample3d_bwd_coef_params(const float* gout, const float* vol, int vol_n, const float* coef,
+                                  float* gcoefs, const float* jac, float* gparams, void* scratch, size_t scratch_bytes,
+                                  int N, int D, int H, int W, int C, void* stream);
 
 int lf_resample3d_fwd_indexed(const float* vol, int vol_n, const int32_t* vol_idx, const float* coef, int kind,
                               float* out, int N, int D, int H, int W, int C, void* stream);
@@ -308,6 +313,8 @@
 int lf_camera_coefs(const float* params, const float* intrinsics, float cube_size, float z_span,
                     int crop_h, int crop_w, float* coefs, float* jac, int N, void* stream);
 int lf_camera_coefs_bwd(const float* gcoefs, const float* jac, float* gparams, int N, void* stream);
+int lf_camera_coefs_padded(const float* params, const float* intrinsics, float cube_size, float z_span,
+                           int crop_h, int crop_w, float* coefs, float* jac, float* o2c_padded, int N, void* stream);
 
 size_t lf_pose_loss_scratch_bytes(int N, int h, int w, int H, int W);
 int lf_pose_loss_fwd(const float* logits, const float* coefs, const float* target_depth,
diff --git a/latentfusion_amd/_lib.py b/latentfusion_amd/_lib.py
--- a/latentfusion_amd/_lib.py
+++ b/latentfusion_amd/_lib.py
@@ -29,6 +29,8 @@
     'lf_resample3d_bwd_coef': (c_int, [P, P, c_int, P, P, P, c_size_t, c_int, c_int, c_int, c_int, c_int, P]),
     'lf_resample3d_bwd_coef_part_scratch_bytes': (c_size_t, [c_int, c_int, c_int, c_int, c_int]),
     'lf_resample3d_bwd_coef_part': (c_int, [P, P, c_int, P, P, P, c_size_t, c_int, c_int, c_int, c_int, c_int, c_int, P]),
+    'lf_resample3d_bwd_coef_params_scratch_bytes': (c_size_t, [c_int, c_int, c_int, c_int]),
+    'lf_resample3d_bwd_coef_params': (c_int, [P, P, c_int, P, P, P, P, P, c_size_t, c_int, c_int, c_int, c_int, c_int, P]),
     'lf_resample3d_fwd_indexed': (c_int, [P, c_int, P, P, c_int, P, c_int, c_int, c_int, c_int, c_int, P]),
     'lf_resample3d_bwd_coef_indexed_scratch_bytes': (c_size_t, [c_int, c_int, c_int, c_int, c_int]),
     'lf_resample3d_bwd_coef_indexed': (c_int, [P, P, c_int, P, P, P, P, c_size_t, c_int, c_int, c_int, c_int, c_int, c_int, P]),
@@ -155,6 +157,7 @@
     'lf_pose_loss_scratch_bytes': (c_size_t, [c_int, c_int, c_int, c_int, c_int]),
     'lf_pose_loss_fwd': (c_int, [P, P, P, P, P, P, P, P, P, c_size_t, c_int, c_int, c_int, c_int, c_int, P]),
     'lf_pose_loss_bwd': (c_int, [P, P, P, P, P, P, P, P, c_size_t, c_int, c_int, c_int, c_int, c_int, P]),
+    'lf_camera_coefs_padded': (c_int, [P, P, c_float, c_float, c_int, c_int, P, P, P, c_int, P]),
     'lf_pose_loss_fwd_depth': (c_int, [P, P, P, P, P, P, P, P, P, c_size_t, c_int, c_int, c_int, c_int, c_int, P]),
     'lf_pose_loss_bwd_depth': (c_int, [P, P, P, P, P, P, P, P, c_size_t, c_int, c_int, c_int, c_int, c_int, P]),
     'lf_pose_loss_fwd_masked': (c_int, [P, P, P, P, P, P, P, P, c_size_t, c_int, c_int, c_int, c_int, c_int, P]),
diff --git a/latentfusion_amd/csrc/image.hip b/latentfusion_amd/csrc/image.hip
--- a/latentfusion_amd/csrc/image.hip
+++ b/latentfusion_amd/csrc/image.hip
@@ -40,7 +40,7 @@
 template <int ND>
 __global__ void camera_coefs_kernel(const float* __restrict__ params, const float* __restrict__ intr,
                                     float cube, float z_span, int crop_h, int crop_w,
-                                    float* __restrict__ out, float* __restrict__ jac, int N) {
+                                    float* __restrict__ out, float* __restrict__ jac, float* __restrict__ out20, int N) {
   typedef DualT<ND> Dual;
   const int tid = blockIdx.x * blockDim.x + threadIdx.x;
   const int n = ND == 1 ? tid / NP : tid, mine = ND == 1 ? tid % NP : 0;
@@ -93,7 +93,10 @@
   o[22] = dconst((double)z_span + 0.01);
   o[23] = t[2];
   for (int j = 0; j < NOUT; ++j) {
-    if (ND != 1 || mine == 0) out[n * NOUT + j] = (float)o[j].v;
+    if (ND != 1 || mine == 0) {
+      out[n * NOUT + j] = (float)o[j].v;
+      if (out20 != nullptr && j < 18) out20[n * LF_MAP_COEFS + j] = (float)o[j].v;
+    }
     if (ND == 1) jac[(n * NOUT + j) * NP + mine] = (float)o[j].d[0];
     else for (int i = 0; i < ND; ++i) jac[(n * NOUT + j) * NP + i] = (float)o[j].d[i];
   }
@@ -369,13 +372,24 @@
 
 }
 
+static int camera_coefs_launch(const float* params, const float* intrinsics, float cube_size, float z_span,
+                               int crop_h, int crop_w, float* coefs, float* jac, float* o2c_padded, int N, void* stream) {
+  lf_clear_error();
+  if (N <= 0 || crop_h <= 0 || crop_w <= 0 || cube_size <= 0.f) return LF_EINVAL;
+  hipLaunchKernelGGL((camera_coefs_kernel<1>), dim3((N * NP + 63) / 64), dim3(64), 0, (hipStream_t)stream, params, intrinsics,
+                     cube_size, z_span, crop_h, crop_w, coefs, jac, o2c_padded, N);
+  return lf_launch_status();
+}
+
 extern "C" int lf_camera_coefs(const float* params, const float* intrinsics, float cube_size, float z_span,
                                int crop_h, int crop_w, float* coefs, float* jac, int N, void* stream) {
-  lf_clear_error();
-  if (N <= 0 || crop_h <= 0 || crop_w <= 0 || cube_size <= 0.f) return LF_EINVAL;
-  hipLaunchKernelGGL((camera_coefs_kernel<1>), dim3((N * NP + 63) / 64), dim3(64), 0, (hipStream_t)stream, params, intrinsics,
-                     cube_size, z_span, crop_h, crop_w, coefs, jac, N);
-  return lf_launch_status();
+  return camera_coefs_launch(params, intrinsics, cube_size, z_span, crop_h, crop_w, coefs, jac, nullptr, N, stream);
+}
+
+extern "C" int lf_camera_coefs_padded(const float* params, const float* intrinsics, float cube_size, float z_span,
+                                      int crop_h, int crop_w, float* coefs, float* jac, float* o2c_padded, int N, void* stream) {
+  if (!o2c_padded) return LF_EINVAL;
+  return camera_coefs_launch(params, intrinsics, cube_size, z_span, crop_h, crop_w, coefs, jac, o2c_padded, N, stream);
 }
 
 extern "C" int lf_camera_coefs_bwd(const float* gcoefs, const float* jac, float* gparams, int N, void* stream) {
diff --git a/latentfusion_amd/csrc/lf_common.h b/latentfusion_amd/csrc/lf_common.h
--- a/latentfusion_amd/csrc/lf_common.h
+++ b/latentfusion_amd/csrc/lf_common.h
@@ -47,6 +47,24 @@
   return v;
 }
 
+__device__ __forceinline__ void lf_store_coherent(float* p, float v) { __hip_atomic_store(p, v, __ATOMIC_RELAXED, __HIP_MEMORY_SCOPE_AGENT); }
+__device__ __forceinline__ float lf_load_coherent(const float* p) { return __hip_atomic_load(p, __ATOMIC_RELAXED, __HIP_MEMORY_SCOPE_AGENT); }
+__device__ __forceinline__ bool lf_last_block_ticket(unsigned* counter, unsigned nblk) {
+  __shared__ bool last;
+  if (threadIdx.x < LF_WAVE) {
+    asm volatile("s_waitcnt vmcnt(0)" ::: "memory");
+    __builtin_amdgcn_wave_barrier();
+    if (threadIdx.x == 0) {
+      last = atomicAdd(counter, 1u) == nblk - 1u;
+      if (last) atomicExch(counter, 0u);
+    }
+  }
+  __syncthreads();
+  return last;
+}
+#define LF_TICKET_HEADER_BYTES LF_SCRATCH_TICKET_BYTES
+#define LF_TICKET_MAX_SAMPLES (LF_TICKET_HEADER_BYTES / 4)
+
 #define LF_AMAX_SLOTS 64
 #define LF_AMAX_STRIDE 32
 static_assert(LF_AMAX_FLOATS == LF_AMAX_SLOTS * LF_AMAX_STRIDE, "lf_hip.h: LF_AMAX_FLOATS");
diff --git a/latentfusion_amd/csrc/resample.hip b/latentfusion_amd/csrc/resample.hip
--- a/latentfusion_amd/csrc/resample.hip
+++ b/latentfusion_amd/csrc/resample.hip
@@ -83,21 +83,61 @@
   return t;
 }
 
-__global__ void __launch_bounds__(256) resample_bwd_coef_reduce(const float* __restrict__ partial,
-                                                                int nblk, float* __restrict__ gcoef) {
-  const int n = blockIdx.x;
+template <bool COH>
+__device__ __forceinline__ double bwd_coef_reduce_sample(const float* partial, int nblk, int n) {
   __shared__ double red[256];
   const int comp = threadIdx.x % 18;
   const int grp = threadIdx.x / 18;
   double s = 0.0;
   if (grp < 14)
-    for (int b = grp; b < nblk; b += 14) s += (double)partial[((long)n * nblk + b) * 18 + comp];
+    for (int b0 = grp; b0 < nblk; b0 += 14 * 8) {
+      float v[8];
+#pragma unroll
+      for (int u = 0; u < 8; ++u) {
+        const float* src = partial + ((long)n * nblk + b0 + 14 * u) * 18 + comp;
+        v[u] = b0 + 14 * u < nblk ? (COH ? lf_load_coherent(src) : *src) : 0.f;
+      }
+#pragma unroll
+      for (int u = 0; u < 8; ++u)
+        if (b0 + 14 * u < nblk) s += (double)v[u];
+    }
   red[threadIdx.x] = (grp < 14) ? s : 0.0;
   __syncthreads();
+  double tot = 0.0;
+  if (threadIdx.x < 18)
+    for (int g = 0; g < 14; ++g) tot += red[g * 18 + threadIdx.x];
+  return tot;
+}
+
+__global__ void __launch_bounds__(256) resample_bwd_coef_reduce(const float* __restrict__ partial,
+                                                                int nblk, float* __restrict__ gcoef) {
+  const int n = blockIdx.x;
+  const double tot = bwd_coef_reduce_sample<false>(partial, nblk, n);
+  if (threadIdx.x < 18) gcoef[(long)n * 18 + threadIdx.x] = (float)tot;
+}
+
+struct CoefChain {
+  unsigned* tickets;
+  float* gcoefs;
+  const float* jac;
+  float* gparams;
+};
+__device__ __forceinline__ void bwd_coef_chain_tail(const float* partial, int nblk, int n, CoefChain ch) {
+  constexpr int NCOEF = 24, NPAR = 10;
+  if (!lf_last_block_ticket(ch.tickets + n, (unsigned)nblk)) return;
+  __shared__ float grow[NCOEF];
+  const double tot = bwd_coef_reduce_sample<true>(partial, nblk, n);
   if (threadIdx.x < 18) {
-    double tot = 0.0;
-    for (int g = 0; g < 14; ++g) tot += red[g * 18 + threadIdx.x];
-    gcoef[(long)n * 18 + threadIdx.x] = (float)tot;
+    grow[threadIdx.x] = (float)tot;
+    ch.gcoefs[(long)n * NCOEF + threadIdx.x] = (float)tot;
+  } else if (threadIdx.x < NCOEF) {
+    grow[threadIdx.x] = ch.gcoefs[(long)n * NCOEF + threadIdx.x];
+  }
+  __syncthreads();
+  if (threadIdx.x < NPAR) {
+    double s = 0.0;
+    for (int j = 0; j < NCOEF; ++j) s += (double)grow[j] * (double)ch.jac[((long)n * NCOEF + j) * NPAR + threadIdx.x];
+    ch.gparams[(long)n * NPAR + threadIdx.x] = (float)s;
   }
 }
 
@@ -191,6 +231,9 @@
 #define GATHER_KERNEL(stem) stem##_kernel
 #define GATHER_TABLE_PARAMS
 #define GATHER_VOL_OFFSET ((long)n * vol_bstride)
+#define GATHER_CHAIN_PARAMS
+#define GATHER_CHAIN_TAIL
+#define GATHER_PARTIAL_STORE(ptr, val) *(ptr) = val
 #include "resample_gather.inc"
 #undef GATHER_KERNEL
 #undef GATHER_TABLE_PARAMS
@@ -202,6 +245,22 @@
 #undef GATHER_KERNEL
 #undef GATHER_TABLE_PARAMS
 #undef GATHER_VOL_OFFSET
+#undef GATHER_CHAIN_PARAMS
+#undef GATHER_CHAIN_TAIL
+#undef GATHER_PARTIAL_STORE
+#define GATHER_KERNEL(stem) stem##_chain_kernel
+#define GATHER_TABLE_PARAMS
+#define GATHER_VOL_OFFSET ((long)n * vol_bstride)
+#define GATHER_CHAIN_PARAMS , CoefChain chain
+#define GATHER_CHAIN_TAIL bwd_coef_chain_tail(partial, nblk, n, chain);
+#define GATHER_PARTIAL_STORE(ptr, val) lf_store_coherent(ptr, val)
+#include "resample_gather.inc"
+#undef GATHER_KERNEL
+#undef GATHER_TABLE_PARAMS
+#undef GATHER_VOL_OFFSET
+#undef GATHER_CHAIN_PARAMS
+#undef GATHER_CHAIN_TAIL
+#undef GATHER_PARTIAL_STORE
 
 template <int KIND>
 __global__ void __launch_bounds__(256) resample_fwd_c16_dedup_kernel(
@@ -440,6 +499,37 @@
   return bwd_coef_launch(gout, vol, vol_n, coef, gcoef, scratch, scratch_bytes, N, N, D, H, W, C, stream);
 }
 
+extern "C" size_t lf_resample3d_bwd_coef_params_scratch_bytes(int N, int D, int H, int W) {
+  return LF_TICKET_HEADER_BYTES + bwd_coef_scratch_bytes(N, N, D, H, W);
+}
+
+extern "C" int lf_resample3d_bwd_coef_params(const float* gout, const float* vol, int vol_n, const float* coef,
+                                             float* gcoefs, const float* jac, float* gparams, void* scratch, size_t scratch_bytes,
+                                             int N, int D, int H, int W, int C, void* stream) {
+  lf_clear_error();
+  if (!gout || !vol || !coef || !gcoefs || !jac || !gparams || !scratch) return LF_EINVAL;
+  if (N <= 0 || N > LF_TICKET_MAX_SAMPLES || D <= 0 || H <= 0 || W <= 0 || C <= 0) return LF_EINVAL;
+  if (vol_n != 1 && vol_n != N) return LF_EINVAL;
+  if (scratch_bytes < lf_resample3d_bwd_coef_params_scratch_bytes(N, D, H, W)) return LF_ENOSPC;
+  BwdCoefPlan p;
+  if (int e = bwd_coef_plan(gout, vol, scratch_bytes - LF_TICKET_HEADER_BYTES, N, N, D, H, W, C, p)) return e;
+  const long bstride = vol_n == 1 ? 0 : p.nvox * C;
+  hipStream_t s = (hipStream_t)stream;
+  float* partial = (float*)((char*)scratch + LF_TICKET_HEADER_BYTES);
+  const CoefChain chain = {(unsigned*)scratch, gcoefs, jac, gparams};
+  if (g_resample_variant >= 2 && p.vec && C == 16 && p.vpb >= 64 && p.nvox * 64 < 0xffffffffL) {
+    if (p.vpb >= 256)
+      hipLaunchKernelGGL((resample_bwd_coef_c16_dedup_chain_kernel<2, 1, true>), p.grid, dim3(256), 0, s, gout, vol, bstride, coef, partial, p.nblk, p.vpb, p.bt, D, H, W, p.st, chain);
+    else
+      hipLaunchKernelGGL((resample_bwd_coef_c16_chain_kernel<8, 1>), p.grid, dim3(256), 0, s, gout, vol, bstride, coef, partial, p.nblk, p.vpb, p.bt, D, H, W, p.st, chain);
+  } else if (p.vec) {
+    hipLaunchKernelGGL((resample_bwd_coef_chain_kernel<4>), p.grid, dim3(256), 0, s, gout, vol, bstride, coef, partial, p.nblk, p.vpb, p.bt, N, D, H, W, C, p.lpv, p.st, chain);
+  } else {
+    hipLaunchKernelGGL((resample_bwd_coef_chain_kernel<1>), p.grid, dim3(256), 0, s, gout, vol, bstride, coef, partial, p.nblk, p.vpb, p.bt, N, D, H, W, C, p.lpv, p.st, chain);
+  }
+  return lf_launch_status();
+}
+
 extern "C" int lf_resample3d_bwd_coef_part(const float* gout, const float* vol, int vol_n, const float* coef,
                                            float* gcoef, void* scratch, size_t scratch_bytes,
                                            int N, int D, int H, int W, int C, int part_n, void* stream) {
diff --git a/latentfusion_amd/csrc/resample_gather.inc b/latentfusion_amd/csrc/resample_gather.inc
--- a/latentfusion_amd/csrc/resample_gather.inc
+++ b/latentfusion_amd/csrc/resample_gather.inc
@@ -46,7 +46,7 @@
 __global__ void __launch_bounds__(256) GATHER_KERNEL(resample_bwd_coef)(
     const float* __restrict__ gout, const float* __restrict__ vol, long vol_bstride, GATHER_TABLE_PARAMS
     const float* __restrict__ coef, float* __restrict__ partial, int nblk, int vpb, BwdTile bt,
-    int N, int D, int H, int W, int C, int lpv, Steps st) {
+    int N, int D, int H, int W, int C, int lpv, Steps st GATHER_CHAIN_PARAMS) {
   const unsigned fb = xcd_contiguous(blockIdx.x, gridDim.x);
   const int n = fb / nblk, blk = fb - n * nblk;
   const float* cf = coef + (long)n * LF_MAP_COEFS;
@@ -121,8 +121,9 @@
   __syncthreads();
   if (threadIdx.x < 18) {
     const float s = (red[0][threadIdx.x] + red[1][threadIdx.x]) + (red[2][threadIdx.x] + red[3][threadIdx.x]);
-    partial[((long)n * nblk + blk) * 18 + threadIdx.x] = s;
-  }
+    GATHER_PARTIAL_STORE(partial + ((long)n * nblk + blk) * 18 + threadIdx.x, s);
+  }
+  GATHER_CHAIN_TAIL
 }
 
 template <int KIND>
@@ -205,7 +206,7 @@
 __global__ void __launch_bounds__(256, MINW) GATHER_KERNEL(resample_bwd_coef_c16)(
     const float* __restrict__ gout, const float* __restrict__ vol, long vol_bstride, GATHER_TABLE_PARAMS
     const float* __restrict__ coef, float* __restrict__ partial, int nblk, int vpb, BwdTile bt,
-    int D, int H, int W, Steps st) {
+    int D, int H, int W, Steps st GATHER_CHAIN_PARAMS) {
   const unsigned fb = xcd_contiguous(blockIdx.x, gridDim.x);
   const int n = fb / nblk, blk = fb - n * nblk;
   const float* cf = coef + n * LF_MAP_COEFS;
@@ -273,15 +274,16 @@
   __syncthreads();
   if (threadIdx.x < 18) {
     const double s = (red[0][threadIdx.x] + red[1][threadIdx.x]) + (red[2][threadIdx.x] + red[3][threadIdx.x]);
-    partial[((long)n * nblk + blk) * 18 + threadIdx.x] = (float)s;
-  }
+    GATHER_PARTIAL_STORE(partial + ((long)n * nblk + blk) * 18 + threadIdx.x, (float)s);
+  }
+  GATHER_CHAIN_TAIL
 }
 
 template <int PIF, int MINW, bool GOPF = false>
 __global__ void __launch_bounds__(256, MINW) GATHER_KERNEL(resample_bwd_coef_c16_dedup)(
     const float* __restrict__ gout, const float* __restrict__ vol, long vol_bstride, GATHER_TABLE_PARAMS
     const float* __restrict__ coef, float* __restrict__ partial, int nblk, int vpb, BwdTile bt,
-    int D, int H, int W, Steps st) {
+    int D, int H, int W, Steps st GATHER_CHAIN_PARAMS) {
   __shared__ u32x4_t tapbuf[4][64];
   __shared__ float pbuf[4][64 * 8];
   __shared__ double red[4][18];
@@ -428,6 +430,7 @@
   __syncthreads();
   if (threadIdx.x < 18) {
     const double s = (red[0][threadIdx.x] + red[1][threadIdx.x]) + (red[2][threadIdx.x] + red[3][threadIdx.x]);
-    partial[((long)n * nblk + blk) * 18 + threadIdx.x] = (float)s;
-  }
-}
+    GATHER_PARTIAL_STORE(partial + ((long)n * nblk + blk) * 18 + threadIdx.x, (float)s);
+  }
+  GATHER_CHAIN_TAIL
+}
diff --git a/latentfusion_amd/engine.py b/latentfusion_amd/engine.py
--- a/latentfusion_amd/engine.py
+++ b/latentfusion_amd/engine.py
@@ -295,6 +295,10 @@
     PROJ_KERNEL = 'library'
     LATENT_KERNEL = 'autograd'
 
+    CHAIN_ITEMS = {5: 'coefficient-gradient finish + camera chain rule in lf_resample3d_bwd_coef_params',
+                   6: 'padded O2C block from lf_camera_coefs_padded'}
+    chain = 'fused'
+
     @staticmethod
     def supports(photographer, loss_weights):
         return (photographer.projection_type in ('factor', 'sum')
@@ -312,6 +316,7 @@
         self.ph = photographer
         self.cube = photographer.cube_size
         dev = z_obj.device
+        self._items, self._scratch = frozenset(), {}
         self.z = self._resident_volume(photographer, z_obj)
         self.S = self.z.shape[-1]
         self.C = self.z.shape[1]
@@ -548,6 +553,7 @@
     def _forward_backward_group(self, params, intr, z_span, need_grad, grad_scale, zt=None, masked_depth=False):
         n = params.shape[0]
         flags = LF_EPI_LRELU | LF_EPI_PIXELNORM
+        self._items = self._chain_items(masked_depth)
         coefs, jac, cf20 = self._coefficients(params, intr, z_span, n)
         proj_gemm = self.PROJ_GEMM and self._wide_factor and not need_grad
         acts, norms, rode = self._blocks_fwd(self._resample(cf20, n), flags, proj_gemm)
@@ -599,12 +605,35 @@
             g = self.plan.data_grad(i, g, acts, norms, flags, bounds)
         return self._finish_backward(g, g_cf, cf20, jac, n, grad_scale, losses)
 
+    def _chain_items(self, masked_depth):
+        if self.chain == 'split':
+            return frozenset()
+        if self.chain != 'fused' and not set(self.chain) <= set(self.CHAIN_ITEMS):
+            raise ValueError(f"chain is 'fused', 'split' or a set of {sorted(self.CHAIN_ITEMS)}, not {self.chain!r}")
+        base = RenderLoopEngine
+        plain = all(getattr(type(self), f) is getattr(base, f) for f in ('_loss_fwd', '_loss_bwd', '_bwd_coef', '_resample'))
+        if not plain or self.generic_tail or self.dec is None or masked_depth:
+            return frozenset()
+        return frozenset(self.CHAIN_ITEMS) if self.chain == 'fused' else frozenset(self.chain)
+
+    def _ticket_scratch(self, kind, nbytes):
+        key = (kind, _s())
+        t = self._scratch.get(key)
+        if t is None or t.numel() * 4 < nbytes:
+            t = self._scratch[key] = torch.zeros(nbytes // 4 + 1, device=self.dev, dtype=torch.float32)
+        return t
+
     def _coefficients(self, params, intr, z_span, n):
         L = _lib.lib()
         params = params.contiguous()
         intr = intr.contiguous()
         coefs = torch.empty(n, NCOEF, device=self.dev, dtype=torch.float32)
         jac = torch.empty(n, NCOEF, NPAR, device=self.dev, dtype=torch.float32)
+        if 6 in self._items:
+            cf20 = torch.empty(n, 20, device=self.dev, dtype=torch.float32)
+            check(L.lf_camera_coefs_padded(params.data_ptr(), intr.data_ptr(), float(self.cube), z_span, self.crop, self.crop,
+                                           coefs.data_ptr(), jac.data_ptr(), cf20.data_ptr(), n, _s()), 'lf_camera_coefs_padded')
+            return coefs, jac, cf20
         check(L.lf_camera_coefs(params.data_ptr(), intr.data_ptr(), float(self.cube), z_span, self.crop,
                                 self.crop, coefs.data_ptr(), jac.data_ptr(), n, _s()), 'lf_camera_coefs')
         cf20 = torch.empty(n, 20, device=self.dev, dtype=torch.float32)
@@ -832,6 +861,18 @@
     def _finish_backward(self, g, g_cf, cf20, jac, n, grad_scale, losses):
         L = _lib.lib()
         dev, s = self.dev, _s()
+        if 5 in self._items:
+            S = self.S
+            gcoefs = g_cf.contiguous()
+            gparams = torch.empty(n, NPAR, device=dev, dtype=torch.float32)
+            scratch = self._ticket_scratch('coef', L.lf_resample3d_bwd_coef_params_scratch_bytes(n, S, S, S))
+            with ops._timed('resample_bwd_coef'):
+                check(L.lf_resample3d_bwd_coef_params(g.data_ptr(), self.z.data_ptr(), 1, cf20.data_ptr(), gcoefs.data_ptr(),
+                                                      jac.data_ptr(), gparams.data_ptr(), scratch.data_ptr(), scratch.numel() * 4,
+                                                      n, S, S, S, self.C, s), 'lf_resample3d_bwd_coef_params')
+            if grad_scale != 1.0:
+                gparams *= grad_scale
+            return losses, gparams
         gcoef18 = torch.empty(n, 18, device=dev, dtype=torch.float32)
         self._bwd_coef(g, cf20, gcoef18, n)
         gcoefs = g_cf.contiguous()
```

Result: no change. 198.8, median of 6 (+0.6%).
